# aexoden/snesimage

Measured on AMD Instinct MI355X. Metric: candidate palettes scored/sec, higher is better.
Workload: dtype f32

## Files before the change

snesimage_amd/csrc/capi.hip:

```cpp
#include "../../include/snesimage_hip.h"
#include "kernels.hpp"
#include "kernels_opt.hpp"
#include "kernels_fast.hpp"
#include "kernels_sparse.hpp"
#include "kernels_sparse2.hpp"
#include "kernels_batch.hpp"
#include "kernels_shared.hpp"
#include "kernels_tile.hpp"
#include "kernels_level.hpp"
#include "kernels_char.hpp"
#include "kernels_char_set.hpp"
#include "kernels_export.hpp"
#include "kernels_import.hpp"
#include "kernels_guide.hpp"
#include "kernels_guide_lab.hpp"
#include "kernels_guide_window.hpp"
#include "kernels_guide_set_window.hpp"

#include <hip/hip_runtime.h>

#include <atomic>
#include <cmath>
#include <cstdio>
#include <cstdlib>
// ... 65 lines not shown
    z = (z ^ (z >> 30)) * 0xBF58476D1CE4E5B9ull;
    z = (z ^ (z >> 27)) * 0x94D049BB133111EBull;
    return z ^ (z >> 31);
}

template <typename T> void dfree(T *&p) { if (p) { (void)hipFree(p); p = nullptr; } }

std::atomic<int> g_fail_alloc_in{-1};
template <typename T> hipError_t dmalloc(T **p, size_t bytes) {
    int left = g_fail_alloc_in.load(std::memory_order_relaxed);
    while (left >= 0) {
        if (g_fail_alloc_in.compare_exchange_weak(left, left - 1, std::memory_order_relaxed)) { if (left == 0) { *p = nullptr; return hipErrorOutOfMemory; } break; }
    }
    return hipMalloc(p, bytes);
}
std::atomic<bool> g_poison_alloc{false};

}

struct snesimage_ctx {
    int device = 0;
    hipStream_t own_stream = nullptr, stream = nullptr;
    uint32_t W = 0, H = 0, sub_count = 0, sub_size = 0, flags = 0;
    int ncol = 0;
    bool dither = false, perceptual = false, nes = false;
    bool backdrop = false, tied_call = false; uint32_t user_size = 0;
    bool dither4 = true; uint32_t dither4_max = 512;
    bool ditherw = true;
    bool dither_rec = true;
    Geom G{};
    BlurK K{};
    size_t npx = 0, src_floats = 0;
    uint32_t chunk = 4096, chunk_alloc = 0;

    std::vector<uint8_t> h_orig; float h_eotf[256], h_lab_eotf[256];

    uint8_t *d_orig = nullptr, *d_tile_pal = nullptr, *d_colors = nullptr, *d_map = nullptr;
    unsigned long long *d_pack = nullptr, *d_packT = nullptr, *d_packC4 = nullptr, *d_packR4 = nullptr;
    float *d_img1C4 = nullptr, *d_mu1R4 = nullptr, *d_sd1R4 = nullptr, *d_a1 = nullptr, *d_a1R4 = nullptr; double *d_r1 = nullptr, *d_r1R4 = nullptr;
    int fast_mask = 0;
    float *d_eotf = nullptr, *d_lab_eotf = nullptr;
    uint32_t *d_pal_rgb8 = nullptr; float *d_pal_lin = nullptr, *d_pal_xyb = nullptr, *d_pal_lab = nullptr;
    float *d_lin0 = nullptr, *d_img1 = nullptr, *d_img1T = nullptr, *d_mu1 = nullptr, *d_sd1 = nullptr;
    float *d_labpx = nullptr, *d_labpxT = nullptr;
    uint8_t *d_target = nullptr, *d_target_own = nullptr; float *d_labpx_t = nullptr, *d_labpxT_t = nullptr, *d_labpx_t_own = nullptr, *d_labpxT_t_own = nullptr;
    uint32_t od_n = 0; int8_t od_tab[256] = {};
    uint32_t od_L = 0; int8_t od_bank[8 * 256] = {}; uint8_t od_level[1024] = {}; uint8_t *d_level = nullptr;
    struct snesimage_levelwork *lvl = nullptr;
    float *d_work = nullptr, *d_cand_tab = nullptr, *d_cand_lab = nullptr;
    double *d_part = nullptr;
    uint8_t *d_maps = nullptr, *d_mapsT = nullptr, *d_mapsC4 = nullptr, *d_mapsR4 = nullptr;
    uint8_t *d_subC4 = nullptr, *d_subR4 = nullptr;
    uint8_t *d_bestmap = nullptr, *d_bestmaps_all = nullptr; BestRec *d_bestrec = nullptr, *d_bestrecs_all = nullptr; int *d_skip = nullptr;
    uint4 *d_rplist = nullptr; int *d_rcount = nullptr;
    float *d_rtab = nullptr, *d_rlab = nullptr; uint32_t rtab_cap = 0;
    bool map_pending = false;
    bool best_valid = false, map_synced = false;
    struct Lane { hipStream_t stream = nullptr; float *d_work = nullptr, *d_cand_tab = nullptr, *d_cand_lab = nullptr; double *d_part = nullptr; uint8_t *d_maps = nullptr, *d_mapsT = nullptr, *d_mapsC4 = nullptr, *d_mapsR4 = nullptr, *d_bestmap = nullptr; BestRec *d_bestrec = nullptr; hipEvent_t done = nullptr; };
    std::vector<Lane> extra; uint32_t nlanes = 2; hipEvent_t ev_ready = nullptr;
    struct Sparse {
        bool lpt = true;
        bool down1 = true;
        bool counters_cleared = false;
        uint32_t h2q_max = 512;
        bool down_tiles = true;
        uint32_t h0_min = 1024;
        bool base_down_side = false;
        uint32_t h0_grid = 8192;
        hipStream_t h0_stream[8] = {}; hipEvent_t ev_scan[8] = {}, ev_h0[8] = {}, ev_hn[8] = {}, ev_vn[8] = {};
        bool v0_aside = true;
        hipEvent_t ev_v0[8] = {};
        bool vn_aside = true;
        uint32_t tiles_grid = 4096;
        uint32_t down1_grid = 32768;
        bool vsplit = true;
        uint32_t scan4_max = 2048;
        uint32_t hgrid = 8192;
        bool weight_mask = true;
        bool h_planes = true;
        bool v2_pair = true;
        uint32_t h_forms = 3;
        bool debug_poison = false;
        bool dedup = true; uint32_t dedup_min = 1024; int *holder = nullptr; bool holder_dirty = false;
        bool enabled = false, side = true; uint32_t min_n = 1; uint32_t cap = 0, lanes = 0;
        SparseGeom S{};
        float *store = nullptr, *cand_tab = nullptr, *cand_lab = nullptr, *ckf = nullptr, *ckh = nullptr; long long zeros_off = 0; uint32_t *bitmap = nullptr; double *cka = nullptr, *part = nullptr;
        CandMeta *meta = nullptr; unsigned int *items = nullptr; int *item_count = nullptr; long long item_stride = 0; int *order = nullptr, *first = nullptr;
        uint4 *plist = nullptr; int *plist_count = nullptr; bool plist_valid = false;
        hipStream_t base_stream = nullptr; hipEvent_t ev_base_in = nullptr, ev_base_h = nullptr, ev_base_done = nullptr, ev_base_narrow = nullptr;
        uint8_t *dmaps = nullptr, *dmapsC4 = nullptr;
        uint8_t *bmap = nullptr, *bmapC4 = nullptr, *bcand = nullptr; unsigned long long *dpack = nullptr; double *ckd = nullptr; uint32_t slot_ci = 0;
        float *rec_lab = nullptr;
        int base_sp = -1, base_si = -1;
        struct Ahead { uint8_t *bmap = nullptr, *bmapC4 = nullptr, *bcand = nullptr; unsigned long long *dpack = nullptr; double *ckd = nullptr; float *btab = nullptr, *blab = nullptr, *rec_lab = nullptr; int *ok = nullptr;
                       hipEvent_t ev = nullptr; bool on = true, have = false; int sp = -1, si = -1; unsigned long long epoch = 0; } ahead;
    } sp;
    uint8_t *d_cand = nullptr; uint32_t cand_cap = 0;
    uint8_t *d_cand_sel = nullptr;
    double *d_errs = nullptr, *d_errs_sel = nullptr;
    double *d_inc_err = nullptr;
    StepResult *d_last = nullptr;
    double *d_scratch_err = nullptr;
    uint8_t *d_dummy_cand = nullptr;
    KmeansWork km{};
    double *d_tile_cost = nullptr; int *d_tile_any = nullptr; unsigned int *d_tile_moved = nullptr;

    struct snesimage_batch *owner = nullptr;
    struct snesimage_group *group = nullptr;
    hipEvent_t ev_own = nullptr;
    struct snesimage_window *win = nullptr;
    bool win_pend = false;
    bool pack_borrowed = false;
    uint32_t pb_w = 1, pb_h = 1;
    struct snesimage_tilework *tile = nullptr;
    struct snesimage_charwork *chr = nullptr;
    struct snesimage_guidework *guide = nullptr;
    uint32_t guide_proxy = 0;
    bool guide_capture = false; std::vector<uint8_t> guide_captured; uint32_t guide_captured_k = 0;

    bool tables_valid = false, src_valid = false, inc_valid = false;
    unsigned long long epoch = 0; bool epoch_by_commit = false;
    int pack_mode = -1, pack_sp = -1, pack_si = -1; bool pack_valid = false;
    uint32_t pend_n = 0, pend_sp = 0, pend_si = 0, pend_method = 0; bool pend = false;

    int timing = 0;
    double t_ms[3] = {0.0, 0.0, 0.0}; uint64_t t_launches = 0, t_cands = 0;
    struct TimingRec { hipEvent_t ev[6]; uint32_t n; bool light; };
    std::vector<TimingRec> t_pending;
};

namespace {

int32_t alloc_lane(snesimage_ctx *c, uint32_t chunk, float *&d_work, float *&d_cand_tab, float *&d_cand_lab, double *&d_part, uint8_t *&d_maps, uint8_t *&d_mapsT, uint8_t *&d_mapsC4, uint8_t *&d_mapsR4) {
    dfree(d_work); dfree(d_cand_tab); dfree(d_cand_lab); dfree(d_part); dfree(d_maps); dfree(d_mapsT); dfree(d_mapsC4); dfree(d_mapsR4);
    HIPCHK(dmalloc(&d_work, sizeof(float) * (size_t)c->G.cand_stride * chunk));
    HIPCHK(dmalloc(&d_cand_tab, sizeof(float) * 8 * (size_t)chunk));
    HIPCHK(dmalloc(&d_cand_lab, sizeof(float) * 3 * (size_t)chunk));
    HIPCHK(dmalloc(&d_part, sizeof(double) * (size_t)chunk * kMaxScales * 18));
    if (c->dither) {
        HIPCHK(dmalloc(&d_maps, c->npx * (size_t)chunk));
        HIPCHK(dmalloc(&d_mapsT, c->npx * (size_t)chunk));
        HIPCHK(dmalloc(&d_mapsC4, c->npx * (size_t)chunk));
        HIPCHK(dmalloc(&d_mapsR4, c->npx * (size_t)chunk));
    }
    return SNES_OK;
}
int32_t alloc_workspace(snesimage_ctx *c, uint32_t chunk, uint32_t lanes = 1) {
    if (c->dither || c->perceptual) lanes = c->nlanes;
    if (lanes > c->nlanes) lanes = c->nlanes;
    if (lanes < c->extra.size() + 1) lanes = (uint32_t)c->extra.size() + 1;
    if (c->chunk_alloc >= chunk && c->extra.size() + 1 >= lanes) return SNES_OK;
    if (chunk < c->chunk_alloc) chunk = c->chunk_alloc;
    HIPCHK(hipStreamSynchronize(c->stream));
    for (auto &L : c->extra) HIPCHK(hipStreamSynchronize(L.stream));
    c->chunk_alloc = 0;
    CHECK(alloc_lane(c, chunk, c->d_work, c->d_cand_tab, c->d_cand_lab, c->d_part, c->d_maps, c->d_mapsT, c->d_mapsC4, c->d_mapsR4));
    if (!c->ev_ready) HIPCHK(hipEventCreateWithFlags(&c->ev_ready, hipEventDisableTiming));
    while (c->extra.size() + 1 < lanes) {
        snesimage_ctx::Lane L;
        HIPCHK(hipStreamCreateWithFlags(&L.stream, hipStreamNonBlocking));
        HIPCHK(hipEventCreateWithFlags(&L.done, hipEventDisableTiming));
        c->extra.push_back(L);
    }
    for (auto &L : c->extra) CHECK(alloc_lane(c, chunk, L.d_work, L.d_cand_tab, L.d_cand_lab, L.d_part, L.d_maps, L.d_mapsT, L.d_mapsC4, L.d_mapsR4));
    if (c->dither && !c->d_bestmaps_all) {
        HIPCHK(dmalloc(&c->d_bestmaps_all, c->npx * (size_t)c->nlanes));
        HIPCHK(dmalloc(&c->d_bestrecs_all, sizeof(BestRec) * c->nlanes));
        HIPCHK(dmalloc(&c->d_skip, sizeof(int)));
    }
    if (c->d_bestmaps_all) {
        c->d_bestmap = c->d_bestmaps_all; c->d_bestrec = c->d_bestrecs_all;
        for (size_t l = 0; l < c->extra.size(); l++) { c->extra[l].d_bestmap = c->d_bestmaps_all + (l + 1) * c->npx; c->extra[l].d_bestrec = c->d_bestrecs_all + (l + 1); }
    }
    c->chunk_alloc = chunk;
    return SNES_OK;
}

int32_t ensure_cand_capacity(snesimage_ctx *c, uint32_t n) {
    if (c->cand_cap >= n) return SNES_OK;
    if (c->stream) HIPCHK(hipStreamSynchronize(c->stream));
    c->cand_cap = 0;
    dfree(c->d_cand); dfree(c->d_cand_sel); dfree(c->d_errs); dfree(c->d_errs_sel);
    uint32_t cap = n < 64 ? 64 : n;
    HIPCHK(dmalloc(&c->d_cand, 3 * (size_t)cap));
    HIPCHK(dmalloc(&c->d_cand_sel, 3 * (size_t)cap));
    HIPCHK(dmalloc(&c->d_errs, sizeof(double) * cap));
    HIPCHK(dmalloc(&c->d_errs_sel, sizeof(double) * cap));
    c->cand_cap = cap;
    return SNES_OK;
}

int32_t ensure_tables(snesimage_ctx *c) {
    if (c->tables_valid) return SNES_OK;
    int n = c->ncol + 2;
    hipLaunchKernelGGL(k_palette_tables, dim3((n + 63) / 64), dim3(64), 0, c->stream, c->d_colors, c->ncol, c->d_eotf, c->d_pal_rgb8, c->d_pal_lin, c->d_pal_xyb);
    if (c->perceptual)
        hipLaunchKernelGGL(k_palette_lab, dim3((c->ncol + 63) / 64), dim3(64), 0, c->stream, c->d_pal_rgb8, c->ncol, c->d_lab_eotf, c->d_pal_lab);
    HIPCHK(hipGetLastError());
    c->tables_valid = true;
    return SNES_OK;
}

int32_t ensure_source(snesimage_ctx *c) {
    if (c->src_valid) return SNES_OK;
    CHECK(alloc_workspace(c, 1));
    const Geom &G = c->G;
    hipLaunchKernelGGL(k_source_scale0, dim3((unsigned)((c->npx + 255) / 256)), dim3(256), 0, c->stream, c->d_orig, c->d_eotf, (int)c->W, (int)c->H, c->d_lin0,
                       c->d_img1, c->d_img1T);
    if (G.nscales > 1) {
        DownParams D{}; D.G = G; D.lin0 = c->d_lin0; D.work = c->d_img1; D.workT = c->d_img1T;
        hipLaunchKernelGGL(k_downscale_chain<false>, dim3(down_grid(G), 1), dim3(256), 0, c->stream, D);
    }
    for (int s = 0; s < G.nscales; s++) {
        HParams Hp{}; Hp.G = G; Hp.K = c->K; Hp.s = s; Hp.npairs = 3; Hp.ncol = c->ncol;
        Hp.in1T = c->d_img1T + G.src_off[s]; Hp.in2T = c->d_img1T + G.src_off[s]; Hp.work = c->d_work;
        int ppw = 256 / G.sh[s];
        hipLaunchKernelGGL((k_hpass<false, false>), dim3((3 + ppw - 1) / ppw), dim3(256), 0, c->stream, Hp);
        VParams Vp{}; Vp.G = G; Vp.K = c->K; Vp.s = s; Vp.npairs = 3; Vp.ncol = c->ncol;
        Vp.img1 = c->d_img1 + G.src_off[s]; Vp.mu1_out = c->d_mu1 + G.src_off[s]; Vp.sd1_out = c->d_sd1 + G.src_off[s]; Vp.a1_out = c->d_a1 + G.src_off[s]; Vp.r1_out = c->d_r1 + G.src_off[s]; Vp.work = c->d_work;
        int ppv = 256 / G.sw[s];
        hipLaunchKernelGGL((k_vpass<false, true, false>), dim3((3 + ppv - 1) / ppv), dim3(256), 0, c->stream, Vp);
    }
    bool padded = false;
    for (int s = 0; s < G.nscales; s++) padded = padded || G.th[s] != G.sh[s];
    if (padded)
        hipLaunchKernelGGL(k_src_pad_rows, dim3(16, G.nscales), dim3(256), 0, c->stream, G, c->d_sd1, c->d_r1);
    for (int s = 0; s < G.nscales; s++)
        if ((c->fast_mask & (1 << s)) || c->sp.enabled) {
            const int N = G.sw[s] * G.sh[s];
            hipLaunchKernelGGL(k_relayout, dim3((N + 255) / 256), dim3(256), 0, c->stream, c->d_img1 + G.src_off[s], G.sw[s], G.sh[s], (float *)nullptr, c->d_img1C4 + G.src_off[s]);
            hipLaunchKernelGGL(k_relayout, dim3((N + 255) / 256), dim3(256), 0, c->stream, c->d_mu1 + G.src_off[s], G.sw[s], G.sh[s], c->d_mu1R4 + G.src_off[s], (float *)nullptr);
            hipLaunchKernelGGL(k_relayout, dim3((N + 255) / 256), dim3(256), 0, c->stream, c->d_sd1 + G.src_off[s], G.sw[s], G.sh[s], c->d_sd1R4 + G.src_off[s], (float *)nullptr);
            hipLaunchKernelGGL(k_relayout, dim3((N + 255) / 256), dim3(256), 0, c->stream, c->d_a1 + G.src_off[s], G.sw[s], G.sh[s], c->d_a1R4 + G.src_off[s], (float *)nullptr);
            hipLaunchKernelGGL(k_relayout_f64, dim3((N + 255) / 256), dim3(256), 0, c->stream, c->d_r1 + G.src_off[s], G.sw[s], G.sh[s], c->d_r1R4 + G.src_off[s]);
        }
    if (c->perceptual)
        hipLaunchKernelGGL(k_pixel_lab, dim3((unsigned)((c->npx + 255) / 256)), dim3(256), 0, c->stream, c->d_orig, c->d_lab_eotf, (int)c->W, (int)c->H, c->d_labpx, c->d_labpxT);
    HIPCHK(hipGetLastError());
    c->src_valid = true;
    return SNES_OK;
}

int32_t run_prep(snesimage_ctx *c, int mode, int sp, int si) {
    if (c->pack_valid && c->pack_mode == mode && ((mode != 2 && mode != 3) || (c->pack_sp == sp && c->pack_si == si))) return SNES_OK;
    CHECK(ensure_tables(c));
    if (c->perceptual) CHECK(ensure_source(c));
    PrepParams P{};
    P.orig = c->d_target; P.tile_pal = c->d_tile_pal; P.pal_rgb8 = c->d_pal_rgb8; P.map = c->d_map; P.pack = c->d_pack; P.packT = c->d_packT; P.packC4 = c->d_packC4; P.packR4 = c->d_packR4; P.subC4 = c->d_subC4; P.subR4 = c->d_subR4;
    P.labpx = c->d_labpx_t; P.pal_lab = c->d_pal_lab;
    P.W = (int)c->W; P.H = (int)c->H; P.sub_size = (int)c->sub_size; P.ncol = c->ncol; P.mode = mode; P.sp = sp; P.si = si; P.perceptual = c->perceptual ? 1 : 0;
    c->sp.counters_cleared = false;
    if (mode == 2 && c->sp.plist_count) {
        P.zero = c->sp.plist_count; P.nzero = 1; c->sp.counters_cleared = true;
    }
    hipLaunchKernelGGL(k_prep, dim3((unsigned)((c->npx + 255) / 256)), dim3(256), 0, c->stream, P);
    HIPCHK(hipGetLastError());
    c->pack_valid = true; c->pack_mode = mode; c->pack_sp = sp; c->pack_si = si;
    c->sp.plist_valid = false;
    return SNES_OK;
}

int32_t prep_for_slot(snesimage_ctx *c, int sp, int si) { return c->dither ? run_prep(c, 1, -1, -1) : (c->tied_call ? run_prep(c, 3, -1, si) : run_prep(c, 2, sp, si)); }

struct DenseView {
    const unsigned long long *pack, *packT, *packC4, *packR4; const uint8_t *subC4, *subR4, *tile_pal;
    float *work, *cand_tab, *cand_lab; double *part; const uint8_t *maps, *mapsT, *mapsC4, *mapsR4;
    bool use_maps, perceptual;
};
int32_t score_stages(snesimage_ctx *c, const DenseView &V, uint32_t nc, double *d_errors, int err_stride, int err_offset, snesimage_ctx::TimingRec *tr) {
    const Geom &G = c->G;
    const int npairs = (int)nc * 3;
    if (G.nscales > 1) {
        DownParams D{}; D.G = G; D.pack = V.pack; D.pal_lin = c->d_pal_lin; D.cand_tab = V.cand_tab; D.cand_lab = V.cand_lab; D.labpx = c->d_labpx_t;
        D.work = V.work; D.ncol = c->ncol; D.perceptual = V.perceptual ? 1 : 0; D.use_maps = V.use_maps ? 1 : 0; D.fast_mask = c->fast_mask & ~1; D.maps = V.maps; D.tile_pal = V.tile_pal; D.sub_size = (int)c->sub_size;
        hipLaunchKernelGGL(k_downscale_chain<true>, dim3(down_grid(G), nc), dim3(256), 0, c->stream, D);
    }
    const bool fast0 = (c->fast_mask & 1) && (V.use_maps || !V.perceptual);
    auto is_fast = [&](int s) { return s == 0 ? fast0 : ((c->fast_mask >> s) & 1) != 0; };
    auto fast_params = [&](int s) {
        FastParams F{}; F.G = G; F.K = c->K; F.s = s; F.npairs = npairs; F.ncol = c->ncol;
        F.packC4 = V.packC4; F.packR4 = V.packR4; F.pal_xyb = c->d_pal_xyb; F.cand_tab = V.cand_tab;
        F.use_maps = V.use_maps ? 1 : 0; F.mapsC4 = reinterpret_cast<const uint32_t *>(V.mapsC4); F.mapsR4 = reinterpret_cast<const uint32_t *>(V.mapsR4);
        F.subC4 = reinterpret_cast<const uint32_t *>(V.subC4); F.subR4 = reinterpret_cast<const uint32_t *>(V.subR4);
        F.img1C4 = c->d_img1C4 + G.src_off[s]; F.mu1R4 = c->d_mu1R4 + G.src_off[s]; F.sd1R4 = c->d_sd1R4 + G.src_off[s]; F.a1R4 = c->d_a1R4 + G.src_off[s]; F.r1R4 = c->d_r1R4 + G.src_off[s];
        F.work = V.work; F.part = V.part;
        return F;
    };
    for (int s = 0; s < G.nscales; s++) {
        if (s == 0 && tr && c->timing == 1) HIPCHK(hipEventRecord(tr->ev[1], c->stream));
        if (is_fast(s)) {
            FastParams F = fast_params(s);
            dim3 grid((unsigned)(npairs * (G.sh[s] / 64)));
            if (s == 0) hipLaunchKernelGGL((k_hpass_fast<true>), grid, dim3(64), 0, c->stream, F);
            else hipLaunchKernelGGL((k_hpass_fast<false>), grid, dim3(64), 0, c->stream, F);
        } else {
            HParams Hp{}; Hp.G = G; Hp.K = c->K; Hp.s = s; Hp.npairs = npairs; Hp.ncol = c->ncol; Hp.perceptual = V.perceptual ? 1 : 0; Hp.use_maps = V.use_maps ? 1 : 0; Hp.sub_size = (int)c->sub_size;
            Hp.packT = V.packT; Hp.pal_xyb = c->d_pal_xyb; Hp.cand_tab = V.cand_tab; Hp.cand_lab = V.cand_lab; Hp.labpxT = c->d_labpxT_t;
            Hp.in1T = c->d_img1T + G.src_off[s]; Hp.in2T = nullptr; Hp.work = V.work; Hp.mapsT = V.mapsT; Hp.tile_pal = V.tile_pal;
            int ppw = 256 / G.sh[s];
            dim3 grid((npairs + ppw - 1) / ppw);
            if (s == 0) {
                if (V.perceptual && !V.use_maps) hipLaunchKernelGGL((k_hpass<true, true>), grid, dim3(256), 0, c->stream, Hp);
                else hipLaunchKernelGGL((k_hpass<true, false>), grid, dim3(256), 0, c->stream, Hp);
            } else hipLaunchKernelGGL((k_hpass<false, false>), grid, dim3(256), 0, c->stream, Hp);
        }
        if (s == 0 && tr && c->timing == 1) HIPCHK(hipEventRecord(tr->ev[2], c->stream));
        if (s == 0 && tr && c->timing) HIPCHK(hipEventRecord(tr->ev[3], c->stream));
        int ppv = 256 / G.sw[s];
        dim3 grid((npairs + ppv - 1) / ppv);
        if (is_fast(s)) {
            FastParams F = fast_params(s);
            if (s == 0) hipLaunchKernelGGL((k_vpass_fast<true>), grid, dim3(256), 0, c->stream, F);
            else hipLaunchKernelGGL((k_vpass_fast<false>), grid, dim3(256), 0, c->stream, F);
        } else {
            VParams Vp{}; Vp.G = G; Vp.K = c->K; Vp.s = s; Vp.npairs = npairs; Vp.ncol = c->ncol; Vp.perceptual = V.perceptual ? 1 : 0; Vp.use_maps = V.use_maps ? 1 : 0; Vp.sub_size = (int)c->sub_size;
            Vp.pack = V.pack; Vp.pal_xyb = c->d_pal_xyb; Vp.cand_tab = V.cand_tab; Vp.cand_lab = V.cand_lab; Vp.labpx = c->d_labpx_t;
            Vp.mu1 = c->d_mu1 + G.src_off[s]; Vp.sd1 = c->d_sd1 + G.src_off[s]; Vp.a1 = c->d_a1 + G.src_off[s]; Vp.r1 = c->d_r1 + G.src_off[s]; Vp.work = V.work; Vp.part = V.part;
            Vp.maps = V.maps; Vp.tile_pal = V.tile_pal;
            if (s == 0) {
                if (V.perceptual && !V.use_maps) hipLaunchKernelGGL((k_vpass<true, false, true>), grid, dim3(256), 0, c->stream, Vp);
                else hipLaunchKernelGGL((k_vpass<true, false, false>), grid, dim3(256), 0, c->stream, Vp);
            } else hipLaunchKernelGGL((k_vpass<false, false, false>), grid, dim3(256), 0, c->stream, Vp);
        }
        if (s == 0 && tr && c->timing) HIPCHK(hipEventRecord(tr->ev[4], c->stream));
    }
    hipLaunchKernelGGL(k_final_score, dim3((nc + 63) / 64), dim3(64), 0, c->stream, V.part, (int)nc, G, d_errors, err_stride, err_offset);
    return SNES_OK;
}

void launch_dither(snesimage_ctx *c, const DitherParams &Dp, uint32_t nblocks) {
    if (c->perceptual && c->dither4 && nblocks <= c->dither4_max) hipLaunchKernelGGL((k_dither4_lab<0>), dim3(nblocks), dim3(512), 0, c->stream, Dp);
    else if (c->perceptual) hipLaunchKernelGGL((k_dither<true, 0>), dim3(nblocks), dim3(128), 0, c->stream, Dp);
    else if (c->dither4 && nblocks <= c->dither4_max && c->sub_size == 15) hipLaunchKernelGGL((k_dither4<15, 0>), dim3(nblocks), dim3(512), 0, c->stream, Dp);
    else if (c->dither4 && nblocks <= c->dither4_max && c->sub_size == 16) hipLaunchKernelGGL((k_dither4<16, 0>), dim3(nblocks), dim3(512), 0, c->stream, Dp);
    else if (c->dither4 && nblocks <= c->dither4_max) hipLaunchKernelGGL((k_dither4<0, 0>), dim3(nblocks), dim3(512), 0, c->stream, Dp);
    else if (c->sub_size == 15) hipLaunchKernelGGL((k_dither<false, 15>), dim3(nblocks), dim3(128), 0, c->stream, Dp);
    else if (c->sub_size == 16) hipLaunchKernelGGL((k_dither<false, 16>), dim3(nblocks), dim3(128), 0, c->stream, Dp);
    else hipLaunchKernelGGL((k_dither<false, 0>), dim3(nblocks), dim3(128), 0, c->stream, Dp);
}

int32_t score_chunk(snesimage_ctx *c, const uint8_t *d_rgb5, uint32_t nc, double *d_errors, int err_stride, int err_offset, int sp, int si, uint8_t *d_maps_out) {
    const bool use_maps = c->dither;
    const uint32_t slot_ci = c->tied_call ? (kTiedSlot | (c->sub_size << 8) | (uint32_t)si) : (sp >= 0) ? (uint32_t)(sp * (int)c->sub_size + si) : 0xffffffffu;
    snesimage_ctx::TimingRec tr{}; tr.n = nc;
    if (c->timing) { for (int i = 0; i < 6; i++) HIPCHK(hipEventCreate(&tr.ev[i])); if (c->timing == 1) HIPCHK(hipEventRecord(tr.ev[0], c->stream)); }
    hipLaunchKernelGGL(k_candidate_tables, dim3((nc + 63) / 64), dim3(64), 0, c->stream, d_rgb5, (int)nc, c->d_eotf, c->d_cand_tab);
    hipLaunchKernelGGL(k_candidate_slot, dim3((nc + 63) / 64), dim3(64), 0, c->stream, c->d_cand_tab, (int)nc, slot_ci);
    if (c->perceptual) hipLaunchKernelGGL(k_candidate_lab, dim3((nc + 63) / 64), dim3(64), 0, c->stream, c->d_cand_tab, (int)nc, c->d_lab_eotf, c->d_cand_lab);
    if (use_maps) {
        DitherParams Dp{};
        Dp.orig = c->d_orig; Dp.tile_pal = c->d_tile_pal; Dp.pal_rgb8 = c->d_pal_rgb8; Dp.pal_lab = c->d_pal_lab; Dp.cand_tab = c->d_cand_tab; Dp.cand_lab = c->d_cand_lab;
        Dp.lab_eotf = c->d_lab_eotf; Dp.maps = c->d_maps; Dp.mapsC4 = c->d_mapsC4;
        Dp.W = (int)c->W; Dp.H = (int)c->H; Dp.sub_size = (int)c->sub_size; Dp.ncol = c->ncol; Dp.slot_ci = slot_ci; Dp.perceptual = c->perceptual ? 1 : 0;
        launch_dither(c, Dp, nc);
        hipLaunchKernelGGL(k_maps_relayout, dim3((unsigned)(c->H / 4), nc), dim3(256), 0, c->stream, c->d_maps, (int)c->W, (int)c->H,
                           reinterpret_cast<uint32_t *>(c->d_mapsR4), (c->fast_mask & 1) ? (uint32_t *)nullptr : reinterpret_cast<uint32_t *>(c->d_mapsT));
        if (d_maps_out) HIPCHK(hipMemcpyAsync(d_maps_out, c->d_maps, c->npx * (size_t)nc, hipMemcpyDeviceToDevice, c->stream));
    } else if (d_maps_out) {
        MapsParams M{}; M.pack = c->d_pack; M.cand_tab = c->d_cand_tab; M.cand_lab = c->d_cand_lab; M.labpx = c->d_labpx_t; M.maps = d_maps_out;
        M.npx = (int)c->npx; M.ncol = c->ncol; M.sub_size = (int)c->sub_size; M.si = si < 0 ? 0 : si; M.ncand = (int)nc; M.perceptual = c->perceptual ? 1 : 0;
        hipLaunchKernelGGL(k_candidate_maps, dim3((unsigned)((c->npx + 255) / 256), nc), dim3(256), 0, c->stream, M);
    }
    { DenseView V{c->d_pack, c->d_packT, c->d_packC4, c->d_packR4, c->d_subC4, c->d_subR4, c->d_tile_pal, c->d_work, c->d_cand_tab, c->d_cand_lab, c->d_part, c->d_maps, c->d_mapsT, c->d_mapsC4, c->d_mapsR4,
                  use_maps, c->perceptual};
      CHECK(score_stages(c, V, nc, d_errors, err_stride, err_offset, &tr)); }
    if (use_maps) hipLaunchKernelGGL(k_keep_best, dim3(1), dim3(1024), 0, c->stream, d_errors, err_stride, err_offset, (int)nc, c->d_maps, (int)c->npx, c->d_bestrec, c->d_bestmap);
    HIPCHK(hipGetLastError());
    if (c->timing) { tr.light = c->timing != 1; if (!tr.light) HIPCHK(hipEventRecord(tr.ev[5], c->stream)); c->t_pending.push_back(tr); }
    return SNES_OK;
}

SparseParams sparse_params(snesimage_ctx *c, uint32_t lane);

int32_t sparse_alloc(snesimage_ctx *c, uint32_t need, uint32_t lanes = 1) {
    auto &sp = c->sp;
    if (lanes > c->nlanes) lanes = c->nlanes;
    if (sp.cap >= need && sp.lanes >= lanes) return SNES_OK;
    if (need < sp.cap) need = sp.cap;
    if (lanes < sp.lanes) lanes = sp.lanes;
    HIPCHK(hipStreamSynchronize(c->stream));
    for (auto &L : c->extra) HIPCHK(hipStreamSynchronize(L.stream));
    if (sp.base_stream) HIPCHK(hipStreamSynchronize(sp.base_stream));
    sp.cap = 0; sp.lanes = 0; sp.plist_valid = false;
    dfree(sp.store); dfree(sp.cand_tab); dfree(sp.ckf); dfree(sp.cka); dfree(sp.part); dfree(sp.meta); dfree(sp.items); dfree(sp.item_count); dfree(sp.plist); sp.plist_count = nullptr;
    const Geom &G = c->G;
    SparseGeom &S = sp.S;
    long long off = 0, okf = 0, oka = 0, okh = 0; int go = 0;
    for (int s = 0; s < G.nscales; s++) {
        const long long N = (long long)G.sw[s] * G.sh[s];
        S.off_lin[s] = off; if (s >= 1) off += 3 * N;
        S.off_xybC[s] = off; if (s >= 1) off += 3 * N;
        S.off_xybR[s] = off; off += 3 * N;
        S.off_hout[s] = off; off += 9 * N;
        S.off_ckf[s] = okf; okf += 3LL * (G.sh[s] / 4 + 2) * 18 * G.sw[s];
        S.off_cka[s] = oka; oka += 3LL * (G.sh[s] / 4 + 2) * 6 * G.sw[s];
        S.off_ckh[s] = okh; if (G.sw[s] >= 64) okh += 3LL * 3 * 18 * G.sh[s];
        S.goff[s] = go; go += G.sh[s] / 4;
    }
    S.cand_stride = off;
    const size_t ncap = (size_t)lanes * need + 1;
    sp.item_stride = (long long)need * (G.sh[0] / 4) * 3;
    HIPCHK(dmalloc(&sp.store, sizeof(float) * (size_t)S.cand_stride * ncap));
    if (g_poison_alloc.load()) HIPCHK(hipMemsetAsync(sp.store, 0xff, sizeof(float) * (size_t)S.cand_stride * ncap, c->stream));
    HIPCHK(dmalloc(&sp.cand_tab, sizeof(float) * 8 * ncap));
    if (c->perceptual) {
        dfree(sp.cand_lab); dfree(sp.bitmap);
        HIPCHK(dmalloc(&sp.cand_lab, sizeof(float) * 3 * ncap));
        HIPCHK(dmalloc(&sp.bitmap, sizeof(uint32_t) * (c->npx / 32) * ncap));
    }
    HIPCHK(dmalloc(&sp.ckf, sizeof(float) * (size_t)okf));
    dfree(sp.ckh); HIPCHK(dmalloc(&sp.ckh, sizeof(float) * (size_t)(okh + 12LL * G.W + 256)));
    sp.zeros_off = okh;
    HIPCHK(hipMemsetAsync(sp.ckh + okh, 0, sizeof(float) * 12 * (size_t)G.W, c->stream));
    HIPCHK(dmalloc(&sp.cka, sizeof(double) * (size_t)oka));
    HIPCHK(dmalloc(&sp.part, sizeof(double) * ncap * kMaxScales * 18));
    HIPCHK(dmalloc(&sp.meta, sizeof(CandMeta) * ncap));
    dfree(sp.order); HIPCHK(dmalloc(&sp.order, sizeof(int) * ncap));
    dfree(sp.first); HIPCHK(dmalloc(&sp.first, sizeof(int) * ncap));
    HIPCHK(dmalloc(&sp.items, sizeof(unsigned int) * (size_t)sp.item_stride * kItemLists * (c->nlanes + 1)));
    if (!sp.base_stream && sp.side) {
        int prio_lo = 0, prio_hi = 0;
        HIPCHK(hipDeviceGetStreamPriorityRange(&prio_lo, &prio_hi));
        HIPCHK(hipStreamCreateWithPriority(&sp.base_stream, hipStreamNonBlocking, prio_hi));
        HIPCHK(hipEventCreateWithFlags(&sp.ev_base_in, hipEventDisableTiming));
        HIPCHK(hipEventCreateWithFlags(&sp.ev_base_h, hipEventDisableTiming));
        HIPCHK(hipEventCreateWithFlags(&sp.ev_base_narrow, hipEventDisableTiming));
        HIPCHK(hipEventCreateWithFlags(&sp.ev_base_done, hipEventDisableTiming));
    }
    HIPCHK(dmalloc(&sp.item_count, sizeof(int) * (kItemLists * (c->nlanes + 1) + 1)));
    HIPCHK(hipMemsetAsync(sp.item_count, 0, sizeof(int) * (kItemLists * (c->nlanes + 1) + 1), c->stream));
    sp.plist_count = sp.item_count + (size_t)kItemLists * (c->nlanes + 1);
    sp.counters_cleared = true;
    HIPCHK(dmalloc(&sp.plist, sizeof(uint4) * c->npx));
    if (c->dither) {
        dfree(sp.dmaps); dfree(sp.dmapsC4); dfree(sp.bmap); dfree(sp.bmapC4); dfree(sp.bcand); dfree(sp.dpack); dfree(sp.ckd);
        HIPCHK(dmalloc(&sp.dmaps, c->npx * (size_t)need * lanes));
        HIPCHK(dmalloc(&sp.dmapsC4, c->npx * (size_t)need * lanes));
        HIPCHK(dmalloc(&sp.bmap, c->npx)); HIPCHK(dmalloc(&sp.bmapC4, c->npx)); HIPCHK(dmalloc(&sp.bcand, 64));
        HIPCHK(dmalloc(&sp.dpack, sizeof(unsigned long long) * c->npx));
        HIPCHK(dmalloc(&sp.ckd, sizeof(double) * 3 * c->W * (c->H / 4 + 1)));
        dfree(sp.rec_lab); if (c->perceptual) HIPCHK(dmalloc(&sp.rec_lab, sizeof(float) * 3 * c->npx));
        auto &ah = sp.ahead;
        dfree(ah.bmap); dfree(ah.bmapC4); dfree(ah.bcand); dfree(ah.dpack); dfree(ah.ckd); dfree(ah.btab); dfree(ah.blab); dfree(ah.rec_lab); dfree(ah.ok); ah.have = false;
        if (ah.on && sp.side && c->sub_size > 1) {
            HIPCHK(dmalloc(&ah.bmap, c->npx)); HIPCHK(dmalloc(&ah.bmapC4, c->npx)); HIPCHK(dmalloc(&ah.bcand, 64)); HIPCHK(dmalloc(&ah.btab, sizeof(float) * 8)); HIPCHK(dmalloc(&ah.ok, sizeof(int)));
            HIPCHK(dmalloc(&ah.dpack, sizeof(unsigned long long) * c->npx));
            HIPCHK(dmalloc(&ah.ckd, sizeof(double) * 3 * c->W * (c->H / 4 + 1)));
            if (c->perceptual) { HIPCHK(dmalloc(&ah.blab, sizeof(float) * 3)); HIPCHK(dmalloc(&ah.rec_lab, sizeof(float) * 3 * c->npx)); }
            if (!ah.ev) HIPCHK(hipEventCreateWithFlags(&ah.ev, hipEventDisableTiming));
        }
    }
    sp.cap = need; sp.lanes = lanes; sp.plist_valid = false;
    {
        SparseParams P = sparse_params(c, c->nlanes);
        P.is_base = 1; P.ncand = 1; P.k0 = P.base;
        hipLaunchKernelGGL(k_sparse_scan, dim3(1), dim3(1024), 0, c->stream, P);
        HIPCHK(hipGetLastError());
    }
    HIPCHK(hipStreamSynchronize(c->stream));
    return SNES_OK;
}

SparseParams sparse_params(snesimage_ctx *c, uint32_t lane) {
    auto &sp = c->sp;
    SparseParams P{};
    P.G = c->G; P.S = sp.S; P.K = c->K; P.ncol = c->ncol; P.base = (int)(sp.lanes * sp.cap);
    P.pack = c->d_pack; P.packC4 = c->d_packC4; P.packR4 = c->d_packR4; P.plist = sp.plist; P.plist_count = sp.plist_count;
    P.pal_lin = c->d_pal_lin; P.pal_xyb = c->d_pal_xyb; P.cand_tab = sp.cand_tab;
    P.perceptual = c->perceptual ? 1 : 0; P.labpx = c->d_labpx_t; P.cand_lab = sp.cand_lab; P.bitmap = sp.bitmap;
    P.img1C4 = c->d_img1C4; P.mu1R4 = c->d_mu1R4; P.sd1R4 = c->d_sd1R4; P.a1R4 = c->d_a1R4; P.r1R4 = c->d_r1R4;
    P.store = sp.store; P.meta = sp.meta;
    P.items = sp.items + (size_t)lane * sp.item_stride * kItemLists; P.item_count = sp.item_count + (size_t)lane * kItemLists; P.item_stride = sp.item_stride;
    P.ckf = sp.ckf; P.cka = sp.cka; P.part = sp.part; P.first = sp.first; P.ckh = sp.ckh; P.zeros = sp.ckh + sp.zeros_off; P.trash = sp.ckh + sp.zeros_off + 12LL * c->G.W;
    for (P.s_first = 0; P.s_first < c->G.nscales && c->G.sw[P.s_first] >= 64; P.s_first++) {}
    P.full_sums = sp.weight_mask ? 0 : 1;
    P.h_planes = (sp.weight_mask && sp.h_planes) ? 1 : 0;
    P.v2_pair = (sp.weight_mask && sp.v2_pair) ? v2_pair_channels(c->G) : 0;
    if (c->dither) {
        const uint32_t l = lane < c->nlanes ? lane : 0;
        P.use_maps = 1; P.sub_size = (int)c->sub_size; P.slot_ci = sp.slot_ci; P.subC4 = c->d_subC4; P.tile_pal = c->d_tile_pal;
        P.perceptual = 0; P.labpx = sp.rec_lab;
        P.maps = sp.dmaps + (size_t)l * sp.cap * c->npx; P.mapsC4 = sp.dmapsC4 + (size_t)l * sp.cap * c->npx; P.bmap = sp.bmap; P.bmapC4 = sp.bmapC4;
    }
    return P;
}

static size_t h2_lds(const snesimage_ctx *c) { return sizeof(float) * 3 * (size_t)(c->ncol + 2); }

static void launch_sparse_h2(const snesimage_ctx *c, const SparseParams &P, size_t gx, unsigned ny, bool h0_only, hipStream_t st) {
    const uint32_t forms = c->sp.h_forms;
    const size_t lds = h2_lds(c);
    const int nfree = h2_free_channels(c->G);
    if ((forms & 4) && h0_only && P.h_planes && !P.full_sums && nfree > 0 && nfree < 3) {
        size_t g1 = gx * (size_t)nfree / 3; if (g1 < 1) g1 = 1;
        const size_t g2 = gx - gx * (size_t)nfree / 3 + 1;
        const dim3 d1((unsigned)g1, ny), d2((unsigned)g2, ny);
        if (!(forms & 2)) { hipLaunchKernelGGL(k_sparse_h2_one<-1>, d1, dim3(64), lds, st, P); hipLaunchKernelGGL(k_sparse_h2_full<-1>, d2, dim3(64), lds, st, P); }
        else if (c->dither) { hipLaunchKernelGGL(k_sparse_h2_one<1>, d1, dim3(64), lds, st, P); hipLaunchKernelGGL(k_sparse_h2_full<1>, d2, dim3(64), lds, st, P); }
        else { hipLaunchKernelGGL(k_sparse_h2_one<0>, d1, dim3(64), lds, st, P); hipLaunchKernelGGL(k_sparse_h2_full<0>, d2, dim3(64), lds, st, P); }
        return;
    }
    const dim3 d((unsigned)gx, ny);
    if (!(forms & 2)) hipLaunchKernelGGL(k_sparse_h2, d, dim3(64), lds, st, P);
    else if (c->dither) hipLaunchKernelGGL(k_sparse_h2_um<true>, d, dim3(64), lds, st, P);
    else hipLaunchKernelGGL(k_sparse_h2_um<false>, d, dim3(64), lds, st, P);
}

int32_t sparse_base_pass(snesimage_ctx *c, int sp_idx, int si, uint32_t n_cand) {
    auto &sp = c->sp;
    const Geom &G = c->G;
    if (!sp.plist_valid) {
        if (!sp.counters_cleared) HIPCHK(hipMemsetAsync(sp.plist_count, 0, sizeof(int), c->stream));
        sp.counters_cleared = false;
        const unsigned long long *win_pack = c->d_pack;
        if (c->dither) {
            const uint32_t j0 = c->sub_size > 1 ? ((uint32_t)si + 1u) % c->sub_size : (uint32_t)si;
            sp.slot_ci = (uint32_t)(sp_idx * (int)c->sub_size + si);
            auto &ah = sp.ahead;
            const int *b_done = nullptr;
            const bool same_state = ah.epoch == c->epoch;
            if (ah.have && ah.sp == sp_idx && ah.si == si && (same_state || (ah.epoch + 1 == c->epoch && c->epoch_by_commit))) {
                std::swap(sp.bmap, ah.bmap); std::swap(sp.bmapC4, ah.bmapC4); std::swap(sp.dpack, ah.dpack); std::swap(sp.ckd, ah.ckd); std::swap(sp.rec_lab, ah.rec_lab);
                hipLaunchKernelGGL(k_ahead_ok, dim3(1), dim3(1), 0, c->stream, same_state ? (const StepResult *)nullptr : c->d_last, ah.ok);
                HIPCHK(hipStreamWaitEvent(c->stream, ah.ev, 0));
                b_done = ah.ok;
            }
            ah.have = false;
            HIPCHK(hipMemcpyAsync(sp.bcand, c->d_colors + 3 * (size_t)(sp_idx * (int)c->sub_size + (int)j0), 3, hipMemcpyDeviceToDevice, c->stream));
            float *btab = sp.cand_tab + 8 * (size_t)(sp.lanes * sp.cap);
            hipLaunchKernelGGL(k_candidate_tables, dim3(1), dim3(64), 0, c->stream, sp.bcand, 1, c->d_eotf, btab);
            DitherParams Dp{};
            Dp.orig = c->d_orig; Dp.tile_pal = c->d_tile_pal; Dp.pal_rgb8 = c->d_pal_rgb8; Dp.cand_tab = btab; Dp.maps = sp.bmap; Dp.mapsC4 = sp.bmapC4;
            Dp.W = (int)c->W; Dp.H = (int)c->H; Dp.sub_size = (int)c->sub_size; Dp.ncol = c->ncol; Dp.slot_ci = sp.slot_ci;
            Dp.rec_pack = sp.dpack; Dp.ck_out = sp.ckd; Dp.excl_sub = sp_idx; Dp.excl_si = si; Dp.excl_j0 = (int)j0; Dp.skip = b_done;
            if (c->perceptual) {
                float *blab = sp.cand_lab + 3 * (size_t)(sp.lanes * sp.cap);
                hipLaunchKernelGGL(k_candidate_lab, dim3(1), dim3(64), 0, c->stream, btab, 1, c->d_lab_eotf, blab);
                Dp.pal_lab = c->d_pal_lab; Dp.cand_lab = blab; Dp.lab_eotf = c->d_lab_eotf; Dp.perceptual = 1; Dp.rec_lab = sp.rec_lab;
                if (c->dither4) hipLaunchKernelGGL((k_dither4_lab<1>), dim3(1), dim3(512), 0, c->stream, Dp); else hipLaunchKernelGGL((k_dither<true, 0, 1>), dim3(1), dim3(128), 0, c->stream, Dp);
            } else
            if (c->dither4 && c->sub_size == 15) hipLaunchKernelGGL((k_dither4<15, 1>), dim3(1), dim3(512), 0, c->stream, Dp);
            else if (c->dither4 && c->sub_size == 16) hipLaunchKernelGGL((k_dither4<16, 1>), dim3(1), dim3(512), 0, c->stream, Dp);
            else if (c->dither4) hipLaunchKernelGGL((k_dither4<0, 1>), dim3(1), dim3(512), 0, c->stream, Dp);
            else if (c->sub_size == 15) hipLaunchKernelGGL((k_dither<false, 15, 1>), dim3(1), dim3(128), 0, c->stream, Dp);
            else if (c->sub_size == 16) hipLaunchKernelGGL((k_dither<false, 16, 1>), dim3(1), dim3(128), 0, c->stream, Dp);
            else hipLaunchKernelGGL((k_dither<false, 0, 1>), dim3(1), dim3(128), 0, c->stream, Dp);
            win_pack = sp.dpack;
        }
        hipLaunchKernelGGL(k_build_plist, dim3((unsigned)((c->npx + 255) / 256)), dim3(256), 0, c->stream, win_pack, (int)c->npx, sp.plist, sp.plist_count);
        SparseParams P = sparse_params(c, c->nlanes);
        P.is_base = 1; P.ncand = 1; P.k0 = P.base;
        hipStream_t bs = sp.side ? sp.base_stream : c->stream;
        const bool down_with_sweeps = sp.side && n_cand >= sp.h0_min && sp.h0_min > 0;
        sp.base_down_side = down_with_sweeps;
        if (!down_with_sweeps) hipLaunchKernelGGL(k_base_down, dim3(down_grid(G)), dim3(256), 0, c->stream, P);
        if (sp.side) { HIPCHK(hipEventRecord(sp.ev_base_in, c->stream)); HIPCHK(hipStreamWaitEvent(bs, sp.ev_base_in, 0)); }
        if (down_with_sweeps) hipLaunchKernelGGL(k_base_down, dim3(down_grid(G)), dim3(256), 0, bs, P);
        if (sp.h2q_max > 0) hipLaunchKernelGGL(k_sparse_h2q_base, dim3((unsigned)((G.sh[0] / 4 * 3 + 3) / 4), (unsigned)(P.s_first * kColBuckets)), dim3(64), h2_lds(c), bs, P);
        else hipLaunchKernelGGL(k_sparse_h2_base, dim3((unsigned)((G.sh[0] / 4 * 3 + 15) / 16), (unsigned)(P.s_first * kColBuckets)), dim3(64), h2_lds(c), bs, P);
        if (sp.side) HIPCHK(hipEventRecord(sp.ev_base_h, bs));
        if (P.s_first > 0 && sp.vsplit) hipLaunchKernelGGL(k_sparse_v2_base_split, dim3((unsigned)(G.W >> 6), 3, (unsigned)P.s_first), dim3(128), 0, bs, P);
        else if (P.s_first > 0) hipLaunchKernelGGL(k_sparse_v2_base, dim3(3, (unsigned)P.s_first), dim3(256), 0, bs, P);
        if (sp.side) HIPCHK(hipEventRecord(sp.ev_base_done, bs));
        if (P.s_first < G.nscales) hipLaunchKernelGGL(k_sparse_h, dim3((unsigned)((G.sh[P.s_first] / 4 * 3 + 15) / 16), (unsigned)((G.nscales - P.s_first) * kColBuckets)), dim3(64), 0, bs, P);
        if (P.s_first < G.nscales) hipLaunchKernelGGL(k_sparse_v_base_narrow, dim3(3, (unsigned)(G.nscales - P.s_first)), dim3(256), 0, bs, P);
        HIPCHK(hipGetLastError());
        if (sp.side) HIPCHK(hipEventRecord(sp.ev_base_narrow, bs));
        if (c->dither && sp.side && sp.ahead.dpack) {
            auto &ah = sp.ahead;
            int ni = si + 1, np = sp_idx;
            if (ni == (int)c->sub_size) { ni = 0; np = (np + 1) % (int)c->sub_count; }
            const int nj0 = (ni + 1) % (int)c->sub_size;
            HIPCHK(hipMemcpyAsync(ah.bcand, c->d_colors + 3 * (size_t)(np * (int)c->sub_size + nj0), 3, hipMemcpyDeviceToDevice, bs));
            hipLaunchKernelGGL(k_candidate_tables, dim3(1), dim3(64), 0, bs, ah.bcand, 1, c->d_eotf, ah.btab);
            DitherParams Dn{};
            Dn.orig = c->d_orig; Dn.tile_pal = c->d_tile_pal; Dn.pal_rgb8 = c->d_pal_rgb8; Dn.cand_tab = ah.btab; Dn.maps = ah.bmap; Dn.mapsC4 = ah.bmapC4;
            Dn.W = (int)c->W; Dn.H = (int)c->H; Dn.sub_size = (int)c->sub_size; Dn.ncol = c->ncol; Dn.slot_ci = (uint32_t)(np * (int)c->sub_size + ni);
            Dn.rec_pack = ah.dpack; Dn.ck_out = ah.ckd; Dn.excl_sub = np; Dn.excl_si = ni; Dn.excl_j0 = nj0;
            if (c->perceptual) {
                hipLaunchKernelGGL(k_candidate_lab, dim3(1), dim3(64), 0, bs, ah.btab, 1, c->d_lab_eotf, ah.blab);
                Dn.pal_lab = c->d_pal_lab; Dn.cand_lab = ah.blab; Dn.lab_eotf = c->d_lab_eotf; Dn.perceptual = 1; Dn.rec_lab = ah.rec_lab;
                if (c->dither4) hipLaunchKernelGGL((k_dither4_lab<1>), dim3(1), dim3(512), 0, bs, Dn); else hipLaunchKernelGGL((k_dither<true, 0, 1>), dim3(1), dim3(128), 0, bs, Dn);
            } else
            if (c->dither4 && c->sub_size == 15) hipLaunchKernelGGL((k_dither4<15, 1>), dim3(1), dim3(512), 0, bs, Dn);
            else if (c->dither4 && c->sub_size == 16) hipLaunchKernelGGL((k_dither4<16, 1>), dim3(1), dim3(512), 0, bs, Dn);
            else if (c->dither4) hipLaunchKernelGGL((k_dither4<0, 1>), dim3(1), dim3(512), 0, bs, Dn);
            else if (c->sub_size == 15) hipLaunchKernelGGL((k_dither<false, 15, 1>), dim3(1), dim3(128), 0, bs, Dn);
            else if (c->sub_size == 16) hipLaunchKernelGGL((k_dither<false, 16, 1>), dim3(1), dim3(128), 0, bs, Dn);
            else hipLaunchKernelGGL((k_dither<false, 0, 1>), dim3(1), dim3(128), 0, bs, Dn);
            HIPCHK(hipGetLastError());
            HIPCHK(hipEventRecord(ah.ev, bs));
            ah.have = true; ah.sp = np; ah.si = ni; ah.epoch = c->epoch;
        }
        sp.plist_valid = true;
    }
    return SNES_OK;
}

int32_t sparse_score_chunk(snesimage_ctx *c, uint32_t lane, hipStream_t stream, const uint8_t *d_rgb5, uint32_t nc, double *d_errors, int err_stride, int err_offset, int list0 = -1) {
    auto &sp = c->sp;
    const Geom &G = c->G;
    SparseParams P = sparse_params(c, lane);
    P.is_base = 0; P.ncand = (int)nc; P.k0 = (int)(lane * sp.cap);
    if (list0 >= 0) { P.holder = sp.holder; P.list0 = list0; }
    if (sp.debug_poison) HIPCHK(hipMemsetAsync(sp.store + (size_t)P.k0 * sp.S.cand_stride, 0xff, sizeof(float) * (size_t)sp.S.cand_stride * nc, stream));
    snesimage_ctx::TimingRec tr{}; tr.n = nc;
    if (c->timing) { for (int i = 0; i < 6; i++) HIPCHK(hipEventCreate(&tr.ev[i])); if (c->timing == 1) HIPCHK(hipEventRecord(tr.ev[0], stream)); }
    if (list0 >= 0) hipLaunchKernelGGL(k_candidate_tables_mark, dim3((nc + 63) / 64), dim3(64), 0, stream, d_rgb5, (int)nc, c->d_eotf, sp.cand_tab + 8 * (size_t)P.k0, sp.holder, list0);
    else
    hipLaunchKernelGGL(k_candidate_tables, dim3((nc + 63) / 64), dim3(64), 0, stream, d_rgb5, (int)nc, c->d_eotf, sp.cand_tab + 8 * (size_t)P.k0);
    if (c->dither) {
        if (c->perceptual) {
            hipLaunchKernelGGL(k_candidate_lab, dim3((nc + 63) / 64), dim3(64), 0, stream, sp.cand_tab + 8 * (size_t)P.k0, (int)nc, c->d_lab_eotf, sp.cand_lab + 3 * (size_t)P.k0);
            hipLaunchKernelGGL(k_dither_first_lab, dim3(nc), dim3(256), 0, stream, P);
        } else
        hipLaunchKernelGGL(k_dither_first, dim3((nc + 15) / 16), dim3(1024), 0, stream, P);
        DitherParams Dp{};
        Dp.orig = c->d_orig; Dp.tile_pal = c->d_tile_pal; Dp.pal_rgb8 = c->d_pal_rgb8; Dp.cand_tab = sp.cand_tab + 8 * (size_t)P.k0;
        Dp.maps = const_cast<uint8_t *>(P.maps); Dp.mapsC4 = const_cast<uint8_t *>(P.mapsC4);
        Dp.W = (int)c->W; Dp.H = (int)c->H; Dp.sub_size = (int)c->sub_size; Dp.ncol = c->ncol; Dp.slot_ci = sp.slot_ci;
        Dp.first_group = sp.first; Dp.first_k0 = P.k0; Dp.ck_in = sp.ckd; Dp.bmap = sp.bmap; Dp.bmapC4 = sp.bmapC4; Dp.rec_in = c->dither_rec ? sp.dpack : nullptr;
        if (c->sp.lpt) {
            hipLaunchKernelGGL(k_sparse_order, dim3(1), dim3(1024), 0, stream, P, sp.order + P.k0); Dp.order = sp.order + P.k0;
        }
        if (c->perceptual) {
            Dp.pal_lab = c->d_pal_lab; Dp.cand_lab = sp.cand_lab + 3 * (size_t)P.k0; Dp.lab_eotf = c->d_lab_eotf; Dp.perceptual = 1;
            if (c->dither4 && nc <= c->dither4_max) hipLaunchKernelGGL((k_dither4_lab<2>), dim3(nc), dim3(512), 0, stream, Dp); else hipLaunchKernelGGL((k_dither<true, 0, 2>), dim3(nc), dim3(128), 0, stream, Dp);
        } else
        if (c->dither4 && nc <= c->dither4_max && c->sub_size == 15) hipLaunchKernelGGL((k_dither4<15, 2>), dim3(nc), dim3(512), 0, stream, Dp);
        else if (c->dither4 && nc <= c->dither4_max && c->sub_size == 16) hipLaunchKernelGGL((k_dither4<16, 2>), dim3(nc), dim3(512), 0, stream, Dp);
        else if (c->dither4 && nc <= c->dither4_max) hipLaunchKernelGGL((k_dither4<0, 2>), dim3(nc), dim3(512), 0, stream, Dp);
        else if (c->ditherw && c->sub_size == 15) hipLaunchKernelGGL((k_ditherw<15>), dim3((nc + 3) / 4), dim3(256), 0, stream, Dp, (int)nc);
        else if (c->ditherw && c->sub_size == 16) hipLaunchKernelGGL((k_ditherw<16>), dim3((nc + 3) / 4), dim3(256), 0, stream, Dp, (int)nc);
        else if (c->ditherw && c->sub_size > 1) hipLaunchKernelGGL((k_ditherw<0>), dim3((nc + 3) / 4), dim3(256), 0, stream, Dp, (int)nc);
        else if (c->sub_size == 15) hipLaunchKernelGGL((k_dither<false, 15, 2>), dim3(nc), dim3(128), 0, stream, Dp);
        else if (c->sub_size == 16) hipLaunchKernelGGL((k_dither<false, 16, 2>), dim3(nc), dim3(128), 0, stream, Dp);
        else hipLaunchKernelGGL((k_dither<false, 0, 2>), dim3(nc), dim3(128), 0, stream, Dp);
        hipLaunchKernelGGL(k_dither_diff, dim3((nc + 3) / 4), dim3(1024), 0, stream, P);
    } else if (c->perceptual) {
        hipLaunchKernelGGL(k_candidate_lab, dim3((nc + 63) / 64), dim3(64), 0, stream, sp.cand_tab + 8 * (size_t)P.k0, (int)nc, c->d_lab_eotf, sp.cand_lab + 3 * (size_t)P.k0);
        HIPCHK(hipMemsetAsync(sp.bitmap + (size_t)P.k0 * (c->npx / 32), 0, sizeof(uint32_t) * (c->npx / 32) * nc, stream));
        hipLaunchKernelGGL(k_sparse_scan_lab, dim3(nc), dim3(256), 0, stream, P);
    } else if (nc <= sp.scan4_max) hipLaunchKernelGGL(k_sparse_scan4, dim3((nc + 3) / 4), dim3(1024), 0, stream, P);
    else hipLaunchKernelGGL(k_sparse_scan, dim3((nc + 15) / 16), dim3(1024), 0, stream, P);
    bool vn_aside = false;
    const bool h0_ahead = sp.side && sp.h0_min > 0 && nc >= sp.h0_min && nc > sp.h2q_max && lane < 8 && P.s_first > 0;
    const bool v0_aside = h0_ahead && sp.v0_aside;
    vn_aside = h0_ahead && !v0_aside && sp.vn_aside && P.s_first < G.nscales;
    if (c->sp.lpt && nc > 512) P.order = sp.order + P.k0;
    if (h0_ahead) {
        if (!sp.h0_stream[lane]) {
            HIPCHK(hipStreamCreateWithFlags(&sp.h0_stream[lane], hipStreamNonBlocking));
            HIPCHK(hipEventCreateWithFlags(&sp.ev_scan[lane], hipEventDisableTiming));
            HIPCHK(hipEventCreateWithFlags(&sp.ev_h0[lane], hipEventDisableTiming));
            HIPCHK(hipEventCreateWithFlags(&sp.ev_hn[lane], hipEventDisableTiming));
            HIPCHK(hipEventCreateWithFlags(&sp.ev_v0[lane], hipEventDisableTiming));
            HIPCHK(hipEventCreateWithFlags(&sp.ev_vn[lane], hipEventDisableTiming));
        }
        hipStream_t hs = sp.h0_stream[lane];
        HIPCHK(hipEventRecord(sp.ev_scan[lane], stream));
        HIPCHK(hipStreamWaitEvent(hs, sp.ev_scan[lane], 0));
        HIPCHK(hipStreamWaitEvent(hs, sp.ev_base_h, 0));
        size_t gx = ((size_t)nc * (G.sh[0] / 4) * 3 + 15) / 16; if (gx > sp.h0_grid) gx = sp.h0_grid;
        launch_sparse_h2(c, P, gx, (unsigned)kColBuckets, true, hs);
        if (c->sp.lpt) hipLaunchKernelGGL(k_sparse_order, dim3(1), dim3(1024), 0, hs, P, sp.order + P.k0);
        HIPCHK(hipEventRecord(sp.ev_h0[lane], hs));
        if (v0_aside) {
            HIPCHK(hipStreamWaitEvent(hs, sp.ev_base_done, 0));
            if (c->timing) HIPCHK(hipEventRecord(tr.ev[3], hs));
            hipLaunchKernelGGL(k_sparse_v2, dim3(v2_pair_grid(nc, P.v2_pair), 1), dim3(256), 0, hs, P);
            if (c->timing) HIPCHK(hipEventRecord(tr.ev[4], hs));
            HIPCHK(hipEventRecord(sp.ev_v0[lane], hs));
        }
    }
    if (sp.down1 && G.nscales > 2) {
        size_t gd = (size_t)nc * 8; if (gd > sp.down1_grid) gd = sp.down1_grid;
        hipLaunchKernelGGL(k_sparse_down1, dim3((unsigned)gd), dim3(256), 0, stream, P);
        if (sp.side && sp.base_down_side) HIPCHK(hipStreamWaitEvent(stream, sp.ev_base_h, 0));
        if (sp.down_tiles && G.nscales >= 4) {
            size_t gt = ((size_t)nc * (G.sh[3] / 4) + SNES_DOWN_TILES_U - 1) / SNES_DOWN_TILES_U; if (gt > sp.tiles_grid) gt = sp.tiles_grid;
            hipLaunchKernelGGL(k_sparse_down_tiles, dim3((unsigned)gt), dim3(256), 0, stream, P);
        } else
        hipLaunchKernelGGL(k_sparse_down, dim3(nc), dim3(256), 0, stream, P, -2);
    } else { if (sp.side && sp.base_down_side) HIPCHK(hipStreamWaitEvent(stream, sp.ev_base_h, 0)); hipLaunchKernelGGL(k_sparse_down, dim3(nc), dim3(256), 0, stream, P, 0); }
    if (sp.side && !sp.base_down_side) HIPCHK(hipStreamWaitEvent(stream, sp.ev_base_h, 0));
    if (c->timing == 1) HIPCHK(hipEventRecord(tr.ev[1], stream));
    { size_t gx = ((size_t)nc * (G.sh[0] / 4) * 3 + 15) / 16; if (gx > sp.hgrid) gx = sp.hgrid;
      if (nc <= sp.h2q_max) {
          size_t gq = ((size_t)nc * (G.sh[0] / 4) * 3 + 3) / 4; if (gq > sp.hgrid) gq = sp.hgrid;
          hipLaunchKernelGGL(k_sparse_h2q, dim3((unsigned)gq, (unsigned)(P.s_first * kColBuckets)), dim3(64), h2_lds(c), stream, P);
      } else
      if (h0_ahead) {
          if (P.s_first > 1 && (sp.h_forms & 1)) hipLaunchKernelGGL(k_sparse_h2_from, dim3((unsigned)gx, (unsigned)((P.s_first - 1) * kColBuckets)), dim3(64), h2_lds(c), stream, P, (int)kColBuckets);
          else if (P.s_first > 1) hipLaunchKernelGGL(k_sparse_h2_from_all, dim3((unsigned)gx, (unsigned)((P.s_first - 1) * kColBuckets)), dim3(64), h2_lds(c), stream, P, (int)kColBuckets);
      } else
      launch_sparse_h2(c, P, gx, (unsigned)(P.s_first * kColBuckets), false, stream);
      if (P.s_first < G.nscales) hipLaunchKernelGGL(k_sparse_h, dim3((unsigned)((gx + 7) / 8), (unsigned)((G.nscales - P.s_first) * kColBuckets)), dim3(64), 0, stream, P);
      if (vn_aside) HIPCHK(hipEventRecord(sp.ev_hn[lane], stream));
      if (h0_ahead) HIPCHK(hipStreamWaitEvent(stream, sp.ev_h0[lane], 0)); }
    if (c->timing == 1) HIPCHK(hipEventRecord(tr.ev[2], stream));
    if (sp.side || stream != c->stream) HIPCHK(hipStreamWaitEvent(stream, sp.side ? sp.ev_base_done : c->ev_ready, 0));
    if (c->sp.lpt && nc > 512) {
        if (!h0_ahead) hipLaunchKernelGGL(k_sparse_order, dim3(1), dim3(1024), 0, stream, P, sp.order + P.k0);
        P.order = sp.order + P.k0;
    }
    if (vn_aside) {
        hipStream_t hs = sp.h0_stream[lane];
        HIPCHK(hipStreamWaitEvent(hs, sp.ev_hn[lane], 0));
        HIPCHK(hipStreamWaitEvent(hs, sp.ev_base_narrow, 0));
        hipLaunchKernelGGL(k_sparse_v, dim3((nc * 3 + 7) / 8, (unsigned)(G.nscales - P.s_first)), dim3(256), 0, hs, P);
        HIPCHK(hipEventRecord(sp.ev_vn[lane], hs));
    }
    if (v0_aside) {
        if (sp.side) HIPCHK(hipStreamWaitEvent(stream, sp.ev_base_narrow, 0));
        if (P.s_first < G.nscales) hipLaunchKernelGGL(k_sparse_v, dim3((nc * 3 + 7) / 8, (unsigned)(G.nscales - P.s_first)), dim3(256), 0, stream, P);
        if (P.s_first > 1) hipLaunchKernelGGL(k_sparse_v2_from, dim3(nc * 3, (unsigned)(P.s_first - 1)), dim3(256), 0, stream, P, 1);
    } else {
    if (c->timing) HIPCHK(hipEventRecord(tr.ev[3], stream));
    hipLaunchKernelGGL(k_sparse_v2, dim3(P.s_first == 1 ? v2_pair_grid(nc, P.v2_pair) : nc * 3, (unsigned)P.s_first), dim3(256), 0, stream, P);
    if (c->timing) HIPCHK(hipEventRecord(tr.ev[4], stream));
    }
    if (vn_aside) HIPCHK(hipStreamWaitEvent(stream, sp.ev_vn[lane], 0));
    else if (!v0_aside) {
    if (sp.side) HIPCHK(hipStreamWaitEvent(stream, sp.ev_base_narrow, 0));
    if (P.s_first < G.nscales) hipLaunchKernelGGL(k_sparse_v, dim3((nc * 3 + 7) / 8, (unsigned)(G.nscales - P.s_first)), dim3(256), 0, stream, P);
    }
    if (v0_aside) HIPCHK(hipStreamWaitEvent(stream, sp.ev_v0[lane], 0));
    hipLaunchKernelGGL(k_final_score_wave, dim3((nc + 3) / 4), dim3(256), 0, stream, sp.part + (size_t)P.k0 * G.nscales * 18, (int)nc, G, d_errors, err_stride, err_offset, P.item_count, (int)kItemLists);
    if (c->dither) {
        uint8_t *bm = lane == 0 ? c->d_bestmap : c->extra[lane - 1].d_bestmap; BestRec *br = lane == 0 ? c->d_bestrec : c->extra[lane - 1].d_bestrec;
        hipLaunchKernelGGL(k_keep_best, dim3(1), dim3(1024), 0, stream, d_errors, err_stride, err_offset, (int)nc, P.maps, (int)c->npx, br, bm);
    }
    HIPCHK(hipGetLastError());
    if (c->timing) { tr.light = c->timing != 1; if (!tr.light) HIPCHK(hipEventRecord(tr.ev[5], stream)); c->t_pending.push_back(tr); }
    return SNES_OK;
}

struct LaneScope {
    snesimage_ctx *c; snesimage_ctx::Lane *L;
    LaneScope(snesimage_ctx *c_, snesimage_ctx::Lane *L_) : c(c_), L(L_) { swap(); }
    ~LaneScope() { swap(); }
    void swap() { std::swap(c->stream, L->stream); std::swap(c->d_work, L->d_work); std::swap(c->d_cand_tab, L->d_cand_tab); std::swap(c->d_cand_lab, L->d_cand_lab);
                  std::swap(c->d_part, L->d_part); std::swap(c->d_maps, L->d_maps); std::swap(c->d_mapsT, L->d_mapsT); std::swap(c->d_mapsC4, L->d_mapsC4); std::swap(c->d_mapsR4, L->d_mapsR4);
                  std::swap(c->d_bestmap, L->d_bestmap); std::swap(c->d_bestrec, L->d_bestrec); }
};

int32_t score_list(snesimage_ctx *c, const uint8_t *d_rgb5, uint32_t n, double *d_errors, int err_stride, int err_offset, int sp, int si, uint8_t *d_maps_out) {
    uint32_t chunk = (c->dither || c->perceptual) ? (n + c->nlanes - 1) / c->nlanes : n;
    if (chunk < 64) chunk = 64;
    if (chunk > c->chunk) chunk = c->chunk;
    if (c->tied_call && chunk > 1024) chunk = 1024;
    const bool sparse = c->sp.enabled && !c->tied_call && !d_maps_out && sp >= 0 && n >= c->sp.min_n && c->pack_mode == (c->dither ? 1 : 2) && !(c->dither && c->sub_size == 1);
    const uint32_t nchunks = (n + chunk - 1) / chunk;
    const uint32_t nl = nchunks < c->nlanes ? nchunks : c->nlanes;
    CHECK(alloc_workspace(c, sparse ? 1 : chunk, nl));
    CHECK(ensure_tables(c));
    CHECK(ensure_source(c));
    if (sparse) {
        CHECK(sparse_alloc(c, chunk, nl));
        if (c->dither && (c->sp.base_sp != sp || c->sp.base_si != si)) c->sp.plist_valid = false;
        CHECK(sparse_base_pass(c, sp, si, n));
        c->sp.base_sp = sp; c->sp.base_si = si;
    }
    if (c->dither) { hipLaunchKernelGGL(k_reset_best, dim3(1), dim3(64), 0, c->stream, c->d_bestrecs_all, (int)c->nlanes); c->best_valid = true; }
    const bool dedup = sparse && !c->dither && c->sp.dedup && n >= c->sp.dedup_min;
    if (dedup) {
        if (!c->sp.holder) { HIPCHK(dmalloc(&c->sp.holder, sizeof(int) * kDedupColours)); c->sp.holder_dirty = true; }
        if (c->sp.holder_dirty) {
            HIPCHK(hipStreamSynchronize(c->stream));
            for (auto &L : c->extra) HIPCHK(hipStreamSynchronize(L.stream));
            HIPCHK(hipMemsetAsync(c->sp.holder, kNoHolder & 0xff, sizeof(int) * kDedupColours, c->stream));
        }
        c->sp.holder_dirty = true;
    }
    if (nl > 1) {
        HIPCHK(hipEventRecord(c->ev_ready, c->stream));
        for (uint32_t l = 1; l < nl; l++) HIPCHK(hipStreamWaitEvent(c->extra[l - 1].stream, c->ev_ready, 0));
    }
    uint32_t i = 0;
    for (uint32_t c0 = 0; c0 < n; c0 += chunk, i++) {
        const uint32_t nc = (n - c0 < chunk) ? (n - c0) : chunk;
        const uint32_t lane = i % nl;
        uint8_t *mo = d_maps_out ? d_maps_out + (size_t)c0 * c->npx : nullptr;
        const int eo = err_offset + (int)c0 * err_stride;
        if (sparse) { CHECK(sparse_score_chunk(c, lane, lane == 0 ? c->stream : c->extra[lane - 1].stream, d_rgb5 + 3 * (size_t)c0, nc, d_errors, err_stride, eo, dedup ? (int)c0 : -1)); continue; }
        if (lane == 0) CHECK(score_chunk(c, d_rgb5 + 3 * (size_t)c0, nc, d_errors, err_stride, eo, sp, si, mo));
        else { LaneScope ls(c, &c->extra[lane - 1]); CHECK(score_chunk(c, d_rgb5 + 3 * (size_t)c0, nc, d_errors, err_stride, eo, sp, si, mo)); }
    }
    for (uint32_t l = 1; l < nl; l++) {
        HIPCHK(hipEventRecord(c->extra[l - 1].done, c->extra[l - 1].stream));
        HIPCHK(hipStreamWaitEvent(c->stream, c->extra[l - 1].done, 0));
    }
    if (dedup) {
        hipLaunchKernelGGL(k_dedup_copy, dim3(1), dim3(1024), 0, c->stream, d_rgb5, (int)n, c->sp.holder, d_errors, err_stride, err_offset);
        HIPCHK(hipGetLastError());
        c->sp.holder_dirty = false;
    }
    return SNES_OK;
}

int32_t ensure_map(snesimage_ctx *c);

int32_t do_optimize(snesimage_ctx *c, bool may_skip = false) {
    CHECK(ensure_tables(c));
    if (!c->dither) {
        c->pack_valid = false;
        CHECK(run_prep(c, 0, -1, -1));
    } else {
        CHECK(alloc_workspace(c, 1));
        if (c->perceptual) CHECK(ensure_source(c));
        hipLaunchKernelGGL(k_candidate_tables, dim3(1), dim3(64), 0, c->stream, c->d_dummy_cand, 1, c->d_eotf, c->d_cand_tab);
        hipLaunchKernelGGL(k_candidate_slot, dim3(1), dim3(64), 0, c->stream, c->d_cand_tab, 1, 0xffffffffu);
        DitherParams Dp{};
        Dp.orig = c->d_orig; Dp.tile_pal = c->d_tile_pal; Dp.pal_rgb8 = c->d_pal_rgb8; Dp.pal_lab = c->d_pal_lab; Dp.cand_tab = c->d_cand_tab; Dp.cand_lab = c->d_cand_lab;
        Dp.lab_eotf = c->d_lab_eotf; Dp.maps = c->d_map; Dp.skip = may_skip ? c->d_skip : nullptr;
        Dp.W = (int)c->W; Dp.H = (int)c->H; Dp.sub_size = (int)c->sub_size; Dp.ncol = c->ncol; Dp.slot_ci = 0xffffffffu; Dp.perceptual = c->perceptual ? 1 : 0;
        launch_dither(c, Dp, 1);
        HIPCHK(hipGetLastError());
        c->pack_valid = false;
    }
    c->inc_valid = false; c->map_synced = true; c->map_pending = false;
    return SNES_OK;
}

int32_t do_error(snesimage_ctx *c, double *d_out) {
    CHECK(ensure_map(c));
    CHECK(alloc_workspace(c, 1));
    CHECK(ensure_tables(c));
    CHECK(ensure_source(c));
    bool saved_dither = c->dither;
    c->dither = false;
    c->pack_valid = false;
    int32_t rc = run_prep(c, 1, -1, -1);
    if (rc == SNES_OK) rc = score_chunk(c, c->d_dummy_cand, 1, d_out, 1, 0, -1, -1, nullptr);
    c->dither = saved_dither;
    c->pack_valid = false;
    return rc;
}

int32_t ensure_incumbent(snesimage_ctx *c) {
    if (c->inc_valid) return SNES_OK;
    CHECK(do_error(c, c->d_inc_err));
    c->inc_valid = true;
    return SNES_OK;
}

int32_t check_slot(snesimage_ctx *c, uint32_t palette, uint32_t index) {
    if (!c) return fail(SNES_ERR_ARG, "null context");
    if (c->backdrop && palette == c->sub_count && index == 0) return SNES_OK;
    if (palette >= c->sub_count || index >= (c->backdrop ? c->user_size : c->sub_size)) return fail(SNES_ERR_ARG, "palette slot out of range");
    return SNES_OK;
}
struct SlotScope {
    snesimage_ctx *c; uint32_t sp, si; bool saved;
    SlotScope(snesimage_ctx *c_, uint32_t palette, uint32_t index) : c(c_), sp(palette), si(index), saved(c_->tied_call) {
        c->tied_call = c->backdrop && palette == c->sub_count;
        if (c->tied_call) { sp = 0; si = c->user_size; }
    }
    ~SlotScope() { c->tied_call = saved; }
};
bool ordered_tables_equal(const snesimage_ctx *a, const snesimage_ctx *b) { return a->od_n == b->od_n && (a->od_n == 0 || memcmp(a->od_tab, b->od_tab, (size_t)a->od_n * a->od_n) == 0); }
const char *kLevelsRefused = "the context holds an ordered-dither bank of several tables: batches, groups and shared-palette sets share launches and one table (per-tile levels for them are not built yet)";
bool blocked(const snesimage_ctx *c) { return c->pb_w * c->pb_h > 1; }
const char *kBlockedRefused = "the context holds palette blocks (snesimage_set_palette_blocks): blocked members of batches, groups and shared-palette sets are not built yet; set 1 x 1 blocks first";
int untied_block(const uint8_t *tp, uint32_t H, uint32_t bw, uint32_t bh) {
    const uint32_t nbx = 32 / bw, nby = (H / 8) / bh;
    for (uint32_t b = 0; b < nbx * nby; b++) {
        const uint32_t tx0 = (b % nbx) * bw, ty0 = (b / nbx) * bh;
        for (uint32_t ty = ty0; ty < ty0 + bh; ty++)
            for (uint32_t tx = tx0; tx < tx0 + bw; tx++) if (tp[ty * 32 + tx] != tp[ty0 * 32 + tx0]) return (int)b;
    }
    return -1;
}
int block_log2(uint32_t v) { return v == 8 ? 3 : v == 4 ? 2 : v == 2 ? 1 : 0; }
struct BlockGeom { uint32_t bw, bh, nbx, nblock; int lbw, lbh; };
BlockGeom block_geom(const snesimage_ctx *c) {
    BlockGeom g{c->pb_w, c->pb_h, 32 / c->pb_w, (32 / c->pb_w) * ((c->H / 8) / c->pb_h), block_log2(c->pb_w), block_log2(c->pb_h)};
    return g;
}
BlockGeom tile_geom(const snesimage_ctx *c) { return BlockGeom{1, 1, 32, 32 * (c->H / 8), 0, 0}; }
uint32_t block_first_tile(const BlockGeom &g, uint32_t b) { return (b / g.nbx) * g.bh * 32 + (b % g.nbx) * g.bw; }
void block_fill(const BlockGeom &g, uint8_t *tp, uint32_t b, uint8_t v) {
    const uint32_t t0 = block_first_tile(g, b);
    for (uint32_t ty = 0; ty < g.bh; ty++)
        for (uint32_t tx = 0; tx < g.bw; tx++) tp[t0 + ty * 32 + tx] = v;
}
void block_move_launch(snesimage_ctx *c) {
    const BlockGeom g = block_geom(c);
    hipLaunchKernelGGL(k_unit_move, dim3((g.nblock + 255) / 256), dim3(256), 0, c->stream, (const double *)c->d_tile_cost, (const int *)c->d_tile_any, (int)c->H, (int)c->sub_count, g.lbw, g.lbh,
                       c->d_tile_pal, c->d_tile_moved);
}
const char *kBackdropRefused = "SNES_BACKDROP contexts are not supported here: the backdrop schedule is not carried through batches, groups, shared-palette sets and split-phase slot windows";

int32_t batch_quiesce(struct snesimage_batch *b);
int32_t set_device(snesimage_ctx *c) { HIPCHK(hipSetDevice(c->device)); return c->owner ? batch_quiesce(c->owner) : SNES_OK; }

int32_t drain_timing(snesimage_ctx *c) {
    for (auto &r : c->t_pending) {
        float ms = 0.0f;
        HIPCHK(hipEventSynchronize(r.ev[r.light ? 4 : 5]));
        if (!r.light) {
            HIPCHK(hipEventElapsedTime(&ms, r.ev[0], r.ev[5])); c->t_ms[0] += ms;
            HIPCHK(hipEventElapsedTime(&ms, r.ev[1], r.ev[2])); c->t_ms[1] += ms;
        }
        HIPCHK(hipEventElapsedTime(&ms, r.ev[3], r.ev[4])); c->t_ms[2] += ms;
        c->t_launches += 1; c->t_cands += r.n;
        for (int i = 0; i < 6; i++) (void)hipEventDestroy(r.ev[i]);
    }
    c->t_pending.clear();
    return SNES_OK;
}

int32_t gen_candidates(snesimage_ctx *c, uint32_t method, uint32_t palette, uint32_t index, uint32_t channel, uint64_t seed, uint64_t step_id, uint32_t n, uint32_t shard_rank = 0,
                       uint32_t shard_count = 1, double *d_errors = nullptr) {
    const uint64_t key = mix64(seed ^ (step_id * 0x9E3779B97F4A7C15ull) ^ 0xD1B54A32D192ED03ull);
    hipLaunchKernelGGL(k_gen_candidates, dim3((n + 63) / 64), dim3(64), 0, c->stream, (int)method, (int)n, key, c->d_colors, (int)(palette * c->sub_size + index), (int)channel, c->d_cand,
                       (int)shard_rank, (int)shard_count, d_errors ? c->d_cand_sel : (uint8_t *)nullptr, d_errors);
    HIPCHK(hipGetLastError());
    return SNES_OK;
}

uint32_t method_count(uint32_t method, uint32_t n_random) { return method == SNES_METHOD_RANDOM ? (n_random ? n_random : 64u) : (method == SNES_METHOD_CHANNEL ? 32u : kNesColorCount); }

int32_t ensure_map(snesimage_ctx *c) {
    if (!c->map_pending) return SNES_OK;
    c->map_pending = false;
    const bool inc = c->inc_valid;
    CHECK(do_optimize(c));
    c->inc_valid = inc;
    return SNES_OK;
}

int32_t commit(snesimage_ctx *c, const double *d_errors, uint32_t n, uint32_t method, uint32_t palette, uint32_t index) {
    PaletteTables T{};
    if (c->tables_valid) {
        T.eotf = c->d_eotf; T.lab_eotf = c->d_lab_eotf; T.rgb8 = c->d_pal_rgb8; T.lin = c->d_pal_lin; T.xyb = c->d_pal_xyb; T.lab = c->perceptual ? c->d_pal_lab : nullptr;
    }
    hipLaunchKernelGGL(k_commit, dim3(1), dim3(256), 0, c->stream, d_errors, (int)n, c->d_cand, c->d_colors, (int)(palette * c->sub_size + index), method == SNES_METHOD_NES ? 1 : 0, c->d_inc_err,
                       c->d_last, T, c->tied_call ? (int)c->sub_count : 0, (int)c->sub_size);
    HIPCHK(hipGetLastError());
    c->pack_valid = false; c->epoch++; c->epoch_by_commit = true;
    const bool was_synced = c->map_synced;
    if (!c->dither) {
        c->map_pending = true; c->map_synced = true;
        c->inc_valid = was_synced;
        return SNES_OK;
    }
    bool may_skip = false;
    if (c->d_skip) {
        hipLaunchKernelGGL(k_take_best_map, dim3(1), dim3(1024), 0, c->stream, c->d_last, c->d_bestrecs_all, c->best_valid ? (int)c->nlanes : 0, c->d_bestmaps_all, (int)c->npx,
                           c->map_synced ? 1 : 0, c->d_map, c->d_skip);
        may_skip = true;
    }
    c->best_valid = false;
    CHECK(do_optimize(c, may_skip));
    c->inc_valid = was_synced;
    return SNES_OK;
}

}

#include "kmeans_host.inc"

namespace {
int32_t write_backdrop(snesimage_ctx *c, const uint8_t *b) {
    CHECK(ensure_map(c));
    for (uint32_t p = 0; p < c->sub_count; p++)
        HIPCHK(hipMemcpyAsync(c->d_colors + 3 * ((size_t)p * c->sub_size + c->user_size), b, 3, hipMemcpyHostToDevice, c->stream));
    HIPCHK(hipStreamSynchronize(c->stream));
    c->tables_valid = false; c->pack_valid = false; c->inc_valid = false; c->map_synced = false; c->epoch++; c->epoch_by_commit = false;
    return SNES_OK;
}
int32_t read_colors(snesimage_ctx *c, uint8_t *all ) {
    HIPCHK(hipMemcpyAsync(all, c->d_colors, 3 * (size_t)c->ncol, hipMemcpyDeviceToHost, c->stream));
    HIPCHK(hipStreamSynchronize(c->stream));
    return SNES_OK;
}
}

extern "C" {

const char *snesimage_last_error(void) { return g_err.c_str(); }
#ifndef SNES_SRC_HASH
#define SNES_SRC_HASH "unknown"
#endif
const char *snesimage_version(void) { return "snesimage_hip 0.3.0 (gfx950) src:" SNES_SRC_HASH; }

int32_t snesimage_create(const uint8_t *rgba, uint32_t w, uint32_t h, uint32_t sub_count, uint32_t sub_size, uint32_t flags, int32_t device, snesimage_ctx **out) {
    if (!rgba || !out) return fail(SNES_ERR_ARG, "null pointer");
    *out = nullptr;
    if (w != 256) return fail(SNES_ERR_ARG, "image width must be 256 (tile stride is fixed at 32, lib.rs:58)");
    if (h < 8 || h > 256 || (h % 8) != 0) return fail(SNES_ERR_ARG, "image height must be a multiple of 8 in [8,256]");
    if (sub_count < 1 || sub_size < 1 || sub_count > 253 || sub_size > 253 || sub_count * sub_size > 253) return fail(SNES_ERR_ARG, "sub_count*sub_size must be in [1,253]");
    const bool backdrop = (flags & SNES_BACKDROP) != 0;
    if (backdrop && (sub_size > 15 || sub_count * (sub_size + 1) > 253)) return fail(SNES_ERR_ARG, "with SNES_BACKDROP sub_size must be at most 15 and sub_count*(sub_size+1) at most 253");
    if (device < 0) return fail(SNES_ERR_ARG, "device must be a HIP device ordinal >= 0 (this library has no CPU path)");
    int ndev = 0;
    HIPCHK(hipGetDeviceCount(&ndev));
    if (device >= ndev) return fail(SNES_ERR_ARG, "no such HIP device");
    HIPCHK(hipSetDevice(device));
    snesimage_ctx *c = new snesimage_ctx();
    c->backdrop = backdrop; c->user_size = sub_size;
    if (backdrop) sub_size += 1;
    c->device = device; c->W = w; c->H = h; c->sub_count = sub_count; c->sub_size = sub_size; c->flags = flags; c->ncol = (int)(sub_count * sub_size);
    c->dither = flags & SNES_DITHER; c->perceptual = flags & SNES_PERCEPTUAL; c->nes = flags & SNES_NES;
    c->npx = (size_t)w * h;
    c->K = make_blur_constants();
    if (const char *e = getenv("SNES_CHUNK")) { int v = atoi(e); if (v > 0) c->chunk = (uint32_t)v; }
    if (const char *e = getenv("SNES_LANES")) { int v = atoi(e); if (v >= 1 && v <= 8) c->nlanes = (uint32_t)v; }
    c->sp.enabled = true;
    if (const char *e = getenv("SNES_SPARSE")) c->sp.enabled = c->sp.enabled && atoi(e) != 0;
    if (const char *e = getenv("SNES_BASE_STREAM")) c->sp.side = atoi(e) != 0;
    if (const char *e = getenv("SNES_LPT")) c->sp.lpt = atoi(e) != 0;
    if (const char *e = getenv("SNES_DOWN1")) c->sp.down1 = atoi(e) != 0;
    if (const char *e = getenv("SNES_DITHER4")) c->dither4 = atoi(e) != 0;
    if (const char *e = getenv("SNES_DITHERW")) c->ditherw = atoi(e) != 0;
    if (const char *e = getenv("SNES_DITHER_AHEAD")) c->sp.ahead.on = atoi(e) != 0;
    if (const char *e = getenv("SNES_DITHER_REC")) c->dither_rec = atoi(e) != 0;
    if (const char *e = getenv("SNES_DITHER4_MAX")) { int v = atoi(e); if (v >= 0) c->dither4_max = (uint32_t)v; }
    if (const char *e = getenv("SNES_DOWN1_GRID")) { int v = atoi(e); if (v >= 64) c->sp.down1_grid = (uint32_t)v; }
    if (const char *e = getenv("SNES_VSPLIT")) c->sp.vsplit = atoi(e) != 0;
    if (const char *e = getenv("SNES_DOWN_TILES")) c->sp.down_tiles = atoi(e) != 0;
    if (const char *e = getenv("SNES_V0_ASIDE")) c->sp.v0_aside = atoi(e) != 0;
    if (const char *e = getenv("SNES_VN_ASIDE")) c->sp.vn_aside = atoi(e) != 0;
    if (const char *e = getenv("SNES_H0_GRID")) { int v = atoi(e); if (v >= 16) c->sp.h0_grid = (uint32_t)v; }
    if (const char *e = getenv("SNES_H0_MIN")) { int v = atoi(e); if (v >= 0) c->sp.h0_min = (uint32_t)v; }
    if (const char *e = getenv("SNES_TILES_GRID")) { int v = atoi(e); if (v >= 64) c->sp.tiles_grid = (uint32_t)v; }
    if (const char *e = getenv("SNES_SCAN4_MAX")) { int v = atoi(e); if (v >= 0) c->sp.scan4_max = (uint32_t)v; }
    if (const char *e = getenv("SNES_H2Q_MAX")) { int v = atoi(e); if (v >= 0) c->sp.h2q_max = (uint32_t)v; }
    if (const char *e = getenv("SNES_HGRID")) { int v = atoi(e); if (v >= 1) c->sp.hgrid = (uint32_t)v; }
    if (const char *e = getenv("SNES_SPARSE_MIN")) { int v = atoi(e); if (v >= 1) c->sp.min_n = (uint32_t)v; }
    if (const char *e = getenv("SNES_DEDUP")) c->sp.dedup = atoi(e) != 0;
    if (const char *e = getenv("SNES_WEIGHT_MASK")) c->sp.weight_mask = atoi(e) != 0;
    if (const char *e = getenv("SNES_H_PLANES")) c->sp.h_planes = atoi(e) != 0;
    if (const char *e = getenv("SNES_V2_PAIR")) c->sp.v2_pair = atoi(e) != 0;
    if (const char *e = getenv("SNES_H_FORMS")) { int v = atoi(e); if (v >= 0 && v <= 7) c->sp.h_forms = (uint32_t)v; }
    if (const char *e = getenv("SNES_DEBUG_POISON")) c->sp.debug_poison = atoi(e) != 0;
    if (const char *e = getenv("SNES_DEDUP_MIN")) { int v = atoi(e); if (v >= 1) c->sp.dedup_min = (uint32_t)v; }
    Geom &G = c->G;
    G.W = (int)w; G.H = (int)h; G.nscales = 0;
    int P2 = 8;
    while (P2 < (int)h) P2 *= 2;
    for (int s = 0; s < kMaxScales; s++) {
        if (s > 0 && (G.sw[s - 1] < 8 || G.th[s - 1] < 8)) break;
        G.sw[s] = (int)w >> s; G.th[s] = s == 0 ? (int)h : (G.th[s - 1] + 1) / 2; G.sh[s] = s == 0 ? (int)h : P2 >> s; G.nscales = s + 1;
    }
    long long off = 0, soff = 0;
    for (int s = 0; s < G.nscales; s++) {
        long long N = (long long)G.sw[s] * G.sh[s];
        G.src_off[s] = soff; soff += 3 * N;
        if (s >= 1) { G.off_xyb[s] = off; off += 3 * N; G.off_xybT[s] = off; off += 3 * N; } else { G.off_xyb[s] = 0; G.off_xybT[s] = 0; }
        G.off_hout[s] = off; off += 9 * N;
    }
    G.cand_stride = off;
    for (int s = 0; s < G.nscales; s++) if ((G.sw[s] % 64) == 0 && (G.th[s] % 64) == 0 && G.th[s] == G.sh[s]) c->fast_mask |= 1 << s;
    if (const char *e = getenv("SNES_NO_FAST")) { if (atoi(e)) c->fast_mask = 0; }
    c->src_floats = (size_t)soff;

    int32_t rc = SNES_OK;
    auto body = [&]() -> int32_t {
        HIPCHK(hipStreamCreateWithFlags(&c->own_stream, hipStreamNonBlocking));
        c->stream = c->own_stream;
        HIPCHK(hipMalloc(&c->d_orig, c->npx * 4));
        HIPCHK(hipMalloc(&c->d_tile_pal, 1024));
        HIPCHK(hipMalloc(&c->d_colors, 3 * 256));
        HIPCHK(hipMalloc(&c->d_map, c->npx));
        HIPCHK(hipMalloc(&c->d_pack, c->npx * 8));
        HIPCHK(hipMalloc(&c->d_packT, c->npx * 8));
        HIPCHK(hipMalloc(&c->d_packC4, c->npx * 8));
        HIPCHK(hipMalloc(&c->d_packR4, c->npx * 8));
        if (c->dither) { HIPCHK(hipMalloc(&c->d_subC4, c->npx)); HIPCHK(hipMalloc(&c->d_subR4, c->npx)); }
        HIPCHK(hipMalloc(&c->d_eotf, 256 * 4));
        HIPCHK(hipMalloc(&c->d_lab_eotf, 256 * 4));
        HIPCHK(hipMalloc(&c->d_pal_rgb8, 256 * 4));
        HIPCHK(hipMalloc(&c->d_pal_lin, 256 * 3 * 4));
        HIPCHK(hipMalloc(&c->d_pal_xyb, 256 * 3 * 4));
        HIPCHK(hipMalloc(&c->d_pal_lab, 256 * 3 * 4));
        HIPCHK(hipMalloc(&c->d_lin0, c->npx * 3 * 4));
        HIPCHK(hipMalloc(&c->d_img1, c->src_floats * 4));
        HIPCHK(hipMalloc(&c->d_img1T, c->src_floats * 4));
        HIPCHK(hipMalloc(&c->d_mu1, c->src_floats * 4));
        HIPCHK(hipMalloc(&c->d_sd1, c->src_floats * 4));
        HIPCHK(hipMalloc(&c->d_a1, c->src_floats * 4));
        HIPCHK(hipMalloc(&c->d_a1R4, c->src_floats * 4));
        HIPCHK(hipMalloc(&c->d_r1, c->src_floats * 8));
        HIPCHK(hipMalloc(&c->d_r1R4, c->src_floats * 8));
        HIPCHK(hipMalloc(&c->d_img1C4, c->src_floats * 4));
        HIPCHK(hipMalloc(&c->d_mu1R4, c->src_floats * 4));
        HIPCHK(hipMalloc(&c->d_sd1R4, c->src_floats * 4));
        if (c->perceptual) { HIPCHK(hipMalloc(&c->d_labpx, c->npx * 3 * 4)); HIPCHK(hipMalloc(&c->d_labpxT, c->npx * 3 * 4)); }
        c->d_target = c->d_orig; c->d_labpx_t = c->d_labpx; c->d_labpxT_t = c->d_labpxT;
        HIPCHK(hipMalloc(&c->d_inc_err, sizeof(double)));
        HIPCHK(hipMalloc(&c->d_scratch_err, sizeof(double)));
        HIPCHK(hipMalloc(&c->d_last, sizeof(StepResult)));
        HIPCHK(hipMalloc(&c->d_dummy_cand, 64));
        HIPCHK(hipMemsetAsync(c->d_dummy_cand, 0, 64, c->stream));
        HIPCHK(hipMemsetAsync(c->d_last, 0, sizeof(StepResult), c->stream));
        HIPCHK(hipMemcpyAsync(c->d_orig, rgba, c->npx * 4, hipMemcpyHostToDevice, c->stream));
        HIPCHK(hipMemsetAsync(c->d_tile_pal, 0, 1024, c->stream));
        HIPCHK(hipMemsetAsync(c->d_colors, 0, 3 * 256, c->stream));
        HIPCHK(hipMemsetAsync(c->d_map, 0, c->npx, c->stream));
        c->h_orig.assign(rgba, rgba + c->npx * 4);
        make_eotf_tables(c->h_eotf, c->h_lab_eotf);
        HIPCHK(hipMemcpyAsync(c->d_eotf, c->h_eotf, sizeof(c->h_eotf), hipMemcpyHostToDevice, c->stream));
        HIPCHK(hipMemcpyAsync(c->d_lab_eotf, c->h_lab_eotf, sizeof(c->h_lab_eotf), hipMemcpyHostToDevice, c->stream));
        HIPCHK(hipStreamSynchronize(c->stream));
        CHECK(ensure_cand_capacity(c, 64));
        if (c->backdrop) {
            unsigned long long sum[3] = {0, 0, 0}, cnt = 0;
            for (size_t px = 0; px < c->npx; px++)
                if (rgba[4 * px + 3] != 0) { sum[0] += rgba[4 * px]; sum[1] += rgba[4 * px + 1]; sum[2] += rgba[4 * px + 2]; cnt++; }
            uint8_t b[3] = {0, 0, 0};
            if (cnt) for (int ch = 0; ch < 3; ch++) b[ch] = (uint8_t)(((sum[ch] + cnt / 2) / cnt) >> 3);
            if (c->nes) { uint8_t raw[3] = {b[0], b[1], b[2]}; host_new_nes_only(raw, c->perceptual, c->h_lab_eotf, b); }
            CHECK(write_backdrop(c, b));
        }
        return SNES_OK;
    };
// ... 4 lines not shown
}

void batch_forget(struct snesimage_batch *b, snesimage_ctx *c);
void group_forget(struct snesimage_group *g, snesimage_ctx *c);
namespace { void window_free(struct snesimage_window *w); void tile_free(snesimage_ctx *c); void char_free(snesimage_ctx *c); void level_free(snesimage_ctx *c); void guide_free(struct snesimage_guidework *&w); }
void snesimage_destroy(snesimage_ctx *c) {
    if (!c) return;
    (void)hipSetDevice(c->device);
    if (c->tile) { if (c->stream) (void)hipStreamSynchronize(c->stream); tile_free(c); }
    if (c->chr) { if (c->stream) (void)hipStreamSynchronize(c->stream); char_free(c); }
    if (c->lvl) { if (c->stream) (void)hipStreamSynchronize(c->stream); level_free(c); }
    if (c->guide) { if (c->stream) (void)hipStreamSynchronize(c->stream); guide_free(c->guide); }
    if (c->win) { if (c->stream) (void)hipStreamSynchronize(c->stream); window_free(c->win); c->win = nullptr; }
    if (c->owner) batch_forget(c->owner, c);
    if (c->group) group_forget(c->group, c);
    if (c->ev_own) (void)hipEventDestroy(c->ev_own);
    if (c->stream) (void)hipStreamSynchronize(c->stream);
    (void)drain_timing(c);
    dfree(c->d_packC4); dfree(c->d_packR4); dfree(c->d_subC4); dfree(c->d_subR4); dfree(c->d_mapsC4); dfree(c->d_mapsR4); dfree(c->d_img1C4); dfree(c->d_mu1R4); dfree(c->d_sd1R4); dfree(c->d_r1); dfree(c->d_r1R4); dfree(c->d_a1); dfree(c->d_a1R4);
    dfree(c->d_orig); dfree(c->d_tile_pal); dfree(c->d_colors); dfree(c->d_map); dfree(c->d_pack); dfree(c->d_packT); dfree(c->d_eotf); dfree(c->d_lab_eotf);
    dfree(c->d_pal_rgb8); dfree(c->d_pal_lin); dfree(c->d_pal_xyb); dfree(c->d_pal_lab); dfree(c->d_lin0); dfree(c->d_img1); dfree(c->d_img1T); dfree(c->d_mu1); dfree(c->d_sd1);
    dfree(c->d_bestmaps_all); dfree(c->d_bestrecs_all); dfree(c->d_skip); dfree(c->d_rplist); dfree(c->d_rcount); dfree(c->d_rtab); dfree(c->d_rlab); dfree(c->d_tile_cost); dfree(c->d_tile_any); dfree(c->d_tile_moved);
    dfree(c->d_target_own); dfree(c->d_labpx_t_own); dfree(c->d_labpxT_t_own); dfree(c->d_level);
    dfree(c->d_labpx); dfree(c->d_labpxT); dfree(c->d_work); dfree(c->d_cand_tab); dfree(c->d_cand_lab); dfree(c->d_part); dfree(c->d_maps); dfree(c->d_mapsT);
    dfree(c->d_cand); dfree(c->d_cand_sel); dfree(c->d_errs); dfree(c->d_errs_sel); dfree(c->d_inc_err); dfree(c->d_last); dfree(c->d_scratch_err); dfree(c->d_dummy_cand);
    for (auto &L : c->extra) { if (L.stream) (void)hipStreamSynchronize(L.stream); dfree(L.d_mapsC4); dfree(L.d_mapsR4); dfree(L.d_work); dfree(L.d_cand_tab); dfree(L.d_cand_lab); dfree(L.d_part); dfree(L.d_maps); dfree(L.d_mapsT); if (L.done) (void)hipEventDestroy(L.done); if (L.stream) (void)hipStreamDestroy(L.stream); }
    if (c->ev_ready) (void)hipEventDestroy(c->ev_ready);
    { auto &q = c->sp; for (int i = 0; i < 8; i++) if (q.h0_stream[i]) { (void)hipStreamSynchronize(q.h0_stream[i]); (void)hipStreamDestroy(q.h0_stream[i]); (void)hipEventDestroy(q.ev_scan[i]); (void)hipEventDestroy(q.ev_h0[i]); (void)hipEventDestroy(q.ev_hn[i]); (void)hipEventDestroy(q.ev_vn[i]); (void)hipEventDestroy(q.ev_v0[i]); }
      if (q.base_stream) { (void)hipStreamSynchronize(q.base_stream); (void)hipStreamDestroy(q.base_stream); (void)hipEventDestroy(q.ev_base_in); (void)hipEventDestroy(q.ev_base_h); (void)hipEventDestroy(q.ev_base_narrow); (void)hipEventDestroy(q.ev_base_done); } dfree(q.store); dfree(q.cand_tab); dfree(q.ckf); dfree(q.cka); dfree(q.part); dfree(q.meta); dfree(q.items); dfree(q.item_count); dfree(q.plist); dfree(q.order); dfree(q.first); dfree(q.holder); dfree(q.cand_lab); dfree(q.bitmap); dfree(q.ckh);
      dfree(q.dmaps); dfree(q.dmapsC4); dfree(q.bmap); dfree(q.bmapC4); dfree(q.bcand); dfree(q.dpack); dfree(q.ckd);
      dfree(q.rec_lab); dfree(q.ahead.blab); dfree(q.ahead.rec_lab); dfree(q.ahead.bmap); dfree(q.ahead.bmapC4); dfree(q.ahead.bcand); dfree(q.ahead.dpack); dfree(q.ahead.ckd); dfree(q.ahead.btab); dfree(q.ahead.ok); if (q.ahead.ev) (void)hipEventDestroy(q.ahead.ev); }
    kmeans_free(c->km);
    if (c->own_stream) (void)hipStreamDestroy(c->own_stream);
    delete c;
}

int32_t snesimage_set_stream(snesimage_ctx *c, void *s) {
    if (!c) return fail(SNES_ERR_ARG, "null context");
    CHECK(set_device(c));
    HIPCHK(hipStreamSynchronize(c->stream));
    c->stream = s ? (hipStream_t)s : c->own_stream;
    return SNES_OK;
}
int32_t snesimage_sync(snesimage_ctx *c) {
    if (!c) return fail(SNES_ERR_ARG, "null context");
    CHECK(set_device(c));
    HIPCHK(hipStreamSynchronize(c->stream));
    return SNES_OK;
}
int32_t snesimage_set_chunk(snesimage_ctx *c, uint32_t chunk) {
    if (!c || chunk == 0 || chunk > 65535) return fail(SNES_ERR_ARG, "chunk must be in [1,65535]");
    if (c->owner) return fail(SNES_ERR_STATE, "the context is lent to a batch, whose launches are sized for the current chunk: destroy the batch first");
    CHECK(set_device(c));
    HIPCHK(hipStreamSynchronize(c->stream));
    c->chunk = chunk;
    c->sp.cap = 0; c->sp.lanes = 0; c->sp.plist_valid = false;
    return SNES_OK;
}

int32_t snesimage_optimize(snesimage_ctx *c) {
    if (!c) return fail(SNES_ERR_ARG, "null context");
    CHECK(set_device(c));
    CHECK(do_optimize(c));
    HIPCHK(hipStreamSynchronize(c->stream));
    return SNES_OK;
}

int32_t snesimage_error(snesimage_ctx *c, double *out) {
    if (!c || !out) return fail(SNES_ERR_ARG, "null pointer");
    CHECK(set_device(c));
    CHECK(do_error(c, c->d_scratch_err));
    HIPCHK(hipMemcpyAsync(out, c->d_scratch_err, sizeof(double), hipMemcpyDeviceToHost, c->stream));
    HIPCHK(hipStreamSynchronize(c->stream));
    return SNES_OK;
}

int32_t snesimage_score_candidates_device(snesimage_ctx *c, uint32_t palette, uint32_t index, const uint8_t *d_rgb5, uint32_t n, double *d_errors, uint8_t *d_maps_out) {
    CHECK(check_slot(c, palette, index));
    if (!d_rgb5 || !d_errors) return fail(SNES_ERR_ARG, "null pointer");
    if (n == 0) return SNES_OK;
    CHECK(set_device(c));
    SlotScope s(c, palette, index);
    CHECK(prep_for_slot(c, (int)s.sp, (int)s.si));
    CHECK(score_list(c, d_rgb5, n, d_errors, 1, 0, (int)s.sp, (int)s.si, d_maps_out));
    return SNES_OK;
}

int32_t snesimage_score_candidates(snesimage_ctx *c, uint32_t palette, uint32_t index, const uint8_t *rgb5, uint32_t n, double *errors) {
    CHECK(check_slot(c, palette, index));
    if (!rgb5 || !errors) return fail(SNES_ERR_ARG, "null pointer");
    if (n == 0) return SNES_OK;
    CHECK(set_device(c));
    CHECK(ensure_cand_capacity(c, n));
    HIPCHK(hipMemcpyAsync(c->d_cand_sel, rgb5, 3 * (size_t)n, hipMemcpyHostToDevice, c->stream));
    CHECK(snesimage_score_candidates_device(c, palette, index, c->d_cand_sel, n, c->d_errs_sel, nullptr));
    HIPCHK(hipMemcpyAsync(errors, c->d_errs_sel, sizeof(double) * n, hipMemcpyDeviceToHost, c->stream));
    HIPCHK(hipStreamSynchronize(c->stream));
    return SNES_OK;
}

int32_t snesimage_remap_candidates_device(snesimage_ctx *c, uint32_t palette, uint32_t index, const uint8_t *d_rgb5, uint32_t n, uint8_t *d_maps_out) {
    CHECK(check_slot(c, palette, index));
    if (!d_rgb5 || !d_maps_out) return fail(SNES_ERR_ARG, "null pointer");
    if (n == 0) return SNES_OK;
    CHECK(set_device(c));
    const uint32_t chunk = n < c->chunk ? n : c->chunk;
    CHECK(alloc_workspace(c, 1));
    if (c->rtab_cap < chunk) {
        HIPCHK(hipStreamSynchronize(c->stream));
        c->rtab_cap = 0; dfree(c->d_rtab); dfree(c->d_rlab);
        HIPCHK(dmalloc(&c->d_rtab, sizeof(float) * 8 * (size_t)chunk)); HIPCHK(dmalloc(&c->d_rlab, sizeof(float) * 3 * (size_t)chunk));
        c->rtab_cap = chunk;
    }
    CHECK(ensure_tables(c));
    if (c->perceptual) CHECK(ensure_source(c));
    SlotScope s(c, palette, index);
    index = s.si;
    CHECK(prep_for_slot(c, (int)s.sp, (int)s.si));
    const uint32_t slot_ci = c->tied_call ? (kTiedSlot | (c->sub_size << 8) | s.si) : s.sp * c->sub_size + s.si;
    for (uint32_t c0 = 0; c0 < n; c0 += chunk) {
        const uint32_t nc = (n - c0 < chunk) ? (n - c0) : chunk;
        const uint8_t *rgb5 = d_rgb5 + 3 * (size_t)c0;
        uint8_t *maps = d_maps_out + (size_t)c0 * c->npx;
        hipLaunchKernelGGL(k_candidate_tables, dim3((nc + 63) / 64), dim3(64), 0, c->stream, rgb5, (int)nc, c->d_eotf, c->d_rtab);
        if (c->perceptual) hipLaunchKernelGGL(k_candidate_lab, dim3((nc + 63) / 64), dim3(64), 0, c->stream, c->d_rtab, (int)nc, c->d_lab_eotf, c->d_rlab);
        if (c->dither) {
            hipLaunchKernelGGL(k_candidate_slot, dim3((nc + 63) / 64), dim3(64), 0, c->stream, c->d_rtab, (int)nc, slot_ci);
            DitherParams Dp{};
            Dp.orig = c->d_orig; Dp.tile_pal = c->d_tile_pal; Dp.pal_rgb8 = c->d_pal_rgb8; Dp.pal_lab = c->d_pal_lab; Dp.cand_tab = c->d_rtab; Dp.cand_lab = c->d_rlab;
            Dp.lab_eotf = c->d_lab_eotf; Dp.maps = maps; Dp.mapsC4 = nullptr;
            Dp.W = (int)c->W; Dp.H = (int)c->H; Dp.sub_size = (int)c->sub_size; Dp.ncol = c->ncol; Dp.slot_ci = slot_ci; Dp.perceptual = c->perceptual ? 1 : 0;
            launch_dither(c, Dp, nc);
        } else {
            MapsParams M{}; M.pack = c->d_pack; M.cand_tab = c->d_rtab; M.cand_lab = c->d_rlab; M.labpx = c->d_labpx_t; M.maps = maps;
            M.npx = (int)c->npx; M.ncol = c->ncol; M.sub_size = (int)c->sub_size; M.si = (int)index; M.ncand = (int)nc; M.perceptual = c->perceptual ? 1 : 0;
            const dim3 grid((unsigned)((c->npx / 4 + 255) / 256), (nc + kRemapCands - 1) / kRemapCands);
            if (c->perceptual) {
                if (!c->d_rplist) { HIPCHK(hipMalloc(&c->d_rplist, sizeof(uint4) * c->npx)); HIPCHK(hipMalloc(&c->d_rcount, sizeof(int))); }
                if (c0 == 0) {
                    HIPCHK(hipMemsetAsync(c->d_rcount, 0, sizeof(int), c->stream));
                    hipLaunchKernelGGL(k_build_plist, dim3((unsigned)((c->npx + 255) / 256)), dim3(256), 0, c->stream, c->d_pack, (int)c->npx, c->d_rplist, c->d_rcount);
                }
                hipLaunchKernelGGL(k_remap_fill4, grid, dim3(256), 0, c->stream, M);
                hipLaunchKernelGGL(k_remap_won_lab, dim3(nc), dim3(256), 0, c->stream, M, (const uint4 *)c->d_rplist, (const int *)c->d_rcount);
            } else hipLaunchKernelGGL((k_remap4<false>), grid, dim3(256), 0, c->stream, M);
        }
    }
    HIPCHK(hipGetLastError());
    return SNES_OK;
}

int32_t snesimage_step_async(snesimage_ctx *c, uint32_t method, uint32_t palette, uint32_t index, uint32_t channel, uint64_t seed, uint64_t step_id, uint32_t n_random) {
    CHECK(check_slot(c, palette, index));
    if (method > 2 || channel > 2) return fail(SNES_ERR_ARG, "bad method or channel");
    CHECK(set_device(c));
    const uint32_t n = method_count(method, n_random);
    CHECK(ensure_cand_capacity(c, n));
    if (method != SNES_METHOD_NES) CHECK(ensure_incumbent(c));
    SlotScope s(c, palette, index);
    CHECK(gen_candidates(c, method, s.sp, s.si, channel, seed, step_id, n));
    CHECK(prep_for_slot(c, (int)s.sp, (int)s.si));
    CHECK(score_list(c, c->d_cand, n, c->d_errs, 1, 0, (int)s.sp, (int)s.si, nullptr));
    CHECK(commit(c, c->d_errs, n, method, s.sp, s.si));
    return SNES_OK;
}

int32_t snesimage_last_step(snesimage_ctx *c, double *best_error, uint8_t *best_rgb5, int32_t *best_k) {
    if (!c) return fail(SNES_ERR_ARG, "null context");
    CHECK(set_device(c));
    StepResult r;
    HIPCHK(hipMemcpyAsync(&r, c->d_last, sizeof(r), hipMemcpyDeviceToHost, c->stream));
    HIPCHK(hipStreamSynchronize(c->stream));
    if (best_error) *best_error = r.error;
    if (best_rgb5) { best_rgb5[0] = r.rgb5[0]; best_rgb5[1] = r.rgb5[1]; best_rgb5[2] = r.rgb5[2]; }
    if (best_k) *best_k = r.best_k;
    return SNES_OK;
}

int32_t snesimage_step(snesimage_ctx *c, uint32_t method, uint32_t palette, uint32_t index, uint32_t channel, uint64_t seed, uint64_t step_id, uint32_t n_random, double *best_error,
                       uint8_t *best_rgb5) {
    CHECK(snesimage_step_async(c, method, palette, index, channel, seed, step_id, n_random));
    return snesimage_last_step(c, best_error, best_rgb5, nullptr);
}

int32_t snesimage_step_begin(snesimage_ctx *c, uint32_t method, uint32_t palette, uint32_t index, uint32_t channel, uint64_t seed, uint64_t step_id, uint32_t n_total, uint32_t shard_rank,
                             uint32_t shard_count, double *d_errors) {
    CHECK(check_slot(c, palette, index));
    if (method > 2 || channel > 2 || shard_count == 0 || shard_rank >= shard_count || !d_errors) return fail(SNES_ERR_ARG, "bad step_begin arguments");
    CHECK(set_device(c));
    const uint32_t n = method_count(method, n_total);
    CHECK(ensure_cand_capacity(c, n));
    if (method != SNES_METHOD_NES) CHECK(ensure_incumbent(c));
    SlotScope s(c, palette, index);
    CHECK(gen_candidates(c, method, s.sp, s.si, channel, seed, step_id, n, shard_rank, shard_count, d_errors));
    const uint32_t n_own = (n > shard_rank) ? (n - shard_rank + shard_count - 1) / shard_count : 0;
    if (n_own) {
        CHECK(prep_for_slot(c, (int)s.sp, (int)s.si));
        CHECK(score_list(c, c->d_cand_sel, n_own, d_errors, (int)shard_count, (int)shard_rank, (int)s.sp, (int)s.si, nullptr));
    }
    if (!n_own) c->best_valid = false;
    c->pend = true; c->pend_n = n; c->pend_sp = palette; c->pend_si = index; c->pend_method = method;
    return SNES_OK;
}

int32_t snesimage_step_commit(snesimage_ctx *c, const double *d_errors) {
    if (!c || !d_errors) return fail(SNES_ERR_ARG, "null pointer");
    if (!c->pend) return fail(SNES_ERR_STATE, "step_commit without step_begin");
    CHECK(set_device(c));
    c->pend = false;
    SlotScope s(c, c->pend_sp, c->pend_si);
    return commit(c, d_errors, c->pend_n, c->pend_method, s.sp, s.si);
}

int32_t snesimage_get_tile_palettes(snesimage_ctx *c, uint8_t *out) {
    if (!c || !out) return fail(SNES_ERR_ARG, "null pointer");
    CHECK(set_device(c));
    HIPCHK(hipMemcpyAsync(out, c->d_tile_pal, 1024, hipMemcpyDeviceToHost, c->stream));
    HIPCHK(hipStreamSynchronize(c->stream));
    return SNES_OK;
}
int32_t snesimage_set_tile_palettes(snesimage_ctx *c, const uint8_t *in) {
    if (!c || !in) return fail(SNES_ERR_ARG, "null pointer");
    for (int i = 0; i < 1024; i++) if (in[i] >= c->sub_count) return fail(SNES_ERR_ARG, "tile palette index out of range");
    if (blocked(c)) {
        const int b = untied_block(in, c->H, c->pb_w, c->pb_h);
        if (b >= 0) return fail(SNES_ERR_ARG, "tile_palettes is not constant over block " + std::to_string(b) + " of the context's " + std::to_string(c->pb_w) + " x " + std::to_string(c->pb_h) +
                                              " palette blocks (snesimage_set_palette_blocks)");
    }
    CHECK(set_device(c));
    CHECK(ensure_map(c));
    HIPCHK(hipMemcpyAsync(c->d_tile_pal, in, 1024, hipMemcpyHostToDevice, c->stream));
    HIPCHK(hipStreamSynchronize(c->stream));
    c->pack_valid = false; c->inc_valid = false; c->map_synced = false; c->epoch++; c->epoch_by_commit = false;
    return SNES_OK;
}
int32_t snesimage_get_palette_rgb5(snesimage_ctx *c, uint8_t *out) {
    if (!c || !out) return fail(SNES_ERR_ARG, "null pointer");
    CHECK(set_device(c));
    if (c->backdrop) {
        std::vector<uint8_t> all(3 * (size_t)c->ncol);
        CHECK(read_colors(c, all.data()));
        for (uint32_t p = 0; p < c->sub_count; p++) memcpy(out + 3 * (size_t)p * c->user_size, &all[3 * (size_t)p * c->sub_size], 3 * (size_t)c->user_size);
        return SNES_OK;
    }
    HIPCHK(hipMemcpyAsync(out, c->d_colors, 3 * (size_t)c->ncol, hipMemcpyDeviceToHost, c->stream));
    HIPCHK(hipStreamSynchronize(c->stream));
    return SNES_OK;
}
int32_t snesimage_get_backdrop_rgb5(snesimage_ctx *c, uint8_t *out) {
    if (!c || !out) return fail(SNES_ERR_ARG, "null pointer");
    if (!c->backdrop) return fail(SNES_ERR_ARG, "the context was created without SNES_BACKDROP");
    CHECK(set_device(c));
    HIPCHK(hipMemcpyAsync(out, c->d_colors + 3 * (size_t)c->user_size, 3, hipMemcpyDeviceToHost, c->stream));
    HIPCHK(hipStreamSynchronize(c->stream));
    return SNES_OK;
}
int32_t snesimage_set_backdrop_rgb5(snesimage_ctx *c, const uint8_t *in) {
    if (!c || !in) return fail(SNES_ERR_ARG, "null pointer");
    if (!c->backdrop) return fail(SNES_ERR_ARG, "the context was created without SNES_BACKDROP");
    if (in[0] > 31 || in[1] > 31 || in[2] > 31) return fail(SNES_ERR_ARG, "backdrop channels are 5-bit values");
    CHECK(set_device(c));
    return write_backdrop(c, in);
}
int32_t snesimage_set_palette_rgb5(snesimage_ctx *c, const uint8_t *in) {
    if (!c || !in) return fail(SNES_ERR_ARG, "null pointer");
    CHECK(set_device(c));
    CHECK(ensure_map(c));
    if (c->backdrop) for (uint32_t p = 0; p < c->sub_count; p++) HIPCHK(hipMemcpyAsync(c->d_colors + 3 * (size_t)p * c->sub_size, in + 3 * (size_t)p * c->user_size, 3 * (size_t)c->user_size, hipMemcpyHostToDevice, c->stream));
    else
    HIPCHK(hipMemcpyAsync(c->d_colors, in, 3 * (size_t)c->ncol, hipMemcpyHostToDevice, c->stream));
    HIPCHK(hipStreamSynchronize(c->stream));
    c->tables_valid = false; c->pack_valid = false; c->inc_valid = false; c->map_synced = false; c->epoch++; c->epoch_by_commit = false;
    return SNES_OK;
}
int32_t snesimage_get_palette_u16(snesimage_ctx *c, uint16_t *out) {
    if (!c || !out) return fail(SNES_ERR_ARG, "null pointer");
    std::vector<uint8_t> raw(3 * (size_t)c->ncol);
    CHECK(snesimage_get_palette_rgb5(c, raw.data()));
    for (int i = 0; i < (int)(c->sub_count * c->user_size); i++) out[i] = rgb5_as_u16(raw[3 * i], raw[3 * i + 1], raw[3 * i + 2]);
    return SNES_OK;
}
// ... 211 lines not shown
```

snesimage_amd/csrc/kernels.hpp:

```cpp
#pragma once
#include "color.hpp"

namespace snes {

constexpr int kMaxScales = SSIM2_NUM_SCALES;
constexpr int kBlurRadius = 5;

SNES_HD long long idx_c4(int x, int y, int H) { return ((long long)(x >> 2) * H + y) * 4 + (x & 3); }
SNES_HD long long idx_r4(int x, int y, int W) { return ((long long)(y >> 2) * W + x) * 4 + (y & 3); }
SNES_HD long long idx_xt4(int x, int y, int H) { return ((((long long)(x >> 6) * (H >> 2)) + (y >> 2)) << 8) + ((x & 63) << 2) + (y & 3); }

template <int NT>
__device__ __forceinline__ void copy_map(uint8_t *__restrict__ dst, const uint8_t *__restrict__ src, int npx) {
    const uint4 *s = reinterpret_cast<const uint4 *>(src);
    uint4 *d = reinterpret_cast<uint4 *>(dst);
    for (int i = threadIdx.x; i < npx / 16; i += NT) d[i] = s[i];
}
template <int NT>
__device__ __forceinline__ void copy_map_sync(uint8_t *__restrict__ dst, const uint8_t *__restrict__ src, int npx) {
    copy_map<NT>(dst, src, npx);
    __syncthreads();
}

struct BlurK {
    float n2[3];
    float d1[3];
};

struct Geom {
    int W, H, nscales;
    int sw[kMaxScales], sh[kMaxScales];
    int th[kMaxScales];
    long long off_xyb[kMaxScales], off_xybT[kMaxScales], off_hout[kMaxScales];
    long long cand_stride;
    long long src_off[kMaxScales];
};

inline unsigned down_grid(const Geom &G) { return (unsigned)((G.W / 32) * ((2 * G.sh[1] + 31) / 32)); }
SNES_HD int down_odd_row(const Geom &G, int s, int y) { return 2 * y + 1 < G.th[s - 1] ? 2 * y + 1 : 2 * y; }

__device__ __constant__ double kSsim2Weight[108] = SSIM2_WEIGHTS;

constexpr int kSumAll = 0x3f, kSumSsim = 0x03, kSumEdge = 0x3c;
struct SumMaskTable { unsigned char m[kMaxScales + 1][3][kMaxScales]; };
constexpr double kSsim2WeightHost[108] = SSIM2_WEIGHTS;
constexpr SumMaskTable make_sum_masks() {
    SumMaskTable t{};
    const int acc_of[6] = {0, 2, 4, 1, 3, 5};
    for (int ns = 1; ns <= kMaxScales; ns++)
        for (int ch = 0; ch < 3; ch++)
            for (int s = 0; s < ns; s++) {
                int m = 0;
                for (int e = 0; e < 6; e++) if (kSsim2WeightHost[(ch * ns + s) * 6 + e] != 0.0) m |= 1 << acc_of[e];
                t.m[ns][ch][s] = (unsigned char)m;
            }
    return t;
}
constexpr SumMaskTable kSumMasksHost = make_sum_masks();
__device__ __constant__ SumMaskTable kSumMasks = make_sum_masks();
constexpr int kSumClasses = 10;
struct SumClassTable { unsigned char m[kSumClasses]; };
constexpr SumClassTable make_sum_classes() {
    SumClassTable t{};
    int n = 0;
    for (int ch = 0; ch < 3; ch++)
        for (int s = 0; s < 3 && s < kMaxScales; s++) {
            const unsigned char m = kSumMasksHost.m[kMaxScales][ch][s];
            bool seen = false;
            for (int i = 0; i < n; i++) seen = seen || t.m[i] == m;
            if (!seen) t.m[n++] = m;
        }
    for (; n < kSumClasses; n++) t.m[n] = (unsigned char)kSumAll;
    return t;
}
constexpr SumClassTable kSumClassesHost = make_sum_classes();
__device__ __constant__ SumClassTable kSumClassTab = make_sum_classes();
constexpr bool sum_class_is_first(int i) { for (int j = 0; j < i; j++) if (kSumClassesHost.m[j] == kSumClassesHost.m[i]) return false; return true; }
__device__ __forceinline__ int sum_class(const int need) {
    int best = kSumClasses - 1, bits = 7;
    for (int i = 0; i < kSumClasses; i++) {
        const int m = kSumClassTab.m[i];
        if ((m & need) == need && __builtin_popcount(m) < bits) { best = i; bits = __builtin_popcount(m); }
    }
    return best;
}
__device__ __forceinline__ int sum_class_of(const int ns, const int ch, const int s) { return sum_class(kSumMasks.m[ns][ch][s]); }
__device__ __forceinline__ bool sum_class_has_ssim(const int ns, const int ch, const int s) { return (kSumClassTab.m[sum_class_of(ns, ch, s)] & kSumSsim) != 0; }

__global__ void k_palette_tables(const uint8_t *__restrict__ colors , int ncol, const float *__restrict__ eotf ,
                                 uint32_t *__restrict__ pal_rgb8, float *__restrict__ pal_lin, float *__restrict__ pal_xyb) {
    int i = blockIdx.x * blockDim.x + threadIdx.x;
    if (i >= ncol + 2) return;
    uint32_t rgb8 = 0;
    if (i < ncol) rgb8 = rgb5_to_rgb8(colors[3 * i], colors[3 * i + 1], colors[3 * i + 2]);
    float r = eotf[rgb8 & 0xff], g = eotf[(rgb8 >> 8) & 0xff], b = eotf[(rgb8 >> 16) & 0xff];
    float X, Y, B;
    linear_to_positive_xyb(r, g, b, X, Y, B);
    pal_rgb8[i] = rgb8;
    pal_lin[3 * i] = r; pal_lin[3 * i + 1] = g; pal_lin[3 * i + 2] = b;
    pal_xyb[3 * i] = X; pal_xyb[3 * i + 1] = Y; pal_xyb[3 * i + 2] = B;
}

__device__ __forceinline__ void candidate_tables_body(const uint8_t *__restrict__ rgb5, int n, const float *__restrict__ eotf, float *__restrict__ cand_tab) {
    int k = blockIdx.x * blockDim.x + threadIdx.x;
    if (k >= n) return;
    uint32_t rgb8 = rgb5_to_rgb8(rgb5[3 * k], rgb5[3 * k + 1], rgb5[3 * k + 2]);
    float r = eotf[rgb8 & 0xff], g = eotf[(rgb8 >> 8) & 0xff], b = eotf[(rgb8 >> 16) & 0xff];
    float X, Y, B;
    linear_to_positive_xyb(r, g, b, X, Y, B);
    float *o = cand_tab + 8 * (size_t)k;
    o[0] = r; o[1] = g; o[2] = b; o[3] = X; o[4] = Y; o[5] = B; o[6] = __uint_as_float(rgb8); o[7] = 0.0f;
}

constexpr int kDedupColours = 32768;
constexpr int kNoHolder = 0x7f7f7f7f;
__device__ __forceinline__ int dedup_key(uint32_t rgb8) {
    const uint32_t r = (rgb8 >> 3) & 31u, g = (rgb8 >> 11) & 31u, b = (rgb8 >> 19) & 31u;
    return rgb5_to_rgb8(r, g, b) == (rgb8 & 0x00ffffffu) ? (int)(r | (g << 5) | (b << 10)) : -1;
}
__device__ __forceinline__ void candidate_tables_mark_body(const uint8_t *__restrict__ rgb5, int n, const float *__restrict__ eotf, float *__restrict__ cand_tab, int *__restrict__ holder, int list0) {
    candidate_tables_body(rgb5, n, eotf, cand_tab);
    const int k = blockIdx.x * blockDim.x + threadIdx.x;
    if (k >= n) return;
    const int key = dedup_key(rgb5_to_rgb8(rgb5[3 * k], rgb5[3 * k + 1], rgb5[3 * k + 2]));
    if (key >= 0) atomicMin(&holder[key], list0 + k);
}
__device__ __forceinline__ bool dedup_is_duplicate(const int *__restrict__ holder, uint32_t rgb8, int idx) {
    const int key = dedup_key(rgb8);
    return key >= 0 && holder[key] != idx;
}
__device__ __forceinline__ void dedup_copy_body(const uint8_t *__restrict__ rgb5, int n, int *__restrict__ holder, double *__restrict__ errors, int err_stride, int err_offset) {
    for (int j = threadIdx.x; j < n; j += blockDim.x) {
        const int key = dedup_key(rgb5_to_rgb8(rgb5[3 * j], rgb5[3 * j + 1], rgb5[3 * j + 2]));
        if (key < 0) continue;
        const int h = holder[key];
        if (h != j && (unsigned)h < (unsigned)n) errors[(size_t)err_offset + (size_t)j * err_stride] = errors[(size_t)err_offset + (size_t)h * err_stride];
    }
    __syncthreads();
    for (int j = threadIdx.x; j < n; j += blockDim.x) {
        const int key = dedup_key(rgb5_to_rgb8(rgb5[3 * j], rgb5[3 * j + 1], rgb5[3 * j + 2]));
        if (key >= 0) holder[key] = kNoHolder;
    }
}

constexpr uint32_t kTiedSlot = 0x7d000000u;
__device__ __forceinline__ bool slot_hit(uint32_t ci, uint32_t slot_ci, uint32_t ncol) {
    if ((slot_ci >> 24) != (kTiedSlot >> 24)) return ci == slot_ci;
    return ci < ncol && ci % ((slot_ci >> 8) & 0xffu) == (slot_ci & 0xffu);
}

struct PrepParams {
    const uint8_t *orig; const uint8_t *tile_pal; const uint32_t *pal_rgb8; uint8_t *map;
    unsigned long long *pack, *packT, *packC4, *packR4;
    uint8_t *subC4, *subR4;
    const float *labpx; const float *pal_lab;
    int W, H, sub_size, ncol, mode, sp, si, perceptual;
    int *zero; int nzero;
};

__device__ __forceinline__ void prep_body(const PrepParams &P) {
    if (P.zero && blockIdx.x == 0 && (int)threadIdx.x < P.nzero) P.zero[threadIdx.x] = 0;
    __shared__ uint32_t s_rgb8[256];
    __shared__ float s_lab[256 * 3];
    for (int i = threadIdx.x; i < P.ncol; i += blockDim.x) {
        s_rgb8[i] = P.pal_rgb8[i];
        if (P.perceptual) { s_lab[3 * i] = P.pal_lab[3 * i]; s_lab[3 * i + 1] = P.pal_lab[3 * i + 1]; s_lab[3 * i + 2] = P.pal_lab[3 * i + 2]; }
    }
    __syncthreads();
    int px = blockIdx.x * blockDim.x + threadIdx.x;
    if (px >= P.W * P.H) return;
    int x = px % P.W, y = px / P.W;
    uint32_t o = reinterpret_cast<const uint32_t *>(P.orig)[px];
    uint32_t rgb = o & 0x00ffffffu;
    bool opaque = (o >> 24) != 0;
    int sub = P.tile_pal[(x >> 3) + (y >> 3) * (P.W >> 3)];
    int base = sub * P.sub_size;
    uint32_t ci, thr = 0;
    if (!opaque) {
        ci = (uint32_t)P.ncol + 1u;
        if (P.mode == 0) P.map[px] = 0;
    } else if (P.mode == 1) {
        ci = (uint32_t)(base + P.map[px]);
    } else {
        bool excl = (P.mode == 2 && sub == P.sp) || P.mode == 3;
        int best = -1;
        if (!P.perceptual) {
            uint32_t bk = 0xffffffffu;
            for (int j = 0; j < P.sub_size; j++) {
                if (excl && j == P.si) continue;
                uint32_t k = red_mean_key(s_rgb8[base + j], rgb);
                if (best < 0 || k < bk) { bk = k; best = j; }
            }
            if (excl) thr = (best < 0) ? 0xffffffffu : bk + (P.si < best ? 1u : 0u);
        } else {
// ... 526 lines not shown
        __syncthreads();
        for (int stride = W >> 1; stride > 0; stride >>= 1) {
            if (x < stride) {
#pragma unroll
                for (int k = 0; k < 6; k++) red[t][k] += red[t + stride][k];
            }
            __syncthreads();
        }
        if (x == 0 && active) {
            double *o = P.part + (((size_t)cand * G.nscales + s) * 3 + ch) * 6;
#pragma unroll
            for (int k = 0; k < 6; k++) o[k] = red[t][k];
        }
    }
}

__device__ __forceinline__ void final_score_body(const double *__restrict__ part, int ncand, const Geom &G, double *__restrict__ errors, int err_stride, int err_offset, int *__restrict__ zero, int nzero) {
    int c = blockIdx.x * blockDim.x + threadIdx.x;
    if (zero && c < nzero) zero[c] = 0;
    if (c >= ncand) return;
    double ssim = 0.0;
    int i = 0;
    for (int ch = 0; ch < 3; ch++)
        for (int s = 0; s < G.nscales; s++) {
            const double *p = part + (((size_t)c * G.nscales + s) * 3 + ch) * 6;
            const double opp = 1.0 / (double)((size_t)G.sw[s] * G.th[s]);
            double avg_ssim[2] = {opp * p[0], sqrt(sqrt(opp * p[1]))};
            double avg_edge[4] = {opp * p[2], sqrt(sqrt(opp * p[3])), opp * p[4], sqrt(sqrt(opp * p[5]))};
            for (int n = 0; n < 2; n++) {
                ssim = fma(kSsim2Weight[i], fabs(avg_ssim[n]), ssim); i++;
                ssim = fma(kSsim2Weight[i], fabs(avg_edge[n]), ssim); i++;
                ssim = fma(kSsim2Weight[i], fabs(avg_edge[n + 2]), ssim); i++;
            }
        }
    ssim *= SSIM2_SCORE_SCALE;
    ssim = fma(SSIM2_SCORE_C3 * ssim * ssim, ssim, fma(SSIM2_SCORE_C1, ssim, SSIM2_SCORE_C2 * ssim * ssim));
    if (ssim > 0.0) ssim = fma(pow(ssim, SSIM2_SCORE_EXP), SSIM2_SCORE_GAIN, SSIM2_SCORE_MAX);
    else ssim = SSIM2_SCORE_MAX;
    errors[(size_t)err_offset + (size_t)c * err_stride] = 100.0 - ssim;
}

__device__ __forceinline__ double readlane_f64(double v, int l) {
    const int lo = __builtin_amdgcn_readlane(__double2loint(v), l), hi = __builtin_amdgcn_readlane(__double2hiint(v), l);
    return __hiloint2double(hi, lo);
}
__device__ __forceinline__ void final_score_wave_body(const double *__restrict__ part, int ncand, const Geom &G, double *__restrict__ errors, int err_stride, int err_offset, int *__restrict__ zero, int nzero) {
    const int gt = blockIdx.x * blockDim.x + threadIdx.x;
    if (zero && gt < nzero) zero[gt] = 0;
    const int lane = threadIdx.x & 63, c = __builtin_amdgcn_readfirstlane(gt >> 6);
    if (c >= ncand) return;
    const int ns = G.nscales, npair = 3 * ns;
    double term[6] = {0.0, 0.0, 0.0, 0.0, 0.0, 0.0};
    if (lane < npair) {
        const int ch = lane / ns, s = lane - ch * ns;
        const double *p = part + (((size_t)c * ns + s) * 3 + ch) * 6;
        const double opp = 1.0 / (double)((size_t)G.sw[s] * G.th[s]);
        term[0] = opp * p[0]; term[1] = opp * p[2]; term[2] = opp * p[4];
        term[3] = sqrt(sqrt(opp * p[1])); term[4] = sqrt(sqrt(opp * p[3])); term[5] = sqrt(sqrt(opp * p[5]));
    }
    double ssim = 0.0;
    int i = 0;
    for (int l = 0; l < npair; l++) {
#pragma unroll
        for (int t = 0; t < 6; t++) { ssim = fma(kSsim2Weight[i], fabs(readlane_f64(term[t], l)), ssim); i++; }
    }
    if (lane != 0) return;
    ssim *= SSIM2_SCORE_SCALE;
    ssim = fma(SSIM2_SCORE_C3 * ssim * ssim, ssim, fma(SSIM2_SCORE_C1, ssim, SSIM2_SCORE_C2 * ssim * ssim));
    if (ssim > 0.0) ssim = fma(pow(ssim, SSIM2_SCORE_EXP), SSIM2_SCORE_GAIN, SSIM2_SCORE_MAX);
    else ssim = SSIM2_SCORE_MAX;
    errors[(size_t)err_offset + (size_t)c * err_stride] = 100.0 - ssim;
}

__global__ void k_candidate_tables(const uint8_t *__restrict__ rgb5, int n, const float *__restrict__ eotf, float *__restrict__ cand_tab) { candidate_tables_body(rgb5, n, eotf, cand_tab); }
__global__ void k_candidate_tables_mark(const uint8_t *__restrict__ rgb5, int n, const float *__restrict__ eotf, float *__restrict__ cand_tab, int *__restrict__ holder, int list0) { candidate_tables_mark_body(rgb5, n, eotf, cand_tab, holder, list0); }
__global__ __launch_bounds__(1024) void k_dedup_copy(const uint8_t *__restrict__ rgb5, int n, int *__restrict__ holder, double *__restrict__ errors, int err_stride, int err_offset) { dedup_copy_body(rgb5, n, holder, errors, err_stride, err_offset); }
__global__ __launch_bounds__(256) void k_prep(PrepParams P) { prep_body(P); }
__global__ void k_final_score(const double *__restrict__ part, int ncand, Geom G, double *__restrict__ errors, int err_stride, int err_offset, int *__restrict__ zero = nullptr, int nzero = 0) {
    final_score_body(part, ncand, G, errors, err_stride, err_offset, zero, nzero);
}
__global__ __launch_bounds__(256) void k_final_score_wave(const double *__restrict__ part, int ncand, Geom G, double *__restrict__ errors, int err_stride, int err_offset, int *__restrict__ zero = nullptr, int nzero = 0) {
    final_score_wave_body(part, ncand, G, errors, err_stride, err_offset, zero, nzero);
}

}
```

snesimage_amd/csrc/kernels_opt.hpp:

```cpp
#pragma once
#include "kernels.hpp"

namespace snes {

__global__ void k_palette_lab(const uint32_t *__restrict__ pal_rgb8, int ncol, const float *__restrict__ lab_eotf, float *__restrict__ pal_lab) {
    int i = blockIdx.x * blockDim.x + threadIdx.x;
    if (i >= ncol) return;
    uint32_t c = pal_rgb8[i];
    Lab l = linear_to_lab(lab_eotf[c & 0xff], lab_eotf[(c >> 8) & 0xff], lab_eotf[(c >> 16) & 0xff]);
    pal_lab[3 * i] = l.l; pal_lab[3 * i + 1] = l.a; pal_lab[3 * i + 2] = l.b;
}
__device__ __forceinline__ void candidate_lab_body(const float *__restrict__ cand_tab, int n, const float *__restrict__ lab_eotf, float *__restrict__ cand_lab) {
    int k = blockIdx.x * blockDim.x + threadIdx.x;
    if (k >= n) return;
    uint32_t c = __float_as_uint(cand_tab[8 * (size_t)k + 6]);
    Lab l = linear_to_lab(lab_eotf[c & 0xff], lab_eotf[(c >> 8) & 0xff], lab_eotf[(c >> 16) & 0xff]);
    cand_lab[3 * k] = l.l; cand_lab[3 * k + 1] = l.a; cand_lab[3 * k + 2] = l.b;
}
__global__ void k_candidate_lab(const float *__restrict__ cand_tab, int n, const float *__restrict__ lab_eotf, float *__restrict__ cand_lab) { candidate_lab_body(cand_tab, n, lab_eotf, cand_lab); }
__global__ void k_candidate_slot(float *__restrict__ cand_tab, int n, uint32_t slot_ci) {
    int k = blockIdx.x * blockDim.x + threadIdx.x;
    if (k < n) cand_tab[8 * (size_t)k + 7] = __uint_as_float(slot_ci);
}
__global__ __launch_bounds__(256) void k_pixel_lab(const uint8_t *__restrict__ orig, const float *__restrict__ lab_eotf, int W, int H, float *__restrict__ labpx, float *__restrict__ labpxT) {
// ... 571 lines not shown
                }
                const uint32_t kc = dither_group_min<1>(&own, t1, tw, tg) >> 3;
                const bool mine = kc < thr;
                const uint32_t nc = mine ? own.w : s_ent[base + best].w;
                const uint8_t m = opaque ? (uint8_t)(mine ? slot_si : best) : 0;
                macc = (macc >> 8) | ((uint32_t)m << 24);
                if ((x & 3) == 3) {
                    const size_t px = (size_t)y * W + x;
                    map4[px >> 2] = macc;
                    if (mapC4) mapC4[idx_c4(x & ~3, y, H) >> 2] = macc;
                }
#pragma unroll
                for (int c = 0; c < 3; c++) {
                    const double d = target[c] - (double)((nc >> (8 * c)) & 0xff);
                    left[c] = (opaque ? d : e[c]) * mult;
                }
                if (j == 63) { wrap[x][0] = left[0]; wrap[x][1] = left[1]; wrap[x][2] = left[2]; }
            }
        }
    }
}

struct BestRec { double err; int k; int pad; };
struct StepResult { double error; int32_t best_k; uint8_t rgb5[3]; uint8_t changed; };
__global__ void k_reset_best(BestRec *__restrict__ recs, int n) {
    if ((int)threadIdx.x < n) { recs[threadIdx.x].err = __longlong_as_double(0x7ff0000000000000ll); recs[threadIdx.x].k = -1; }
}
__global__ __launch_bounds__(1024) void k_keep_best(const double *__restrict__ errors, int stride, int off, int nc, const uint8_t *__restrict__ maps, int npx, BestRec *__restrict__ rec,
                                                   uint8_t *__restrict__ bestmap) {
    __shared__ double s_e[1024];
    __shared__ int s_i[1024];
    const int t = threadIdx.x;
    double be = __longlong_as_double(0x7ff0000000000000ll); int bi = 0x7fffffff;
    for (int i = t; i < nc; i += 1024) { const double e = errors[off + (size_t)i * stride]; if (e < be) { be = e; bi = i; } }
    s_e[t] = be; s_i[t] = bi;
    __syncthreads();
    for (int st = 512; st > 0; st >>= 1) {
        if (t < st) {
            const double e2 = s_e[t + st]; const int i2 = s_i[t + st];
            if (e2 < s_e[t] || (e2 == s_e[t] && i2 < s_i[t])) { s_e[t] = e2; s_i[t] = i2; }
        }
        __syncthreads();
    }
    be = s_e[0]; bi = s_i[0];
    if (bi == 0x7fffffff || !(be < rec->err)) return;
    const uint4 *src = reinterpret_cast<const uint4 *>(maps + (size_t)bi * npx);
    uint4 *dst = reinterpret_cast<uint4 *>(bestmap);
    for (int i = t; i < npx / 16; i += 1024) dst[i] = src[i];
    __syncthreads();
    if (t == 0) { rec->err = be; rec->k = off + bi * stride; }
}
__global__ void k_ahead_ok(const StepResult *__restrict__ last, int *__restrict__ ok) { *ok = (last && last->changed) ? 0 : 1; }
__global__ __launch_bounds__(1024) void k_take_best_map(const StepResult *__restrict__ last, const BestRec *__restrict__ recs, int nrec, const uint8_t *__restrict__ bestmaps, int npx,
                                                       int map_synced, uint8_t *__restrict__ map, int *__restrict__ skip) {
    const int best_k = last->best_k;
    int lane = -1;
    if (best_k >= 0) for (int r = 0; r < nrec; r++) if (recs[r].k == best_k) lane = r;
    if (lane >= 0) {
        const uint4 *src = reinterpret_cast<const uint4 *>(bestmaps + (size_t)lane * npx);
        uint4 *dst = reinterpret_cast<uint4 *>(map);
        for (int i = threadIdx.x; i < npx / 16; i += 1024) dst[i] = src[i];
    }
    if (threadIdx.x == 0) *skip = (lane >= 0 || (best_k < 0 && map_synced)) ? 1 : 0;
}

__global__ __launch_bounds__(256) void k_maps_relayout(const uint8_t *__restrict__ maps, int W, int H, uint32_t *__restrict__ r4, uint32_t *__restrict__ mT) {
    __shared__ uint8_t s_b[4][256 + 4];
    const int q = blockIdx.x, t = threadIdx.x;
    const size_t cb = (size_t)blockIdx.y * W * H;
    const uint32_t w4 = reinterpret_cast<const uint32_t *>(maps + cb + (size_t)(4 * q + (t >> 6)) * W)[t & 63];
    *reinterpret_cast<uint32_t *>(&s_b[t >> 6][4 * (t & 63)]) = w4;
    __syncthreads();
    const uint32_t w = (uint32_t)s_b[0][t] | ((uint32_t)s_b[1][t] << 8) | ((uint32_t)s_b[2][t] << 16) | ((uint32_t)s_b[3][t] << 24);
    r4[(cb >> 2) + (size_t)q * W + t] = w;
    if (mT) mT[(cb >> 2) + (size_t)t * (H >> 2) + q] = w;
}


__device__ __forceinline__ unsigned long long dev_mix64(unsigned long long z) {
    z = (z ^ (z >> 30)) * 0xBF58476D1CE4E5B9ull;
    z = (z ^ (z >> 27)) * 0x94D049BB133111EBull;
    return z ^ (z >> 31);
}
__device__ __forceinline__ void gen_candidates_body(int method, int n, unsigned long long key, const uint8_t *__restrict__ colors, int slot, int channel, uint8_t *__restrict__ cand,
                                                    int rank, int count, uint8_t *__restrict__ sel, double *__restrict__ errors) {
    int k = blockIdx.x * blockDim.x + threadIdx.x;
    if (k >= n) return;
    uint8_t c[3];
    if (method == 0) {
        unsigned long long z = dev_mix64(key + ((unsigned long long)k + 1ull) * 0x9E3779B97F4A7C15ull);
        c[0] = (uint8_t)(z & 31); c[1] = (uint8_t)((z >> 5) & 31); c[2] = (uint8_t)((z >> 10) & 31);
    } else if (method == 1) {
        c[0] = colors[3 * slot]; c[1] = colors[3 * slot + 1]; c[2] = colors[3 * slot + 2];
        c[channel] = (uint8_t)k;
    } else {
        if (k < (int)kNesColorCount) { c[0] = kNesTableDev[k][0]; c[1] = kNesTableDev[k][1]; c[2] = kNesTableDev[k][2]; } else { c[0] = c[1] = c[2] = 0; }
    }
    cand[3 * k] = c[0]; cand[3 * k + 1] = c[1]; cand[3 * k + 2] = c[2];
    if (sel) {
        errors[k] = __longlong_as_double(0x7ff0000000000000ll);
        if (k % count == rank) { const int j = k / count; sel[3 * j] = c[0]; sel[3 * j + 1] = c[1]; sel[3 * j + 2] = c[2]; }
    }
}

__global__ void k_shard_select(const uint8_t *__restrict__ cand, int n, int rank, int count, uint8_t *__restrict__ sel, double *__restrict__ errors) {
    int k = blockIdx.x * blockDim.x + threadIdx.x;
    if (k >= n) return;
    errors[k] = __longlong_as_double(0x7ff0000000000000ll);
    if (k % count == rank) { int j = k / count; sel[3 * j] = cand[3 * k]; sel[3 * j + 1] = cand[3 * k + 1]; sel[3 * j + 2] = cand[3 * k + 2]; }
}

struct PaletteTables { const float *eotf, *lab_eotf; uint32_t *rgb8; float *lin, *xyb, *lab; };
__device__ __forceinline__ void commit_apply(const double best, const int best_k, const uint8_t *__restrict__ cand, uint8_t *__restrict__ colors, int slot, double *__restrict__ inc_err,
                                             StepResult *__restrict__ last, const PaletteTables &T) {
    uint8_t c[3] = {colors[3 * slot], colors[3 * slot + 1], colors[3 * slot + 2]};
    uint8_t changed = 0;
    if (best_k >= 0) {
        uint8_t nc[3] = {cand[3 * best_k], cand[3 * best_k + 1], cand[3 * best_k + 2]};
        changed = (nc[0] != c[0] || nc[1] != c[1] || nc[2] != c[2]) ? 1 : 0;
        c[0] = nc[0]; c[1] = nc[1]; c[2] = nc[2];
        colors[3 * slot] = c[0]; colors[3 * slot + 1] = c[1]; colors[3 * slot + 2] = c[2];
        if (T.rgb8) {
            const uint32_t rgb8 = rgb5_to_rgb8(c[0], c[1], c[2]);
            const float r = T.eotf[rgb8 & 0xff], g = T.eotf[(rgb8 >> 8) & 0xff], b = T.eotf[(rgb8 >> 16) & 0xff];
            float X, Y, B;
            linear_to_positive_xyb(r, g, b, X, Y, B);
            T.rgb8[slot] = rgb8;
            T.lin[3 * slot] = r; T.lin[3 * slot + 1] = g; T.lin[3 * slot + 2] = b;
            T.xyb[3 * slot] = X; T.xyb[3 * slot + 1] = Y; T.xyb[3 * slot + 2] = B;
            if (T.lab) {
                const Lab l = linear_to_lab(T.lab_eotf[rgb8 & 0xff], T.lab_eotf[(rgb8 >> 8) & 0xff], T.lab_eotf[(rgb8 >> 16) & 0xff]);
                T.lab[3 * slot] = l.l; T.lab[3 * slot + 1] = l.a; T.lab[3 * slot + 2] = l.b;
            }
        }
        if (best < 1.7976931348623157e308) *inc_err = best;
    }
    last->error = *inc_err; last->best_k = best_k; last->rgb5[0] = c[0]; last->rgb5[1] = c[1]; last->rgb5[2] = c[2]; last->changed = changed;
}

__device__ __forceinline__ void commit_decide(const double min_e, const int min_k, const uint8_t *__restrict__ cand, uint8_t *__restrict__ colors, int slot, int nes, double *__restrict__ inc_err,
                                              StepResult *__restrict__ last, const PaletteTables &T) {
    const double start = nes ? 1.7976931348623157e308 : *inc_err;
    double best = start; int best_k = -1;
    if (min_k != 0x7fffffff && min_e < start) { best = min_e; best_k = min_k; }
    if (nes && best_k < 0) best_k = 0;
    commit_apply(best, best_k, cand, colors, slot, inc_err, last, T);
}

__device__ __forceinline__ void tied_spread(uint8_t *__restrict__ colors, int slot, int count, int stride, const PaletteTables &T) {
    for (int p = 1; p < count; p++) {
        const int d = slot + p * stride;
        for (int ch = 0; ch < 3; ch++) colors[3 * d + ch] = colors[3 * slot + ch];
        if (!T.rgb8) continue;
        T.rgb8[d] = T.rgb8[slot];
        for (int ch = 0; ch < 3; ch++) { T.lin[3 * d + ch] = T.lin[3 * slot + ch]; T.xyb[3 * d + ch] = T.xyb[3 * slot + ch]; if (T.lab) T.lab[3 * d + ch] = T.lab[3 * slot + ch]; }
    }
}

__device__ __forceinline__ void commit_body(const double *__restrict__ errors, int n, const uint8_t *__restrict__ cand, uint8_t *__restrict__ colors, int slot, int nes, double *__restrict__ inc_err,
                                            StepResult *__restrict__ last, const PaletteTables &T) {
    __shared__ double s_e[256];
    __shared__ int s_k[256];
    const int t = threadIdx.x;
    double be = __longlong_as_double(0x7ff0000000000000ll); int bk = 0x7fffffff;
    for (int k = t; k < n; k += 256) { const double e = errors[k]; if (e < be) { be = e; bk = k; } }
    s_e[t] = be; s_k[t] = bk;
    __syncthreads();
    for (int st = 128; st > 0; st >>= 1) {
        if (t < st) {
            const double e2 = s_e[t + st]; const int k2 = s_k[t + st];
            if (e2 < s_e[t] || (e2 == s_e[t] && k2 < s_k[t])) { s_e[t] = e2; s_k[t] = k2; }
        }
        __syncthreads();
    }
    if (t != 0) return;
    commit_decide(s_e[0], s_k[0], cand, colors, slot, nes, inc_err, last, T);
}

__global__ void k_debug_math(int op, const float *__restrict__ x, const float *__restrict__ y, int n, const float *__restrict__ lab_eotf, float *__restrict__ out) {
    int i = blockIdx.x * blockDim.x + threadIdx.x;
    if (i >= n) return;
    switch (op) {
    case 0: out[i] = d_sinf(x[i]); break;
    case 1: out[i] = d_cosf(x[i]); break;
    case 2: out[i] = d_expf_neg(x[i]); break;
// ... 197 lines not shown
```

snesimage_amd/csrc/kernels_sparse.hpp:

```cpp
#pragma once
#include "kernels.hpp"

namespace snes {

constexpr int kGroupsTotal = 126;

struct CandMeta {
    int ngroups[kMaxScales];
    int xmin;
    int won;
    unsigned char glist[kGroupsTotal + 2];
    short gslot[kGroupsTotal];
    unsigned char gcb[kGroupsTotal];
};
__device__ __forceinline__ int item_k(unsigned int it) { return (int)(it >> 14); }
__device__ __forceinline__ int item_g(unsigned int it) { return (int)((it >> 8) & 63u); }
__device__ __forceinline__ int item_j(unsigned int it) { return (int)((it >> 2) & 63u); }
__device__ __forceinline__ int item_ch(unsigned int it) { return (int)(it & 3u); }
constexpr int kColBuckets = 4;
constexpr int kItemLists = kMaxScales * kColBuckets;

struct SparseGeom {
    long long off_lin[kMaxScales], off_xybC[kMaxScales], off_xybR[kMaxScales], off_hout[kMaxScales];
    long long cand_stride;
// ... 1135 lines not shown
__global__ __launch_bounds__(256) void k_remap_fill4(MapsParams P) {
    const int q = blockIdx.x * 256 + threadIdx.x;
    if (q * 4 >= P.npx) return;
    const uint4 a = reinterpret_cast<const uint4 *>(P.pack)[2 * (size_t)q], b = reinterpret_cast<const uint4 *>(P.pack)[2 * (size_t)q + 1];
    const uint32_t lo[4] = {a.x, a.z, b.x, b.z};
    uint32_t word = 0;
#pragma unroll
    for (int i = 0; i < 4; i++) {
        const uint32_t ci0 = lo[i] >> 24;
        word |= (ci0 == (uint32_t)P.ncol ? (uint32_t)P.si : (ci0 == (uint32_t)P.ncol + 1u ? 0u : ci0 % (uint32_t)P.sub_size)) << (8 * i);
    }
    const int c0 = blockIdx.y * kRemapCands;
    for (int cc = 0; cc < kRemapCands && c0 + cc < P.ncand; cc++) reinterpret_cast<uint32_t *>(P.maps + (size_t)(c0 + cc) * P.npx)[q] = word;
}
__global__ __launch_bounds__(256) void k_remap_won_lab(MapsParams P, const uint4 *__restrict__ plist, const int *__restrict__ plist_count) {
    __shared__ uint32_t s_queue[4][128];
    const int lane = threadIdx.x & 63, w = threadIdx.x >> 6;
    const int cand = (int)blockIdx.x;
    if (cand >= P.ncand) return;
    Lab cl; cl.l = P.cand_lab[3 * cand]; cl.a = P.cand_lab[3 * cand + 1]; cl.b = P.cand_lab[3 * cand + 2];
    const float cch = sqrtf(cl.a * cl.a + cl.b * cl.b);
    uint8_t *map = P.maps + (size_t)cand * P.npx;
    const int n = *plist_count;
    auto full_test = [&](int i) {
        const uint4 e = plist[i];
        Lab t; t.l = P.labpx[3 * (size_t)e.x]; t.a = P.labpx[3 * (size_t)e.x + 1]; t.b = P.labpx[3 * (size_t)e.x + 2];
        const float d = ciede2000(cl, t), bd = __uint_as_float(e.z & 0x7fffffffu);
        if ((d < bd) || ((e.z & 0x80000000u) && d == bd)) map[e.x] = (uint8_t)P.si;
    };
    uint32_t *q = s_queue[w];
    int queued = 0;
    for (int i0 = 64 * w; i0 < n; i0 += 256) {
        const int i = i0 + lane;
        bool maybe = false;
        if (i < n) {
            const uint4 e = plist[i];
            if (e.z == 0xffffffffu) map[e.x] = (uint8_t)P.si;
            else {
                Lab t; t.l = P.labpx[3 * (size_t)e.x]; t.a = P.labpx[3 * (size_t)e.x + 1]; t.b = P.labpx[3 * (size_t)e.x + 2];
                const float bd = __uint_as_float(e.z & 0x7fffffffu);
                maybe = !ciede2000_cannot_beat(cl, t, bd) && !ciede2000_cannot_beat_ab(cl, cch, t, bd);
            }
        }
        const unsigned long long mm = __ballot(maybe);
        if (maybe) q[queued + __popcll(mm & ((1ull << lane) - 1ull))] = (uint32_t)i;
        queued += __popcll(mm);
        if (queued >= 64) {
            full_test((int)q[lane]);
            queued -= 64;
            if (lane < queued) { const uint32_t v = q[64 + lane]; q[lane] = v; }
        }
    }
    if (lane < queued) full_test((int)q[lane]);
}

__device__ __forceinline__ void sparse_order_body(const SparseParams &P, int *__restrict__ order) {
    __shared__ int s_cnt[66];
    const int t = threadIdx.x, H4 = P.G.sh[0] >> 2;
    const int *first = P.first + P.k0;
    if (t < 66) s_cnt[t] = 0;
    __syncthreads();
    for (int i = t; i < P.ncand; i += blockDim.x) atomicAdd(&s_cnt[first[i]], 1);
    __syncthreads();
    if (t == 0) { int run = 0; for (int b = 0; b <= H4; b++) { const int c = s_cnt[b]; s_cnt[b] = run; run += c; } }
    __syncthreads();
    for (int i = t; i < P.ncand; i += blockDim.x) order[atomicAdd(&s_cnt[first[i]], 1)] = i;
}
__global__ __launch_bounds__(1024) void k_sparse_order(SparseParams P, int *__restrict__ order) { sparse_order_body(P, order); }

__global__ __launch_bounds__(256) void k_sparse_scan_lab(SparseParams P) { sparse_scan_lab_body(P); }
__global__ __launch_bounds__(1024) void k_sparse_scan(SparseParams P) { sparse_scan_body<1>(P); }
__global__ __launch_bounds__(1024) void k_sparse_scan4(SparseParams P) { sparse_scan_body<4>(P); }
__global__ __launch_bounds__(1024) void k_dither_first(SparseParams P) { dither_first_body(P); }
__global__ __launch_bounds__(256) void k_dither_first_lab(SparseParams P) { dither_first_lab_body(P); }
__global__ __launch_bounds__(1024) void k_dither_diff(SparseParams P) { dither_diff_body(P); }
__global__ __launch_bounds__(256) void k_sparse_down(SparseParams P, int only_scale) { sparse_down_body(P, only_scale, (int)blockIdx.x); }
__global__ __launch_bounds__(256) void k_sparse_down1(SparseParams P) { sparse_down1_body(P, (int)blockIdx.x, (int)gridDim.x); }
__global__ __launch_bounds__(256) void k_sparse_down_tiles(SparseParams P) { sparse_down_tiles_body<SNES_DOWN_TILES_U>(P, (int)blockIdx.x, (int)gridDim.x); }
__global__ __launch_bounds__(256) void k_base_down(SparseParams P) { base_down_body(P); }
__global__ __launch_bounds__(64) void k_sparse_h(SparseParams P) { sparse_h_body(P); }
__global__ __launch_bounds__(256, 1) void k_sparse_v_base(SparseParams P) { sparse_v_base_body(P); }
__global__ __launch_bounds__(256) void k_build_plist(const unsigned long long *__restrict__ pack, int npx, uint4 *__restrict__ plist, int *__restrict__ count) { build_plist_body(pack, npx, plist, count); }

}
```

snesimage_amd/csrc/window_host.inc:

```

struct WindowPolicy {
    double calls = 0.0, accepts = 0.0;
    uint32_t next(uint32_t used, uint32_t acc, uint32_t lo, uint32_t hi, uint32_t ranks, uint32_t taken, double weight = 1.0) {
        calls = 0.85 * calls + used; accepts = 0.85 * accepts + acc;
        const double p = (accepts + 0.5) / (calls + 8.0);
        double best = -1.0; uint32_t best_k = lo;
        for (uint32_t k = lo; k <= hi; k = k < 4 ? 2 * k : k + (k < 32 * ranks ? 4 : 8) * ranks) {
            const double through = (1.0 - std::pow(1.0 - p, (double)k)) / p, rate = through / (15.0 + weight * (double)k / ranks);
            if (rate > best) { best = rate; best_k = k; }
        }
        if (!acc && used == taken) { const uint32_t twice = 2 * taken > hi ? hi : 2 * taken; if (twice > best_k) best_k = twice; }
        return best_k;
    }
};

struct WindowRec {
    unsigned char *h_blob = nullptr, *d_blob = nullptr;
    snes::BatchArgs *h_args = nullptr, *d_args = nullptr;
    snes::WindowSlot *h_slots = nullptr, *d_slots = nullptr;
    snes::WindowResult *h_res = nullptr, *d_res = nullptr;
    snes::StepResult *h_log = nullptr, *d_log = nullptr;
    uint8_t *d_cand = nullptr; double *d_errs = nullptr;
    hipEvent_t ev[7] = {nullptr, nullptr, nullptr, nullptr, nullptr, nullptr, nullptr}, args = nullptr, done = nullptr;
    uint32_t K = 0, stride = 0; bool logged = false;
    int seq = 0, base = 0;
};

struct snesimage_window {
    std::vector<snesimage_ctx *> child[2];
    hipEvent_t ev_ready = nullptr;
    uint32_t cap = 0;
    static constexpr int kRing = 3;
    WindowRec rec[kRing];
    int *d_dead = nullptr; int seq_next = 1;
    hipStream_t aux = nullptr; bool use_aux = true;
    bool side_borrowed = false;
    hipStream_t side = nullptr; bool use_side = true;
    uint32_t depth = 2;
    uint32_t adapt = 8;
    WindowPolicy policy;
    uint32_t clean_streak = 0;
    uint32_t g_adapt = 8; WindowPolicy g_policy; uint32_t g_clean_streak = 0;
    snes::GuidePixel *g_list = nullptr; unsigned long long *g_tab = nullptr;
};

namespace {

constexpr uint32_t kWindowMin = 8;
constexpr uint32_t kMemberCand = 96;
uint32_t window_max() {
    static uint32_t v = [] { uint32_t m = 64; if (const char *e = getenv("SNES_WINDOW_MAX")) { int x = atoi(e); if (x >= 1 && x <= snes::kMaxWindow) m = (uint32_t)x; } return m; }();
    return v;
}

void ctx_schedule_next(const snesimage_ctx *c, int nes, uint32_t *palette, uint32_t *index, uint32_t *channel, uint32_t *step, uint32_t *method) {
    if (c->backdrop) snesimage_schedule_next_backdrop(c->sub_count, c->user_size, nes, palette, index, channel, step, method);
    else snesimage_schedule_next(c->sub_count, c->sub_size, nes, palette, index, channel, step, method);
}
bool window_capable(const snesimage_ctx *c) { return c->sp.enabled && !c->owner && !(c->dither && c->sub_size == 1); }

struct WindowGen {
    uint32_t n;
    void (*next)(const snesimage_ctx *c, uint32_t *palette, uint32_t *index);
    int32_t (*generate)(snesimage_ctx *c, WindowRec &r, uint32_t K, uint32_t n, double *d_errors);
};

void window_release_child(snesimage_ctx *k) {
    k->d_orig = nullptr; k->d_tile_pal = nullptr; k->d_colors = nullptr; k->d_map = nullptr; k->d_eotf = nullptr; k->d_lab_eotf = nullptr;
    k->d_pal_rgb8 = nullptr; k->d_pal_lin = nullptr; k->d_pal_xyb = nullptr; k->d_pal_lab = nullptr; k->d_lin0 = nullptr; k->d_img1 = nullptr; k->d_img1T = nullptr; k->d_mu1 = nullptr; k->d_sd1 = nullptr;
    k->d_a1 = nullptr; k->d_a1R4 = nullptr; k->d_r1 = nullptr; k->d_r1R4 = nullptr; k->d_img1C4 = nullptr; k->d_mu1R4 = nullptr; k->d_sd1R4 = nullptr; k->d_labpx = nullptr; k->d_labpxT = nullptr; k->d_target = nullptr; k->d_labpx_t = nullptr; k->d_labpxT_t = nullptr;
    k->d_inc_err = nullptr; k->d_last = nullptr; k->d_scratch_err = nullptr; k->d_dummy_cand = nullptr;
    if (k->pack_borrowed) { k->d_pack = nullptr; k->d_packC4 = nullptr; k->d_packR4 = nullptr; k->d_subC4 = nullptr; k->d_subR4 = nullptr; }
    k->stream = nullptr; k->own_stream = nullptr;
    snesimage_destroy(k);
}

int32_t window_make_child(snesimage_ctx *c, snesimage_ctx **out) {
    std::unique_ptr<snesimage_ctx, void (*)(snesimage_ctx *)> k(new snesimage_ctx(), window_release_child);
    k->device = c->device; k->W = c->W; k->H = c->H; k->sub_count = c->sub_count; k->sub_size = c->sub_size; k->user_size = c->sub_size; k->flags = c->flags;  k->ncol = c->ncol;
    k->dither_rec = c->dither_rec; k->dither4 = c->dither4; k->dither4_max = c->dither4_max; k->ditherw = c->ditherw; k->sp.ahead.on = false;
    k->dither = c->dither; k->perceptual = c->perceptual; k->nes = c->nes; k->G = c->G; k->K = c->K; k->npx = c->npx; k->src_floats = c->src_floats; k->fast_mask = c->fast_mask;
    k->chunk = kMemberCand; k->nlanes = 1;
    k->sp.enabled = true; k->sp.side = false; k->sp.lpt = c->sp.lpt; k->sp.down1 = c->sp.down1; k->sp.h2q_max = c->sp.h2q_max; k->sp.scan4_max = c->sp.scan4_max; k->sp.vsplit = c->sp.vsplit; k->sp.down_tiles = c->sp.down_tiles; k->sp.tiles_grid = c->sp.tiles_grid; k->sp.h0_min = c->sp.h0_min; k->sp.hgrid = c->sp.hgrid; k->sp.min_n = 1;
    k->sp.weight_mask = c->sp.weight_mask; k->sp.h_planes = c->sp.h_planes; k->sp.v2_pair = c->sp.v2_pair; k->sp.h_forms = c->sp.h_forms; k->sp.debug_poison = c->sp.debug_poison;
    k->d_orig = c->d_orig; k->d_tile_pal = c->d_tile_pal; k->d_colors = c->d_colors; k->d_map = c->d_map; k->d_eotf = c->d_eotf; k->d_lab_eotf = c->d_lab_eotf;
    k->d_pal_rgb8 = c->d_pal_rgb8; k->d_pal_lin = c->d_pal_lin; k->d_pal_xyb = c->d_pal_xyb; k->d_pal_lab = c->d_pal_lab;
    k->d_img1C4 = c->d_img1C4; k->d_mu1R4 = c->d_mu1R4; k->d_sd1R4 = c->d_sd1R4; k->d_a1R4 = c->d_a1R4; k->d_r1R4 = c->d_r1R4; k->d_labpx = c->d_labpx; k->d_labpxT = c->d_labpxT; k->d_target = c->d_target; k->d_labpx_t = c->d_labpx_t; k->d_labpxT_t = c->d_labpxT_t; k->od_n = c->od_n; memcpy(k->od_tab, c->od_tab, sizeof k->od_tab);
    k->d_inc_err = c->d_inc_err; k->d_last = c->d_last;
    k->stream = c->stream;
    k->tables_valid = true; k->src_valid = true;
    if (c->dither) {
        k->pack_borrowed = true;
        k->d_pack = c->d_pack; k->d_packC4 = c->d_packC4; k->d_packR4 = c->d_packR4; k->d_subC4 = c->d_subC4; k->d_subR4 = c->d_subR4;
    } else {
        HIPCHK(dmalloc(&k->d_pack, c->npx * 8));
        HIPCHK(dmalloc(&k->d_packC4, c->npx * 8));
        HIPCHK(dmalloc(&k->d_packR4, c->npx * 8));
    }
    CHECK(sparse_alloc(k.get(), kMemberCand));
    *out = k.release();
    return SNES_OK;
}

size_t window_slots_bytes(uint32_t K) { return (sizeof(snes::WindowSlot) * (size_t)K + 15) & ~(size_t)15; }
size_t window_blob_bytes(uint32_t cap) { return window_slots_bytes(cap) + sizeof(snes::BatchArgs) * (size_t)cap; }
void window_rec_free(WindowRec &r) {
    if (r.h_blob) (void)hipHostFree(r.h_blob); if (r.h_res) (void)hipHostFree(r.h_res); if (r.h_log) (void)hipHostFree(r.h_log);
    r.h_blob = nullptr; r.h_args = nullptr; r.h_slots = nullptr; r.h_res = nullptr; r.h_log = nullptr; r.d_args = nullptr; r.d_slots = nullptr;
    dfree(r.d_blob); dfree(r.d_res); dfree(r.d_log); dfree(r.d_cand); dfree(r.d_errs);
}

void window_free(snesimage_window *w) {
    if (!w) return;
    for (auto &set : w->child) for (auto *k : set) window_release_child(k);
    if (w->ev_ready) (void)hipEventDestroy(w->ev_ready);
    if (w->side) { (void)hipStreamSynchronize(w->side); if (!w->side_borrowed) (void)hipStreamDestroy(w->side); }
    if (w->aux) { (void)hipStreamSynchronize(w->aux); (void)hipStreamDestroy(w->aux); }
    for (auto &r : w->rec) { window_rec_free(r); for (auto &e : r.ev) if (e) (void)hipEventDestroy(e); if (r.done) (void)hipEventDestroy(r.done); if (r.args) (void)hipEventDestroy(r.args); }
    dfree(w->d_dead); dfree(w->g_list); dfree(w->g_tab);
    delete w;
}

int32_t window_reserve(snesimage_ctx *c, uint32_t K, uint32_t own, int set = 0) {
    if (!c->win) {
        c->win = new snesimage_window();
        if (const char *e = getenv("SNES_WINDOW_SIDE")) c->win->use_side = atoi(e) != 0;
        if (const char *e = getenv("SNES_WINDOW_AUX")) c->win->use_aux = atoi(e) != 0;
        if (const char *e = getenv("SNES_WINDOW_DEPTH")) { int v = atoi(e); if (v >= 1) c->win->depth = v > 2 ? 2u : (uint32_t)v; }
    }
    snesimage_window *w = c->win;
    if (!w->d_dead) {
        HIPCHK(dmalloc(&w->d_dead, sizeof(int)));
        HIPCHK(hipMemsetAsync(w->d_dead, 0, sizeof(int), c->stream));
        static const bool borrow = [] { const char *e = getenv("SNES_WINDOW_BORROW"); return !e || atoi(e) != 0; }();
        if (borrow && c->sp.base_stream) { w->side = c->sp.base_stream; w->side_borrowed = true; }
        else HIPCHK(hipStreamCreateWithFlags(&w->side, hipStreamNonBlocking));
        for (auto &r : w->rec) { for (auto &e : r.ev) HIPCHK(hipEventCreateWithFlags(&e, hipEventDisableTiming)); HIPCHK(hipEventCreateWithFlags(&r.done, hipEventDisableTiming)); HIPCHK(hipEventCreateWithFlags(&r.args, hipEventDisableTiming)); }
        HIPCHK(hipEventCreateWithFlags(&w->ev_ready, hipEventDisableTiming));
    }
    if (K > w->cap) {
        HIPCHK(hipStreamSynchronize(c->stream));
        w->cap = 0;
        uint32_t cap = 16; while (cap < K) cap *= 2;
        for (auto &r : w->rec) {
            window_rec_free(r);
            HIPCHK(hipHostMalloc(&r.h_blob, window_blob_bytes(cap)));
            HIPCHK(hipHostMalloc(&r.h_log, sizeof(snes::StepResult) * cap));
            HIPCHK(hipHostMalloc(&r.h_res, sizeof(snes::WindowResult)));
            HIPCHK(dmalloc(&r.d_blob, window_blob_bytes(cap)));
            HIPCHK(dmalloc(&r.d_log, sizeof(snes::StepResult) * cap));
            HIPCHK(dmalloc(&r.d_res, sizeof(snes::WindowResult)));
            HIPCHK(dmalloc(&r.d_cand, 3 * 64 * (size_t)cap));
            HIPCHK(dmalloc(&r.d_errs, sizeof(double) * 64 * (size_t)cap));
        }
        w->cap = cap;
    }
    while (w->child[set].size() < own) {
        snesimage_ctx *k = nullptr;
        CHECK(window_make_child(c, &k));
        w->child[set].push_back(k);
    }
    return SNES_OK;
}

int32_t window_enqueue(snesimage_ctx *c, WindowRec &r, uint32_t n_slots, uint64_t seed, uint64_t first_step_id, uint32_t palette, uint32_t index, uint32_t channel, uint32_t step, uint32_t n_random,
                       uint32_t shard_rank, uint32_t shard_count, double *d_errors, int set = 0, bool ahead = false, const WindowGen *gen = nullptr) {
    snesimage_window *w = c->win;
// ... 221 lines not shown
```

Measured before the change: 3.523 million.

## Fuse per-call head kernels and fold dedup copy into final score tail

Adds a combined head kernel that runs prep, pixel-list build, candidate generation, candidate tables and dedup-holder marking in one launch. It also adds a tail variant of the final score kernel that uses a grid ticket so the last block performs the dedup copy. Both are aimed at per-call launch overhead and the gaps between small kernels at the start and end of each step. In exchange it adds a global atomic ticket and last-block logic, plus a special-case path that only applies to single-group, non-perceptual lists. Profiling scripts that compare the variants are also added.

After: 3.328 million. 5.5% lower.

```diff
diff --git a/profiles/call_ends.py b/profiles/call_ends.py
--- /dev/null
+++ b/profiles/call_ends.py
@@ -0,0 +1,90 @@
+#!/usr/bin/env python3
+import argparse
+import glob
+import json
+import os
+import statistics
+import subprocess
+import sys
+import tempfile
+
+import numpy as np
+
+HERE = os.path.dirname(os.path.dirname(os.path.abspath(__file__)))
+ap = argparse.ArgumentParser()
+ap.add_argument("out")
+ap.add_argument("--parent", required=True)
+ap.add_argument("--rounds", type=int, default=6)
+ap.add_argument("--main", action="store_true")
+ap.add_argument("--outputs", action="store_true")
+ap.add_argument("--limit", type=int, default=240, help="seconds per run")
+args = ap.parse_args()
+
+parent = os.path.abspath(args.parent)
+legs = [("parent", parent, {}), ("new", HERE, {}), ("tail", HERE, {"SNES_CALL_ENDS": "1"}), ("head", HERE, {"SNES_CALL_ENDS": "2"}),
+        ("off", HERE, {"SNES_CALL_ENDS": "0"}), ("parent_b", parent, {})]
+if os.path.exists(args.out):
+    res = json.load(open(args.out))
+else:
+    res = {"what": "python bench.py [args], the legs alternating on one MI355X, one process per run",
+           "legs": {n: {"tree": "parent" if t == parent else "this", "env": e} for n, t, e in legs}, "runs": [], "outputs": {}}
+
+
+def save():
+    json.dump(res, open(args.out, "w"), indent=1)
+
+
+def bench(tree, env, extra):
+    cmd = ["timeout", "-k", "10", str(args.limit), sys.executable, "bench.py"] + extra
+    p = subprocess.run(cmd, cwd=tree, env=dict(os.environ, **env), stdout=subprocess.PIPE, stderr=subprocess.PIPE, text=True)
+    if p.returncode != 0:
+        print(p.stdout[-2000:], p.stderr[-4000:], file=sys.stderr)
+        res["failed"] = {"cmd": cmd, "leg_env": env, "rc": p.returncode}
+        save()
+        sys.exit("run failed with status %d: nothing more is started" % p.returncode)
+    line = [ln for ln in p.stdout.splitlines() if ln.startswith("{")][-1]
+    return json.loads(line)
+
+
+def summary():
+    out = {}
+    for label in sorted({r["invocation"] for r in res["runs"]}):
+        rounds = sorted({r["round"] for r in res["runs"] if r["invocation"] == label})
+        ms = {n: [next((r["ms_per_step"] for r in res["runs"] if r["invocation"] == label and r["round"] == k and r["leg"] == n), None) for k in rounds] for n, _, _ in legs}
+        pa = [v for v in ms["parent"] + ms["parent_b"] if v is not None]
+        e = {"rounds": rounds, "parent_min_max_ms": [min(pa), max(pa)], "parent_spread_percent": 100.0 * (max(pa) - min(pa)) / statistics.median(pa),
+             "parent_b_minus_parent_percent": [100.0 * (b - a) / a for a, b in zip(ms["parent"], ms["parent_b"]) if a and b], "legs": {}}
+        for n, _, _ in legs[1:5]:
+            gain = [100.0 * (a - b) / a for a, b in zip(ms["parent"], ms[n]) if a and b]
+            e["legs"][n] = {"ms_per_step": ms[n], "gain_percent_per_round": gain, "median_gain_percent": statistics.median(gain),
+                            "same_sign_every_round": all(g > 0 for g in gain) or all(g < 0 for g in gain)}
+        out[label] = e
+    return out
+
+
+if args.main:
+    for rnd in range(1, args.rounds + 1):
+        for label, extra in (("default", []), ("s20", ["--gpus", "1", "--steps", "20", "--warmup", "5"])):
+            for name, tree, env in legs:
+                d = bench(tree, env, extra)
+                res["runs"].append({"leg": name, "invocation": label, "args": extra, "env": env, "ms_per_step": d["ms_per_step"], "steps": d.get("steps"),
+                                    "library": d.get("library"), "round": rnd})
+                print("%-8s %-8s %.4f ms" % (label, name, d["ms_per_step"]), flush=True)
+                save()
+    res["summary"] = summary()
+    save()
+    print(json.dumps(res["summary"], indent=1))
+
+if args.outputs:
+    (na, ta, ea), (nb, tb, eb) = legs[0], legs[1]
+    for cfg in ("rgb", "perceptual", "dither"):
+        cargs = [] if cfg == "rgb" else ["--config", cfg]
+        with tempfile.TemporaryDirectory() as tmp:
+            for n, t, e in ((na, ta, ea), (nb, tb, eb)):
+                bench(t, e, cargs + ["--steps", "20", "--warmup", "5", "--dump-outputs", os.path.join(tmp, n)])
+            fa = sorted(os.path.basename(f) for f in glob.glob(os.path.join(tmp, na, "*.npy")))
+            fb = sorted(os.path.basename(f) for f in glob.glob(os.path.join(tmp, nb, "*.npy")))
+            same = {f: bool(np.array_equal(np.load(os.path.join(tmp, na, f)), np.load(os.path.join(tmp, nb, f)))) for f in fa if f in fb}
+            res["outputs"][cfg] = {"arrays": fa, "same_names": fa == fb, "array_equal": same, "all_identical": bool(fa) and fa == fb and all(same.values())}
+            print("outputs %-10s %s" % (cfg, res["outputs"][cfg]), flush=True)
+            save()
diff --git a/profiles/call_ends_gap.py b/profiles/call_ends_gap.py
--- /dev/null
+++ b/profiles/call_ends_gap.py
@@ -0,0 +1,34 @@
+#!/usr/bin/env python3
+import sqlite3
+import statistics
+import sys
+
+db = sqlite3.connect(sys.argv[1])
+skip = int(sys.argv[2]) if len(sys.argv) > 2 else 8
+tabs = [r[0] for r in db.execute("select name from sqlite_master where type in ('table','view')")]
+kd = [t for t in tabs if t.startswith("rocpd_kernel_dispatch")][0]
+ks = [t for t in tabs if t.startswith("rocpd_info_kernel_symbol")][0]
+rows = db.execute(f"select d.start, d.end, s.kernel_name from {kd} d join {ks} s on d.kernel_id = s.id order by d.start").fetchall()
+
+
+def short(name):
+    return name.split("(")[0].replace("_ZN4snes", "").replace("void snes::", "").replace("snes::", "")[:40]
+
+
+finals = [i for i, r in enumerate(rows) if "k_final_score" in r[2]]
+gaps, example = [], None
+for a in finals[skip:]:
+    v_end = max((r[1] for r in rows[max(0, a - 40):a] if "k_sparse_v" in r[2]), default=None)
+    nxt = next((j for j in range(a, min(len(rows), a + 40)) if "k_sparse_down1" in rows[j][2]), None)
+    if v_end is None or nxt is None:
+        continue
+    gaps.append((rows[nxt][0] - v_end) / 1e3)
+    example = (v_end, a, nxt)
+if not gaps:
+    sys.exit("no pair of long calls found")
+print("end of the last V kernel -> start of k_sparse_down1 of the next call, %d calls: median %.1f us, min %.1f, max %.1f" % (
+    len(gaps), statistics.median(gaps), min(gaps), max(gaps)))
+v_end, a, nxt = example
+print("the last of them (us from the end of that V kernel: start, end, duration):")
+for st, en, name in rows[a:nxt + 1]:
+    print("%8.1f %8.1f %7.1f  %s" % ((st - v_end) / 1e3, (en - v_end) / 1e3, (en - st) / 1e3, short(name)))
diff --git a/snesimage_amd/csrc/capi.hip b/snesimage_amd/csrc/capi.hip
--- a/snesimage_amd/csrc/capi.hip
+++ b/snesimage_amd/csrc/capi.hip
@@ -171,6 +171,7 @@
         uint32_t h_forms = 3;
         bool debug_poison = false;
         bool dedup = true; uint32_t dedup_min = 1024; int *holder = nullptr; bool holder_dirty = false;
+        uint32_t call_ends = 3; unsigned int *ticket = nullptr; bool head_done = false; int *plist_spare = nullptr;
         bool enabled = false, side = true; uint32_t min_n = 1; uint32_t cap = 0, lanes = 0;
         SparseGeom S{};
         float *store = nullptr, *cand_tab = nullptr, *cand_lab = nullptr, *ckf = nullptr, *ckh = nullptr; long long zeros_off = 0; uint32_t *bitmap = nullptr; double *cka = nullptr, *part = nullptr;
@@ -330,14 +331,19 @@
     return SNES_OK;
 }
 
-int32_t run_prep(snesimage_ctx *c, int mode, int sp, int si) {
-    if (c->pack_valid && c->pack_mode == mode && ((mode != 2 && mode != 3) || (c->pack_sp == sp && c->pack_si == si))) return SNES_OK;
-    CHECK(ensure_tables(c));
-    if (c->perceptual) CHECK(ensure_source(c));
+bool pack_current(const snesimage_ctx *c, int mode, int sp, int si) { return c->pack_valid && c->pack_mode == mode && ((mode != 2 && mode != 3) || (c->pack_sp == sp && c->pack_si == si)); }
+PrepParams prep_params(const snesimage_ctx *c, int mode, int sp, int si) {
     PrepParams P{};
     P.orig = c->d_target; P.tile_pal = c->d_tile_pal; P.pal_rgb8 = c->d_pal_rgb8; P.map = c->d_map; P.pack = c->d_pack; P.packT = c->d_packT; P.packC4 = c->d_packC4; P.packR4 = c->d_packR4; P.subC4 = c->d_subC4; P.subR4 = c->d_subR4;
     P.labpx = c->d_labpx_t; P.pal_lab = c->d_pal_lab;
     P.W = (int)c->W; P.H = (int)c->H; P.sub_size = (int)c->sub_size; P.ncol = c->ncol; P.mode = mode; P.sp = sp; P.si = si; P.perceptual = c->perceptual ? 1 : 0;
+    return P;
+}
+int32_t run_prep(snesimage_ctx *c, int mode, int sp, int si) {
+    if (pack_current(c, mode, sp, si)) return SNES_OK;
+    CHECK(ensure_tables(c));
+    if (c->perceptual) CHECK(ensure_source(c));
+    PrepParams P = prep_params(c, mode, sp, si);
     c->sp.counters_cleared = false;
     if (mode == 2 && c->sp.plist_count) {
         P.zero = c->sp.plist_count; P.nzero = 1; c->sp.counters_cleared = true;
@@ -471,7 +477,7 @@
     for (auto &L : c->extra) HIPCHK(hipStreamSynchronize(L.stream));
     if (sp.base_stream) HIPCHK(hipStreamSynchronize(sp.base_stream));
     sp.cap = 0; sp.lanes = 0; sp.plist_valid = false;
-    dfree(sp.store); dfree(sp.cand_tab); dfree(sp.ckf); dfree(sp.cka); dfree(sp.part); dfree(sp.meta); dfree(sp.items); dfree(sp.item_count); dfree(sp.plist); sp.plist_count = nullptr;
+    dfree(sp.store); dfree(sp.cand_tab); dfree(sp.ckf); dfree(sp.cka); dfree(sp.part); dfree(sp.meta); dfree(sp.items); dfree(sp.item_count); dfree(sp.plist); sp.plist_count = nullptr; sp.plist_spare = nullptr;
     const Geom &G = c->G;
     SparseGeom &S = sp.S;
     long long off = 0, okf = 0, oka = 0, okh = 0; int go = 0;
@@ -516,9 +522,9 @@
         HIPCHK(hipEventCreateWithFlags(&sp.ev_base_narrow, hipEventDisableTiming));
         HIPCHK(hipEventCreateWithFlags(&sp.ev_base_done, hipEventDisableTiming));
     }
-    HIPCHK(dmalloc(&sp.item_count, sizeof(int) * (kItemLists * (c->nlanes + 1) + 1)));
-    HIPCHK(hipMemsetAsync(sp.item_count, 0, sizeof(int) * (kItemLists * (c->nlanes + 1) + 1), c->stream));
-    sp.plist_count = sp.item_count + (size_t)kItemLists * (c->nlanes + 1);
+    HIPCHK(dmalloc(&sp.item_count, sizeof(int) * (kItemLists * (c->nlanes + 1) + 2)));
+    HIPCHK(hipMemsetAsync(sp.item_count, 0, sizeof(int) * (kItemLists * (c->nlanes + 1) + 2), c->stream));
+    sp.plist_count = sp.item_count + (size_t)kItemLists * (c->nlanes + 1); sp.plist_spare = sp.plist_count + 1;
     sp.counters_cleared = true;
     HIPCHK(dmalloc(&sp.plist, sizeof(uint4) * c->npx));
     if (c->dither) {
@@ -595,7 +601,7 @@
     else hipLaunchKernelGGL(k_sparse_h2_um<false>, d, dim3(64), lds, st, P);
 }
 
-int32_t sparse_base_pass(snesimage_ctx *c, int sp_idx, int si, uint32_t n_cand) {
+int32_t sparse_base_pass(snesimage_ctx *c, int sp_idx, int si, uint32_t n_cand, bool head = false) {
     auto &sp = c->sp;
     const Geom &G = c->G;
     if (!sp.plist_valid) {
@@ -636,7 +642,7 @@
             else hipLaunchKernelGGL((k_dither<false, 0, 1>), dim3(1), dim3(128), 0, c->stream, Dp);
             win_pack = sp.dpack;
         }
-        hipLaunchKernelGGL(k_build_plist, dim3((unsigned)((c->npx + 255) / 256)), dim3(256), 0, c->stream, win_pack, (int)c->npx, sp.plist, sp.plist_count);
+        if (!head) hipLaunchKernelGGL(k_build_plist, dim3((unsigned)((c->npx + 255) / 256)), dim3(256), 0, c->stream, win_pack, (int)c->npx, sp.plist, sp.plist_count);
         SparseParams P = sparse_params(c, c->nlanes);
         P.is_base = 1; P.ncand = 1; P.k0 = P.base;
         hipStream_t bs = sp.side ? sp.base_stream : c->stream;
@@ -686,7 +692,7 @@
     return SNES_OK;
 }
 
-int32_t sparse_score_chunk(snesimage_ctx *c, uint32_t lane, hipStream_t stream, const uint8_t *d_rgb5, uint32_t nc, double *d_errors, int err_stride, int err_offset, int list0 = -1) {
+int32_t sparse_score_chunk(snesimage_ctx *c, uint32_t lane, hipStream_t stream, const uint8_t *d_rgb5, uint32_t nc, double *d_errors, int err_stride, int err_offset, int list0 = -1, bool tail = false, bool head = false) {
     auto &sp = c->sp;
     const Geom &G = c->G;
     SparseParams P = sparse_params(c, lane);
@@ -695,6 +701,7 @@
     if (sp.debug_poison) HIPCHK(hipMemsetAsync(sp.store + (size_t)P.k0 * sp.S.cand_stride, 0xff, sizeof(float) * (size_t)sp.S.cand_stride * nc, stream));
     snesimage_ctx::TimingRec tr{}; tr.n = nc;
     if (c->timing) { for (int i = 0; i < 6; i++) HIPCHK(hipEventCreate(&tr.ev[i])); if (c->timing == 1) HIPCHK(hipEventRecord(tr.ev[0], stream)); }
+    if (head) {} else
     if (list0 >= 0) hipLaunchKernelGGL(k_candidate_tables_mark, dim3((nc + 63) / 64), dim3(64), 0, stream, d_rgb5, (int)nc, c->d_eotf, sp.cand_tab + 8 * (size_t)P.k0, sp.holder, list0);
     else
     hipLaunchKernelGGL(k_candidate_tables, dim3((nc + 63) / 64), dim3(64), 0, stream, d_rgb5, (int)nc, c->d_eotf, sp.cand_tab + 8 * (size_t)P.k0);
@@ -815,6 +822,9 @@
     if (P.s_first < G.nscales) hipLaunchKernelGGL(k_sparse_v, dim3((nc * 3 + 7) / 8, (unsigned)(G.nscales - P.s_first)), dim3(256), 0, stream, P);
     }
     if (v0_aside) HIPCHK(hipStreamWaitEvent(stream, sp.ev_v0[lane], 0));
+    if (tail) hipLaunchKernelGGL(k_final_score_dedup, dim3((nc + 15) / 16), dim3(1024), 0, stream, sp.part + (size_t)P.k0 * G.nscales * 18, (int)nc, G, d_errors, err_stride, err_offset, P.item_count, (int)kItemLists,
+                                 d_rgb5, sp.holder, sp.ticket);
+    else
     hipLaunchKernelGGL(k_final_score_wave, dim3((nc + 3) / 4), dim3(256), 0, stream, sp.part + (size_t)P.k0 * G.nscales * 18, (int)nc, G, d_errors, err_stride, err_offset, P.item_count, (int)kItemLists);
     if (c->dither) {
         uint8_t *bm = lane == 0 ? c->d_bestmap : c->extra[lane - 1].d_bestmap; BestRec *br = lane == 0 ? c->d_bestrec : c->extra[lane - 1].d_bestrec;
@@ -834,11 +844,29 @@
                   std::swap(c->d_bestmap, L->d_bestmap); std::swap(c->d_bestrec, L->d_bestrec); }
 };
 
-int32_t score_list(snesimage_ctx *c, const uint8_t *d_rgb5, uint32_t n, double *d_errors, int err_stride, int err_offset, int sp, int si, uint8_t *d_maps_out) {
+uint32_t list_chunk(const snesimage_ctx *c, uint32_t n) {
     uint32_t chunk = (c->dither || c->perceptual) ? (n + c->nlanes - 1) / c->nlanes : n;
     if (chunk < 64) chunk = 64;
     if (chunk > c->chunk) chunk = c->chunk;
     if (c->tied_call && chunk > 1024) chunk = 1024;
+    return chunk;
+}
+int32_t dedup_prepare(snesimage_ctx *c) {
+    if (!c->sp.holder) { HIPCHK(dmalloc(&c->sp.holder, sizeof(int) * (kDedupColours + 1))); c->sp.ticket = reinterpret_cast<unsigned int *>(c->sp.holder + kDedupColours); c->sp.holder_dirty = true; }
+    if (c->sp.holder_dirty) {
+        HIPCHK(hipStreamSynchronize(c->stream));
+        for (auto &L : c->extra) HIPCHK(hipStreamSynchronize(L.stream));
+        HIPCHK(hipMemsetAsync(c->sp.holder, kNoHolder & 0xff, sizeof(int) * kDedupColours, c->stream));
+        HIPCHK(hipMemsetAsync(c->sp.ticket, 0, sizeof(unsigned int), c->stream));
+    }
+    c->sp.holder_dirty = true;
+    return SNES_OK;
+}
+
+int32_t score_list(snesimage_ctx *c, const uint8_t *d_rgb5, uint32_t n, double *d_errors, int err_stride, int err_offset, int sp, int si, uint8_t *d_maps_out, bool call_ends = false) {
+    const bool head = c->sp.head_done;
+    c->sp.head_done = false;
+    const uint32_t chunk = list_chunk(c, n);
     const bool sparse = c->sp.enabled && !c->tied_call && !d_maps_out && sp >= 0 && n >= c->sp.min_n && c->pack_mode == (c->dither ? 1 : 2) && !(c->dither && c->sub_size == 1);
     const uint32_t nchunks = (n + chunk - 1) / chunk;
     const uint32_t nl = nchunks < c->nlanes ? nchunks : c->nlanes;
@@ -848,20 +876,14 @@
     if (sparse) {
         CHECK(sparse_alloc(c, chunk, nl));
         if (c->dither && (c->sp.base_sp != sp || c->sp.base_si != si)) c->sp.plist_valid = false;
-        CHECK(sparse_base_pass(c, sp, si, n));
+        CHECK(sparse_base_pass(c, sp, si, n, head));
         c->sp.base_sp = sp; c->sp.base_si = si;
     }
+    if (head && !(sparse && nl == 1)) return fail(SNES_ERR_STATE, "internal: the head of a call was launched for a list that does not take the group-sparse path as one launch group");
     if (c->dither) { hipLaunchKernelGGL(k_reset_best, dim3(1), dim3(64), 0, c->stream, c->d_bestrecs_all, (int)c->nlanes); c->best_valid = true; }
     const bool dedup = sparse && !c->dither && c->sp.dedup && n >= c->sp.dedup_min;
-    if (dedup) {
-        if (!c->sp.holder) { HIPCHK(dmalloc(&c->sp.holder, sizeof(int) * kDedupColours)); c->sp.holder_dirty = true; }
-        if (c->sp.holder_dirty) {
-            HIPCHK(hipStreamSynchronize(c->stream));
-            for (auto &L : c->extra) HIPCHK(hipStreamSynchronize(L.stream));
-            HIPCHK(hipMemsetAsync(c->sp.holder, kNoHolder & 0xff, sizeof(int) * kDedupColours, c->stream));
-        }
-        c->sp.holder_dirty = true;
-    }
+    if (dedup && !head) CHECK(dedup_prepare(c));
+    const bool tail = dedup && call_ends && (c->sp.call_ends & 1) && !c->perceptual && nl == 1 && n <= chunk;
     if (nl > 1) {
         HIPCHK(hipEventRecord(c->ev_ready, c->stream));
         for (uint32_t l = 1; l < nl; l++) HIPCHK(hipStreamWaitEvent(c->extra[l - 1].stream, c->ev_ready, 0));
@@ -872,7 +894,7 @@
         const uint32_t lane = i % nl;
         uint8_t *mo = d_maps_out ? d_maps_out + (size_t)c0 * c->npx : nullptr;
         const int eo = err_offset + (int)c0 * err_stride;
-        if (sparse) { CHECK(sparse_score_chunk(c, lane, lane == 0 ? c->stream : c->extra[lane - 1].stream, d_rgb5 + 3 * (size_t)c0, nc, d_errors, err_stride, eo, dedup ? (int)c0 : -1)); continue; }
+        if (sparse) { CHECK(sparse_score_chunk(c, lane, lane == 0 ? c->stream : c->extra[lane - 1].stream, d_rgb5 + 3 * (size_t)c0, nc, d_errors, err_stride, eo, dedup ? (int)c0 : -1, tail, head)); continue; }
         if (lane == 0) CHECK(score_chunk(c, d_rgb5 + 3 * (size_t)c0, nc, d_errors, err_stride, eo, sp, si, mo));
         else { LaneScope ls(c, &c->extra[lane - 1]); CHECK(score_chunk(c, d_rgb5 + 3 * (size_t)c0, nc, d_errors, err_stride, eo, sp, si, mo)); }
     }
@@ -880,6 +902,8 @@
         HIPCHK(hipEventRecord(c->extra[l - 1].done, c->extra[l - 1].stream));
         HIPCHK(hipStreamWaitEvent(c->stream, c->extra[l - 1].done, 0));
     }
+    if (tail) c->sp.holder_dirty = false;
+    else
     if (dedup) {
         hipLaunchKernelGGL(k_dedup_copy, dim3(1), dim3(1024), 0, c->stream, d_rgb5, (int)n, c->sp.holder, d_errors, err_stride, err_offset);
         HIPCHK(hipGetLastError());
@@ -1006,6 +1030,37 @@
     hipLaunchKernelGGL(k_gen_candidates, dim3((n + 63) / 64), dim3(64), 0, c->stream, (int)method, (int)n, key, c->d_colors, (int)(palette * c->sub_size + index), (int)channel, c->d_cand,
                        (int)shard_rank, (int)shard_count, d_errors ? c->d_cand_sel : (uint8_t *)nullptr, d_errors);
     HIPCHK(hipGetLastError());
+    return SNES_OK;
+}
+
+int32_t call_head(snesimage_ctx *c, uint32_t method, uint32_t sp_idx, uint32_t si, uint32_t channel, uint64_t seed, uint64_t step_id, uint32_t n, uint32_t n_list, uint32_t shard_rank = 0,
+                  uint32_t shard_count = 1, double *d_errors = nullptr) {
+    auto &sp = c->sp;
+    const bool fuse = (sp.call_ends & 2) && sp.enabled && !c->dither && !c->perceptual && !c->tied_call && !c->owner && !c->group && n_list >= 1 && n_list >= sp.min_n && n_list <= c->chunk &&
+                      !pack_current(c, 2, (int)sp_idx, (int)si);
+    if (!fuse) {
+        CHECK(gen_candidates(c, method, sp_idx, si, channel, seed, step_id, n, shard_rank, shard_count, d_errors));
+        if (n_list) CHECK(prep_for_slot(c, (int)sp_idx, (int)si));
+        return SNES_OK;
+    }
+    CHECK(alloc_workspace(c, 1, 1));
+    CHECK(ensure_tables(c));
+    CHECK(ensure_source(c));
+    CHECK(sparse_alloc(c, list_chunk(c, n_list), 1));
+    const bool dedup = sp.dedup && n_list >= sp.dedup_min;
+    if (dedup) CHECK(dedup_prepare(c));
+    std::swap(sp.plist_count, sp.plist_spare);
+    CallHeadParams H{};
+    H.prep = prep_params(c, 2, (int)sp_idx, (int)si);
+    H.pixel_blocks = (int)((c->npx + 255) / 256); H.plist = sp.plist; H.plist_count = sp.plist_count; H.count_spare = sp.plist_spare;
+    H.method = (int)method; H.n = (int)n; H.key = mix64(seed ^ (step_id * 0x9E3779B97F4A7C15ull) ^ 0xD1B54A32D192ED03ull); H.colors = c->d_colors; H.slot = (int)(sp_idx * c->sub_size + si); H.channel = (int)channel;
+    H.cand = c->d_cand; H.rank = (int)shard_rank; H.count = (int)shard_count; H.sel = d_errors ? c->d_cand_sel : nullptr; H.errors = d_errors;
+    H.eotf = c->d_eotf; H.cand_tab = sp.cand_tab; H.holder = dedup ? sp.holder : nullptr;
+    hipLaunchKernelGGL(k_call_head, dim3((unsigned)H.pixel_blocks + (n + 255) / 256), dim3(256), 0, c->stream, H);
+    HIPCHK(hipGetLastError());
+    c->pack_valid = true; c->pack_mode = 2; c->pack_sp = (int)sp_idx; c->pack_si = (int)si;
+    sp.counters_cleared = true; sp.plist_valid = false;
+    sp.head_done = true;
     return SNES_OK;
 }
 
@@ -1123,6 +1178,7 @@
     if (const char *e = getenv("SNES_WEIGHT_MASK")) c->sp.weight_mask = atoi(e) != 0;
     if (const char *e = getenv("SNES_H_PLANES")) c->sp.h_planes = atoi(e) != 0;
     if (const char *e = getenv("SNES_V2_PAIR")) c->sp.v2_pair = atoi(e) != 0;
+    if (const char *e = getenv("SNES_CALL_ENDS")) { int v = atoi(e); if (v >= 0 && v <= 3) c->sp.call_ends = (uint32_t)v; }
     if (const char *e = getenv("SNES_H_FORMS")) { int v = atoi(e); if (v >= 0 && v <= 7) c->sp.h_forms = (uint32_t)v; }
     if (const char *e = getenv("SNES_DEBUG_POISON")) c->sp.debug_poison = atoi(e) != 0;
     if (const char *e = getenv("SNES_DEDUP_MIN")) { int v = atoi(e); if (v >= 1) c->sp.dedup_min = (uint32_t)v; }
@@ -1293,7 +1349,7 @@
     CHECK(set_device(c));
     SlotScope s(c, palette, index);
     CHECK(prep_for_slot(c, (int)s.sp, (int)s.si));
-    CHECK(score_list(c, d_rgb5, n, d_errors, 1, 0, (int)s.sp, (int)s.si, d_maps_out));
+    CHECK(score_list(c, d_rgb5, n, d_errors, 1, 0, (int)s.sp, (int)s.si, d_maps_out, true));
     return SNES_OK;
 }
 
@@ -1369,9 +1425,8 @@
     CHECK(ensure_cand_capacity(c, n));
     if (method != SNES_METHOD_NES) CHECK(ensure_incumbent(c));
     SlotScope s(c, palette, index);
-    CHECK(gen_candidates(c, method, s.sp, s.si, channel, seed, step_id, n));
-    CHECK(prep_for_slot(c, (int)s.sp, (int)s.si));
-    CHECK(score_list(c, c->d_cand, n, c->d_errs, 1, 0, (int)s.sp, (int)s.si, nullptr));
+    CHECK(call_head(c, method, s.sp, s.si, channel, seed, step_id, n, n));
+    CHECK(score_list(c, c->d_cand, n, c->d_errs, 1, 0, (int)s.sp, (int)s.si, nullptr, true));
     CHECK(commit(c, c->d_errs, n, method, s.sp, s.si));
     return SNES_OK;
 }
@@ -1403,11 +1458,10 @@
     CHECK(ensure_cand_capacity(c, n));
     if (method != SNES_METHOD_NES) CHECK(ensure_incumbent(c));
     SlotScope s(c, palette, index);
-    CHECK(gen_candidates(c, method, s.sp, s.si, channel, seed, step_id, n, shard_rank, shard_count, d_errors));
     const uint32_t n_own = (n > shard_rank) ? (n - shard_rank + shard_count - 1) / shard_count : 0;
+    CHECK(call_head(c, method, s.sp, s.si, channel, seed, step_id, n, n_own, shard_rank, shard_count, d_errors));
     if (n_own) {
-        CHECK(prep_for_slot(c, (int)s.sp, (int)s.si));
-        CHECK(score_list(c, c->d_cand_sel, n_own, d_errors, (int)shard_count, (int)shard_rank, (int)s.sp, (int)s.si, nullptr));
+        CHECK(score_list(c, c->d_cand_sel, n_own, d_errors, (int)shard_count, (int)shard_rank, (int)s.sp, (int)s.si, nullptr, true));
     }
     if (!n_own) c->best_valid = false;
     c->pend = true; c->pend_n = n; c->pend_sp = palette; c->pend_si = index; c->pend_method = method;
diff --git a/snesimage_amd/csrc/kernels.hpp b/snesimage_amd/csrc/kernels.hpp
--- a/snesimage_amd/csrc/kernels.hpp
+++ b/snesimage_amd/csrc/kernels.hpp
@@ -101,15 +101,17 @@
     pal_xyb[3 * i] = X; pal_xyb[3 * i + 1] = Y; pal_xyb[3 * i + 2] = B;
 }
 
+__device__ __forceinline__ void candidate_row(uint32_t rgb8, const float *__restrict__ eotf, float *__restrict__ o) {
+    float r = eotf[rgb8 & 0xff], g = eotf[(rgb8 >> 8) & 0xff], b = eotf[(rgb8 >> 16) & 0xff];
+    float X, Y, B;
+    linear_to_positive_xyb(r, g, b, X, Y, B);
+    o[0] = r; o[1] = g; o[2] = b; o[3] = X; o[4] = Y; o[5] = B; o[6] = __uint_as_float(rgb8); o[7] = 0.0f;
+}
 __device__ __forceinline__ void candidate_tables_body(const uint8_t *__restrict__ rgb5, int n, const float *__restrict__ eotf, float *__restrict__ cand_tab) {
     int k = blockIdx.x * blockDim.x + threadIdx.x;
     if (k >= n) return;
     uint32_t rgb8 = rgb5_to_rgb8(rgb5[3 * k], rgb5[3 * k + 1], rgb5[3 * k + 2]);
-    float r = eotf[rgb8 & 0xff], g = eotf[(rgb8 >> 8) & 0xff], b = eotf[(rgb8 >> 16) & 0xff];
-    float X, Y, B;
-    linear_to_positive_xyb(r, g, b, X, Y, B);
-    float *o = cand_tab + 8 * (size_t)k;
-    o[0] = r; o[1] = g; o[2] = b; o[3] = X; o[4] = Y; o[5] = B; o[6] = __uint_as_float(rgb8); o[7] = 0.0f;
+    candidate_row(rgb8, eotf, cand_tab + 8 * (size_t)k);
 }
 
 constexpr int kDedupColours = 32768;
@@ -802,5 +804,18 @@
 __global__ __launch_bounds__(256) void k_final_score_wave(const double *__restrict__ part, int ncand, Geom G, double *__restrict__ errors, int err_stride, int err_offset, int *__restrict__ zero = nullptr, int nzero = 0) {
     final_score_wave_body(part, ncand, G, errors, err_stride, err_offset, zero, nzero);
 }
-
-}
+__global__ __launch_bounds__(1024) void k_final_score_dedup(const double *__restrict__ part, int ncand, Geom G, double *errors, int err_stride, int err_offset, int *__restrict__ zero, int nzero,
+                                                            const uint8_t *__restrict__ rgb5, int *__restrict__ holder, unsigned int *__restrict__ ticket) {
+    final_score_wave_body(part, ncand, G, errors, err_stride, err_offset, zero, nzero);
+    __shared__ int s_last;
+    __threadfence();
+    __syncthreads();
+    if (threadIdx.x == 0) s_last = atomicAdd(ticket, 1u) == gridDim.x - 1u ? 1 : 0;
+    __syncthreads();
+    if (!s_last) return;
+    __threadfence();
+    dedup_copy_body(rgb5, ncand, holder, errors, err_stride, err_offset);
+    if (threadIdx.x == 0) *ticket = 0u;
+}
+
+}
diff --git a/snesimage_amd/csrc/kernels_opt.hpp b/snesimage_amd/csrc/kernels_opt.hpp
--- a/snesimage_amd/csrc/kernels_opt.hpp
+++ b/snesimage_amd/csrc/kernels_opt.hpp
@@ -677,10 +677,8 @@
     z = (z ^ (z >> 27)) * 0x94D049BB133111EBull;
     return z ^ (z >> 31);
 }
-__device__ __forceinline__ void gen_candidates_body(int method, int n, unsigned long long key, const uint8_t *__restrict__ colors, int slot, int channel, uint8_t *__restrict__ cand,
-                                                    int rank, int count, uint8_t *__restrict__ sel, double *__restrict__ errors) {
-    int k = blockIdx.x * blockDim.x + threadIdx.x;
-    if (k >= n) return;
+__device__ __forceinline__ uint32_t gen_candidate_at(int k, int method, unsigned long long key, const uint8_t *__restrict__ colors, int slot, int channel, uint8_t *__restrict__ cand,
+                                                 int rank, int count, uint8_t *__restrict__ sel, double *__restrict__ errors) {
     uint8_t c[3];
     if (method == 0) {
         unsigned long long z = dev_mix64(key + ((unsigned long long)k + 1ull) * 0x9E3779B97F4A7C15ull);
@@ -696,6 +694,13 @@
         errors[k] = __longlong_as_double(0x7ff0000000000000ll);
         if (k % count == rank) { const int j = k / count; sel[3 * j] = c[0]; sel[3 * j + 1] = c[1]; sel[3 * j + 2] = c[2]; }
     }
+    return (uint32_t)c[0] | ((uint32_t)c[1] << 8) | ((uint32_t)c[2] << 16);
+}
+__device__ __forceinline__ void gen_candidates_body(int method, int n, unsigned long long key, const uint8_t *__restrict__ colors, int slot, int channel, uint8_t *__restrict__ cand,
+                                                    int rank, int count, uint8_t *__restrict__ sel, double *__restrict__ errors) {
+    int k = blockIdx.x * blockDim.x + threadIdx.x;
+    if (k >= n) return;
+    gen_candidate_at(k, method, key, colors, slot, channel, cand, rank, count, sel, errors);
 }
 
 __global__ void k_shard_select(const uint8_t *__restrict__ cand, int n, int rank, int count, uint8_t *__restrict__ sel, double *__restrict__ errors) {
diff --git a/snesimage_amd/csrc/kernels_sparse.hpp b/snesimage_amd/csrc/kernels_sparse.hpp
--- a/snesimage_amd/csrc/kernels_sparse.hpp
+++ b/snesimage_amd/csrc/kernels_sparse.hpp
@@ -1241,4 +1241,27 @@
 __global__ __launch_bounds__(256, 1) void k_sparse_v_base(SparseParams P) { sparse_v_base_body(P); }
 __global__ __launch_bounds__(256) void k_build_plist(const unsigned long long *__restrict__ pack, int npx, uint4 *__restrict__ plist, int *__restrict__ count) { build_plist_body(pack, npx, plist, count); }
 
-}
+struct CallHeadParams {
+    PrepParams prep; int pixel_blocks; uint4 *plist; int *plist_count, *count_spare;
+    int method, n; unsigned long long key; const uint8_t *colors; int slot, channel; uint8_t *cand; int rank, count; uint8_t *sel; double *errors;
+    const float *eotf; float *cand_tab; int *holder;
+};
+__global__ __launch_bounds__(256) void k_call_head(CallHeadParams H) {
+    if ((int)blockIdx.x < H.pixel_blocks) {
+        prep_body(H.prep);
+        build_plist_body(H.prep.pack, H.prep.W * H.prep.H, H.plist, H.plist_count);
+        return;
+    }
+    const int b = (int)blockIdx.x - H.pixel_blocks;
+    if (b == 0 && threadIdx.x == 0) *H.count_spare = 0;
+    const int k = b * (int)blockDim.x + (int)threadIdx.x;
+    if (k >= H.n) return;
+    const uint32_t c = gen_candidate_at(k, H.method, H.key, H.colors, H.slot, H.channel, H.cand, H.rank, H.count, H.sel, H.errors);
+    int j = k;
+    if (H.sel) { if (k % H.count != H.rank) return; j = k / H.count; }
+    const uint32_t rgb8 = rgb5_to_rgb8(c & 0xffu, (c >> 8) & 0xffu, c >> 16);
+    candidate_row(rgb8, H.eotf, H.cand_tab + 8 * (size_t)j);
+    if (H.holder) { const int key = dedup_key(rgb8); if (key >= 0) atomicMin(&H.holder[key], j); }
+}
+
+}
diff --git a/snesimage_amd/csrc/window_host.inc b/snesimage_amd/csrc/window_host.inc
--- a/snesimage_amd/csrc/window_host.inc
+++ b/snesimage_amd/csrc/window_host.inc
@@ -82,7 +82,7 @@
     k->dither = c->dither; k->perceptual = c->perceptual; k->nes = c->nes; k->G = c->G; k->K = c->K; k->npx = c->npx; k->src_floats = c->src_floats; k->fast_mask = c->fast_mask;
     k->chunk = kMemberCand; k->nlanes = 1;
     k->sp.enabled = true; k->sp.side = false; k->sp.lpt = c->sp.lpt; k->sp.down1 = c->sp.down1; k->sp.h2q_max = c->sp.h2q_max; k->sp.scan4_max = c->sp.scan4_max; k->sp.vsplit = c->sp.vsplit; k->sp.down_tiles = c->sp.down_tiles; k->sp.tiles_grid = c->sp.tiles_grid; k->sp.h0_min = c->sp.h0_min; k->sp.hgrid = c->sp.hgrid; k->sp.min_n = 1;
-    k->sp.weight_mask = c->sp.weight_mask; k->sp.h_planes = c->sp.h_planes; k->sp.v2_pair = c->sp.v2_pair; k->sp.h_forms = c->sp.h_forms; k->sp.debug_poison = c->sp.debug_poison;
+    k->sp.weight_mask = c->sp.weight_mask; k->sp.h_planes = c->sp.h_planes; k->sp.v2_pair = c->sp.v2_pair; k->sp.call_ends = c->sp.call_ends; k->sp.h_forms = c->sp.h_forms; k->sp.debug_poison = c->sp.debug_poison;
     k->d_orig = c->d_orig; k->d_tile_pal = c->d_tile_pal; k->d_colors = c->d_colors; k->d_map = c->d_map; k->d_eotf = c->d_eotf; k->d_lab_eotf = c->d_lab_eotf;
     k->d_pal_rgb8 = c->d_pal_rgb8; k->d_pal_lin = c->d_pal_lin; k->d_pal_xyb = c->d_pal_xyb; k->d_pal_lab = c->d_pal_lab;
     k->d_img1C4 = c->d_img1C4; k->d_mu1R4 = c->d_mu1R4; k->d_sd1R4 = c->d_sd1R4; k->d_a1R4 = c->d_a1R4; k->d_r1R4 = c->d_r1R4; k->d_labpx = c->d_labpx; k->d_labpxT = c->d_labpxT; k->d_target = c->d_target; k->d_labpx_t = c->d_labpx_t; k->d_labpxT_t = c->d_labpxT_t; k->od_n = c->od_n; memcpy(k->od_tab, c->od_tab, sizeof k->od_tab);
```
